# polimi-ispl/deep_prior_interpolation

Hardware: AMD Instinct MI355X
Metric: Adam iters/sec on 3D MultiRes-UNet (whole job over n_gpus; per_gpu beside it); recon SNR(dB) vs ref under config.snr_vs_reference (higher is better)
Workload: dtype f32

## Files before the change

deep_prior_interpolation_amd/_lib.py:

```python
import ctypes as C
import os

_HERE = os.path.dirname(os.path.abspath(__file__))
LIB_PATH = os.path.join(_HERE, "libdpi_hip.so")


class DpiError(RuntimeError):
    pass


ABI_VERSION = 406

IO_X_BF16, IO_Y_BF16, IO_DY_BF16, IO_DX_BF16 = 1, 2, 4, 8
STORE_FWD_BF16, STORE_GRAD_BF16 = 1, 2


class ConvDesc(C.Structure):
    _fields_ = [("size", C.c_int), ("Cin", C.c_int), ("Cout", C.c_int), ("D", C.c_int), ("H", C.c_int), ("W", C.c_int),
                ("k", C.c_int), ("kd", C.c_int), ("stride", C.c_int), ("precision", C.c_int), ("io", C.c_int)]

    def __init__(self, Cin=0, Cout=0, D=1, H=1, W=1, k=1, kd=1, stride=1, precision=0, io=0):
        super().__init__(C.sizeof(ConvDesc), int(Cin), int(Cout), int(D), int(H), int(W), int(k), int(kd), int(stride), int(precision), int(io))


class AdamTensor(C.Structure):
    _fields_ = [("p", C.c_void_p), ("g", C.c_void_p), ("m", C.c_void_p), ("v", C.c_void_p)]


_P = C.c_void_p
_I = C.c_int
_Z = C.c_size_t
_F = C.c_float
_U64 = C.c_uint64
_DESC = C.POINTER(ConvDesc)
_U = C.c_uint

SIGNATURES = {
    "dpi_last_error": (C.c_char_p, []),
    "dpi_version": (_I, []),
    "dpi_conv_desc_size": (_I, []),
    "dpi_device_info": (_I, [_I, C.POINTER(_I), C.POINTER(_I), C.POINTER(_Z), C.c_char_p, _I]),
    "dpi_profile_marker": (_I, [_I, _P]),
    "dpi_conv_fwd_stat_blocks": (_I, [_DESC]),
    "dpi_conv_fwd": (_I, [_DESC, _P, _P, _P, _P, _P, _P, _P]),
    "dpi_conv_bwd_data": (_I, [_DESC, _P, _P, _P, _I, _P]),
    "dpi_conv_fwd_ws_floats": (_Z, [_DESC]),
    "dpi_conv_bwd_data_ws_floats": (_Z, [_DESC]),
    "dpi_conv_fwd_ws": (_I, [_DESC, _P, _P, _P, _P, _P, _P, _P, _Z, _P]),
    "dpi_conv_bwd_data_ws": (_I, [_DESC, _P, _P, _P, _I, _P, _Z, _P]),
    "dpi_conv_bwd_data_dual": (_I, [_DESC, _P, _P, _DESC, _P, _P, _P, _I, _P, _Z, _P]),
    "dpi_conv_bwd_weight_ws_floats": (_Z, [_DESC]),
    "dpi_conv_bwd_weight": (_I, [_DESC, _P, _P, _P, _P, _P, _Z, _P]),
    "dpi_stat_blocks": (_I, [_I, _Z]),
    "dpi_channel_stats": (_I, [_P, _P, _I, _Z, _P, _P]),
    "dpi_bn_finalize": (_I, [_P, _I, _I, _Z, _P, _P, _F, _F, _F, _I, _P, _P, _P, _P, _P, _P, _P]),
    "dpi_chain_apply": (_I, [_P, _P, _I, _Z, _P, _P]),
    "dpi_bn_bwd_reduce": (_I, [_P, _P, _P, _P, _P, _P, _F, _F, _I, _Z, _P, _P]),
    "dpi_bn_bwd_apply": (_I, [_P, _P, _P, _P, _P, _P, _F, _F, _P, _I, _I, _Z, _P, _P, _P, _P]),
    "dpi_bn_bwd_apply_fork": (_I, [_P, _P, _P, _P, _P, _P, _F, _F, _P, _I, _I, _Z, _P, _P, _P,
                                   _P, _P, _P, _P, _P, _F, _P, _P, _P, _P, _P, _P, _F, _P, _P]),
    "dpi_bn_bwd_apply_dual": (_I, [_P, _I, _I, _Z] + [_P, _P, _P, _P, _P, _F, _P, _P, _P, _P] * 2 + [_I, _I, _P, _P, _P, _F, _P, _P]),
    "dpi_chain_add_stats": (_I, [_P, _P, _P, _P, _I, _Z, _F, _P, _P, _P]),
    "dpi_lrelu_bwd": (_I, [_P, _P, _F, _Z, _P, _P]),
    "dpi_act_fwd": (_I, [_P, _Z, _I, _P, _P]),
    "dpi_act_bwd": (_I, [_P, _P, _Z, _I, _P, _P]),
    "dpi_add": (_I, [_P, _P, _Z, _P, _P]),
    "dpi_channel_sum": (_I, [_P, _I, _Z, _P, _P, _P]),
    "dpi_upsample2x_fwd": (_I, [_P, _P, _I, _I, _I, _I, _I, _I, _I, _I, _P, _P]),
    "dpi_upsample2x_bwd_ws_floats": (_Z, [_I, _I, _I, _I, _I, _I, _I, _I]),
    "dpi_upsample2x_bwd": (_I, [_P, _I, _I, _I, _I, _I, _I, _I, _I, _P, _P, _P]),
    "dpi_crop_copy": (_I, [_P, _I, _I, _I, _I, _I, _I, _I, _I, _I, _I, _P, _P]),
    "dpi_crop_copy_bwd": (_I, [_P, _I, _I, _I, _I, _I, _I, _I, _I, _I, _I, _P, _P]),
    "dpi_maxpool2x2_fwd": (_I, [_P, _I, _I, _I, _P, _P]),
    "dpi_maxpool2x2_bwd": (_I, [_P, _P, _I, _I, _I, _P, _P]),
    "dpi_deconv4x4s2_fwd": (_I, [_P, _P, _P, _I, _I, _I, _I, _P, _P]),
    "dpi_deconv4x4s2_bwd_data": (_I, [_P, _P, _I, _I, _I, _I, _P, _P]),
    "dpi_deconv4x4s2_bwd_weight": (_I, [_P, _P, _I, _I, _I, _I, _P, _P]),
    "dpi_loss_ws_doubles": (_Z, [_Z]),
    "dpi_masked_loss": (_I, [_P, _P, _P, _Z, _I, _F, _P, _P, _P, _P]),
    "dpi_adam_multi": (_I, [_P, _P, _I, _P, C.c_double, C.c_double, C.c_double, _P, _P]),
    "dpi_langevin_multi": (_I, [_P, _P, _I, _P, _I, C.c_double, C.c_double, C.c_double, C.c_double, C.c_double, _U64, _P, _P, _P]),
    "dpi_moments_update": (_I, [_P, _P, _P, _Z, _P, _I, _I, _P, _P]),
    "dpi_loop_control": (_I, [_P, _P, _P, _I, _P, _P, _P, _I, C.c_double, C.c_double, _I, C.c_double, C.c_double, _I, C.c_double, _P]),
    "dpi_copy_if": (_I, [_P, _P, _P, _Z, _P]),
    "dpi_masked_loss_holdout": (_I, [_P, _P, _P, _P, _I, _I, _Z, _I, _F, _P, _P, _P, _P]),
    "dpi_loop_control_holdout": (_I, [_P, _P, _P, _I, _P, _P, _P, _I, C.c_double, C.c_double, _I, C.c_double, C.c_double, _I, C.c_double, _P]),
    "dpi_ema_loss": (_I, [_P, _P, _P, _P, _P, _I, _I, _Z, _I, _F, _P, _P, _P, _P, _P]),
    "dpi_loop_control_ema": (_I, [_P, _P, _I, _P, _P, _I, _P, _P, _P, _I, C.c_double, C.c_double, _I, C.c_double, C.c_double, _I, C.c_double, _P]),
    "dpi_noise_add": (_I, [_P, _Z, _F, _U64, _P, _P, _P]),
    "dpi_fill_normal": (_I, [_P, _Z, _F, _F, _U64, _U64, _P]),
    "dpi_fir_axis0": (_I, [_P, _P, _I, _I, _I, _Z, _P, _P]),
    "dpi_axpy": (_I, [_F, _P, _Z, _P, _P]),
    "dpi_diff_axis": (_I, [_P, _Z, _I, _Z, _I, _F, _I, _P, _P]),
    "dpi_hale2d": (_I, [_P, _P, _P, _P, _Z, _I, _I, _I, _P, _P]),
    "dpi_structure_tensor": (_I, [_P, _Z, _I, _I, _F, _F, _P, _P, _P, _P]),
    "dpi_dips": (_I, [_P, _P, _P, _Z, _P, _P, _P]),
    "dpi_hale_sections": (_I, [_P, _P, _I, _I, _I, _I, _I, _P, _P]),
    "dpi_structure_tensor_sections": (_I, [_P, _I, _I, _I, _I, _F, _F, _F, _P, _P, _P, _P, _P, _P]),
    "dpi_max_ws_floats": (_Z, [_Z]),
    "dpi_scaled_max": (_I, [_P, _Z, _F, _P, _P, _P]),
    "dpi_threshold": (_I, [_P, _Z, _P, _P, _P]),
    "dpi_pocs_project": (_I, [_P, _P, _P, _Z, _P, _P]),
    "dpi_overlap_add": (_I, [_P, _I, _I, _I, _I, _I, _I, _P, _I, _I, _I, _P]),
    "dpi_overlap_normalize": (_I, [_P, _I, _I, _I, _I, _I, _I, _I, _I, _I, _F, _P]),
    "dpi_overlap_add_weighted": (_I, [_P, _P, _I, _I, _I, _I, _I, _I, _P, _I, _P, _I, _P, _I, _U, _P, _I, _I, _I, _I, _P]),
    "dpi_overlap_finalize_weighted": (_I, [_P, _I, _I, _I, _I, _F, _P, _P, _P]),
    "dpi_channel_stats_io": (_I, [_P, _P, _I, _Z, _P, _U, _P]),
    "dpi_chain_apply_io": (_I, [_P, _P, _I, _Z, _P, _U, _P]),
    "dpi_chain_add_stats_io": (_I, [_P, _P, _P, _P, _I, _Z, _F, _P, _P, _U, _P]),
    "dpi_bn_bwd_reduce_io": (_I, [_P, _P, _P, _P, _P, _P, _F, _F, _I, _Z, _P, _U, _P]),
    "dpi_bn_bwd_apply_io": (_I, [_P, _P, _P, _P, _P, _P, _F, _F, _P, _I, _I, _Z, _P, _P, _P, _U, _P]),
    "dpi_bn_bwd_apply_fork_io": (_I, [_P, _P, _P, _P, _P, _P, _F, _F, _P, _I, _I, _Z, _P, _P, _P,
                                      _P, _P, _P, _P, _P, _F, _P, _P, _P, _P, _P, _P, _F, _P, _U, _P]),
    "dpi_bn_bwd_apply_dual_io": (_I, [_P, _I, _I, _Z] + [_P, _P, _P, _P, _P, _F, _P, _P, _P, _P] * 2 + [_I, _I, _P, _P, _P, _F, _P, _U, _P]),
    "dpi_upsample2x_fwd_io": (_I, [_P, _P, _I, _I, _I, _I, _I, _I, _I, _I, _P, _U, _P]),
    "dpi_upsample2x_bwd_io": (_I, [_P, _I, _I, _I, _I, _I, _I, _I, _I, _P, _P, _U, _P]),
    "dpi_noise_add_io": (_I, [_P, _Z, _F, _U64, _P, _P, _U, _P]),
    "dpi_noise_add_regen_io": (_I, [_Z, _F, _U64, _U64, _F, _U64, _P, _P, _U, _P]),
    "dpi_set_option": (_I, [C.c_char_p, _I]),
    "dpi_pack_scratch_bytes": (_Z, []),
    "dpi_pack_release": (_I, []),
    "dpi_pack_forget": (_I, [_P]),
    "dpi_pack_slot_count": (_Z, []),
    "dpi_join_bwd_ws_doubles": (_Z, [_I, _Z]),
    "dpi_join_bwd": (_I, [_P, _P, _P, _P, _P, _F, _I, _Z,  _P, _P, _P, _P, _P, _F,  _P, _P, _P, _P, _P, _F,  _P, _P,  _I, _I, _P, _P, _P, _F,
                          _P, _P, _P, _P, _P, _P, _P, _U, _P]),
    "dpi_chain_add_apply": (_I, [_P, _P, _P, _P, _P, _I, _Z, _P, _U, _P]),
}

_lib = None


def load():
    global _lib
    if _lib is not None:
        return _lib
    if not os.path.exists(LIB_PATH):
        raise DpiError("libdpi_hip.so not found at %s — run `python -c 'import __graft_entry__ as g; g.build()'` "
                       "(hipcc --offload-arch=gfx950); there is no CPU fallback" % LIB_PATH)
    import torch
    lib = C.CDLL(LIB_PATH)
    for name, (res, args) in SIGNATURES.items():
        try:
            fn = getattr(lib, name)
        except AttributeError as e:
            raise DpiError("libdpi_hip.so does not export %s (stale build?)" % name) from e
        fn.restype = res
        fn.argtypes = args
    if lib.dpi_version() < ABI_VERSION or lib.dpi_conv_desc_size() != C.sizeof(ConvDesc):
        raise DpiError("libdpi_hip.so is ABI version %d with a %d-byte dpi_conv_desc; this binding needs >= %d and %d bytes (stale build? "
                       "re-run __graft_entry__.build())" % (lib.dpi_version(), lib.dpi_conv_desc_size(), ABI_VERSION, C.sizeof(ConvDesc)))
    lib.set_option = lambda key, value: check(lib.dpi_set_option(key.encode(), int(value)), "dpi_set_option(%s)" % key)
    _lib = lib
    return lib


def check(code, what=""):
    if code != 0:
        msg = load().dpi_last_error()
        raise DpiError("%s failed (%d): %s" % (what, code, msg.decode() if msg else "?"))


def ptr(t):
    return None if t is None else t.data_ptr()


def stream():
    import torch
    return torch.cuda.current_stream().cuda_stream
```

deep_prior_interpolation_amd/csrc/api.cpp:

```cpp
#include <stdarg.h>
#include <string.h>
#include "common.h"

static thread_local char g_err[512] = "";

void dpi_set_error(const char* fmt, ...) {
  va_list ap;
  va_start(ap, fmt);
  vsnprintf(g_err, sizeof(g_err), fmt, ap);
  va_end(ap);
}

int dpi_check_launch(const char* what) {
  const hipError_t e = hipGetLastError();
  if (e != hipSuccess) {
    dpi_set_error("%s: %s", what, hipGetErrorString(e));
    return DPI_E_LAUNCH;
  }
  return DPI_OK;
}

extern "C" const char* dpi_last_error(void) { return g_err; }
extern "C" int dpi_version(void) { return 406; }
extern "C" int dpi_conv_desc_size(void) { return (int)sizeof(dpi_conv_desc); }

extern "C" int dpi_device_info(int device, int* cus, int* lds_bytes, size_t* hbm_bytes, char* name, int name_len) {
  hipDeviceProp_t p;
  const hipError_t e = hipGetDeviceProperties(&p, device);
  if (e != hipSuccess) {
    dpi_set_error("device_info: %s", hipGetErrorString(e));
    return DPI_E_LAUNCH;
  }
  if (cus) *cus = p.multiProcessorCount;
  if (lds_bytes) *lds_bytes = (int)p.sharedMemPerBlock;
  if (hbm_bytes) *hbm_bytes = p.totalGlobalMem;
  if (name && name_len > 0) {
    strncpy(name, p.gcnArchName, name_len - 1);
    name[name_len - 1] = 0;
  }
  return DPI_OK;
}

__global__ void dpi_marker_kernel() {}

extern "C" int dpi_profile_marker(int id, void* stream) {
  DPI_REQUIRE(id >= 1 && id < 65536, "profile_marker: id %d out of range", id);
  dpi_marker_kernel<<<(unsigned)id, 64, 0, (hipStream_t)stream>>>();
  return dpi_check_launch("profile_marker");
}

extern "C" int dpi_set_option(const char* key, int value) {
  DPI_REQUIRE(key != nullptr, "set_option: key is NULL");
  struct Entry { const char* key; int lo, hi; void (*set)(int); };
  static const Entry table[] = {
      {"splitk", 0, 1, dpi_set_splitk},
      {"dual_bwd_data", 0, 1, dpi_set_dual_bwd_data},
      {"bw_pair", 0, 2, dpi_set_bw_pair},
      {"bw_workgroups", 1, 1 << 24, [](int v) { dpi_set_bw_tuning(v, -1); }},
      {"bw_xcd_order", 0, 1, [](int v) { dpi_set_bw_tuning(0, v); }},
      {"mfma_min_cout", 0, 1 << 20, dpi_set_mfma_min_cout},
      {"bwd_weight_mfma_min_cout", 0, 1 << 20, dpi_set_bwd_weight_mfma_min_cout},
      {"fewco_mfma", 0, 1, dpi_set_fewco_mfma},
      {"q4", 0, 2, [](int v) { dpi_set_q4(v, -1); }},
      {"q4_ck", 0, 4, [](int v) { dpi_set_q4(-1, v); }},
      {"q4_debug", 0, 0xFFFF, dpi_set_q4_debug},
      {"bf16_debug", 0, 0x7F, dpi_set_bf16_debug},
  };
  for (const Entry& e : table)
    if (strcmp(key, e.key) == 0) {
      DPI_REQUIRE(value >= e.lo && value <= e.hi && !(strcmp(key, "q4_ck") == 0 && value != 0 && value != 2 && value != 4),
                  "set_option: %s = %d out of range [%d, %d]", key, value, e.lo, e.hi);
      e.set(value);
      return DPI_OK;
    }
  dpi_set_error("set_option: unknown key '%s'", key);
  return DPI_E_ARG;
}
```

deep_prior_interpolation_amd/csrc/dpi_hip_internal.h:

```cpp
#pragma once
#define DPI_INTERNAL __attribute__((visibility("hidden")))
extern "C" {
DPI_INTERNAL void dpi_set_bw_tuning(int want_workgroups, int xcd_order);
DPI_INTERNAL void dpi_set_bf16_debug(int flags);
DPI_INTERNAL void dpi_set_splitk(int on);
DPI_INTERNAL void dpi_set_dual_bwd_data(int on);
DPI_INTERNAL void dpi_set_bw_pair(int mode);
DPI_INTERNAL void dpi_set_mfma_min_cout(int n);
DPI_INTERNAL void dpi_set_bwd_weight_mfma_min_cout(int n);
DPI_INTERNAL void dpi_set_fewco_mfma(int on);
DPI_INTERNAL void dpi_set_q4(int on, int ck);
DPI_INTERNAL void dpi_set_q4_debug(int flags);
}
```

deep_prior_interpolation_amd/csrc/elementwise.hip:

```cpp
#include "common.h"
#include <stdlib.h>

namespace {

constexpr int kStatSpan = 16384;
constexpr int kMaxStatBlocks = 2048;

__host__ __device__ inline size_t stat_span(size_t V, int nblk) {
  size_t s = (V + nblk - 1) / nblk;
  return (s + 3) & ~(size_t)3;
}

typedef float ew_f32x4 __attribute__((ext_vector_type(4)));
constexpr size_t kNtMinFloats = (size_t)32 << 20;
__device__ __forceinline__ float4 ld4(const float* p, bool nt) {
  if (nt) { const ew_f32x4 v = __builtin_nontemporal_load(reinterpret_cast<const ew_f32x4*>(p)); return make_float4(v[0], v[1], v[2], v[3]); }
  return *reinterpret_cast<const float4*>(p);
}
__device__ __forceinline__ void st4(float* p, float4 v, bool nt) {
  if (nt) __builtin_nontemporal_store((ew_f32x4){v.x, v.y, v.z, v.w}, reinterpret_cast<ew_f32x4*>(p));
  else *reinterpret_cast<float4*>(p) = v;
}

template <bool xb = false>
__global__ __launch_bounds__(256) void channel_stats_kernel(const float* __restrict__ x, const float* __restrict__ chain,
                                                            int C, size_t V, int nblk, double* __restrict__ partials) {
  const bool nt = (size_t)gridDim.y * V >= kNtMinFloats;
  const int c = blockIdx.y, b = blockIdx.x;
  const size_t span = stat_span(V, nblk);
  const size_t beg = (size_t)b * span, end = beg + span < V ? beg + span : V;
  const float* __restrict__ xc = dpi_at(x, (size_t)c * V, xb);
  const Chain t = load_chain(chain, c);
  double s = 0.0, q = 0.0;
  const bool vec = (V & 3) == 0;
  for (size_t i = beg + (size_t)threadIdx.x * 4; i < end; i += 1024) {
    float v[4];
    if (vec) {
      const float4 f = dpi_ld4(xc, i, xb, nt);
      v[0] = f.x; v[1] = f.y; v[2] = f.z; v[3] = f.w;
    } else {
#pragma unroll
      for (int k = 0; k < 4; ++k) v[k] = i + k < end ? dpi_ld(xc, i + k, xb) : 0.f;
    }
    float ls = 0.f;
    double lq = 0.0;
#pragma unroll
    for (int k = 0; k < 4; ++k)
      if (i + k < end) {
        const float y = apply_chain(t, v[k]);
        ls += y;
        lq += (double)y * y;
      }
    s += ls; q += lq;
  }
  __shared__ double sh[8];
  const double S = block_sum(s, sh);
  const double Q = block_sum(q, sh + 4);
  if (threadIdx.x == 0) {
    partials[((size_t)b * C + c) * 2 + 0] = S;
    partials[((size_t)b * C + c) * 2 + 1] = Q;
  }
}

__global__ __launch_bounds__(256) void bn_finalize_kernel(const double* __restrict__ partials, int nblk, int C, double count,
                                                         const float* __restrict__ gamma, const float* __restrict__ beta,
                                                         float eps, float momentum, float slope, int act_first,
                                                         const float* __restrict__ in_chain, float* running_mean, float* running_var, int64_t* nbt,
                                                         float* __restrict__ mean_invstd, float* __restrict__ chain_out) {
  const int c = blockIdx.x, lane = threadIdx.x;
  double s = 0.0, q = 0.0;
  {
    double s1 = 0.0, q1 = 0.0;
    int b = lane;
    for (; b + 256 < nblk; b += 512) {
      const double2 u = *reinterpret_cast<const double2*>(partials + ((size_t)b * C + c) * 2);
      const double2 v = *reinterpret_cast<const double2*>(partials + ((size_t)(b + 256) * C + c) * 2);
      s += u.x; q += u.y; s1 += v.x; q1 += v.y;
    }
    if (b < nblk) {
      const double2 u = *reinterpret_cast<const double2*>(partials + ((size_t)b * C + c) * 2);
      s += u.x; q += u.y;
    }
    s += s1; q += q1;
  }
  __shared__ double sh[8];
  s = block_sum(s, sh);
  q = block_sum(q, sh + 4);
  if (lane == 0) {
    const double mean = s / count;
    double var = q / count - mean * mean;
    if (var < 0.0) var = 0.0;
    const float invstd = (float)(1.0 / sqrt(var + (double)eps));
    const float meanf = (float)mean;
    if (mean_invstd) { mean_invstd[c] = meanf; mean_invstd[C + c] = invstd; }
    if (running_mean) running_mean[c] = (1.f - momentum) * running_mean[c] + momentum * meanf;
    if (running_var) {
      const double unb = count > 1.0 ? var * (count / (count - 1.0)) : var;
      running_var[c] = (1.f - momentum) * running_var[c] + momentum * (float)unb;
    }
    if (nbt && c == 0) *nbt += 1;
    if (chain_out) {
      const float g = gamma ? gamma[c] : 1.f, bt = beta ? beta[c] : 0.f;
      const float a = g * invstd;
      float* o = chain_out + (size_t)c * DPI_CHAIN_STRIDE;
      if (in_chain) {
        const float* ic = in_chain + (size_t)c * DPI_CHAIN_STRIDE;
        o[0] = ic[0]; o[1] = ic[1]; o[2] = ic[2]; o[3] = a * ic[3]; o[4] = fmaf(a, ic[4], bt - meanf * a);
      } else if (act_first) { o[0] = 1.f; o[1] = 0.f; o[2] = slope; o[3] = a; o[4] = bt - meanf * a; }
      else { o[0] = a; o[1] = bt - meanf * a; o[2] = slope; o[3] = 1.f; o[4] = 0.f; }
    }
  }
}

template <bool xb = false, bool yb = false>
__global__ __launch_bounds__(256) void chain_apply_kernel(const float* __restrict__ x, const float* __restrict__ chain, size_t V,
                                                          float* __restrict__ y) {
  const bool nt = (size_t)gridDim.y * V >= kNtMinFloats;
  const int c = blockIdx.y;
  const Chain t = load_chain(chain, c);
  const float* __restrict__ xc = dpi_at(x, (size_t)c * V, xb);
  float* __restrict__ yc = dpi_at(y, (size_t)c * V, yb);
  const bool vec = (V & 3) == 0;
  for (size_t i = ((size_t)blockIdx.x * 256 + threadIdx.x) * 4; i < V; i += (size_t)gridDim.x * 1024) {
    if (vec) {
      float4 f = dpi_ld4(xc, i, xb, nt);
      f.x = apply_chain(t, f.x); f.y = apply_chain(t, f.y); f.z = apply_chain(t, f.z); f.w = apply_chain(t, f.w);
      dpi_st4(yc, i, f, yb, nt);
    } else {
      for (int k = 0; k < 4 && i + k < V; ++k) dpi_st(yc, i + k, apply_chain(t, dpi_ld(xc, i + k, xb)), yb);
    }
  }
}

struct BnBwd {
  float mean, invstd, a, pb, pre, post;
  bool chained;
  Chain in;
};
__device__ __forceinline__ BnBwd bn_bwd_consts(const float* __restrict__ mean_invstd, const float* __restrict__ gamma,
                                               const float* __restrict__ beta, const float* __restrict__ in_chain, float pre,
                                               float post, int C, int c) {
  BnBwd k;
  k.chained = in_chain != nullptr;
  k.in = load_chain(in_chain, c);
  k.mean = mean_invstd[c]; k.invstd = mean_invstd[C + c];
  k.a = (gamma ? gamma[c] : 1.f) * k.invstd;
  k.pb = (beta ? beta[c] : 0.f) - k.mean * k.a;
  k.pre = pre; k.post = post;
  return k;
}
__device__ __forceinline__ void bn_bwd_elem(const BnBwd& k, float x, float dy, float& xhat, float& g) {
  if (k.chained) x = apply_chain(k.in, x);
  const float u = x > 0.f ? x : x * k.pre;
  xhat = (u - k.mean) * k.invstd;
  const float yv = fmaf(k.a, u, k.pb);
  g = (k.post == 1.f || yv > 0.f) ? dy : dy * k.post;
}

template <bool fb = false, bool gb = false>
__global__ __launch_bounds__(256) void bn_bwd_reduce_kernel(const float* __restrict__ dy, const float* __restrict__ x,
                                                            const float* __restrict__ mean_invstd, const float* __restrict__ gamma,
                                                            const float* __restrict__ beta, const float* __restrict__ in_chain,
                                                            float pre, float post, int C, size_t V, int nblk,
                                                            double* __restrict__ partials) {
  const bool nt = (size_t)gridDim.y * V >= kNtMinFloats;
  const int c = blockIdx.y, b = blockIdx.x;
  const size_t span = stat_span(V, nblk);
  const size_t beg = (size_t)b * span, end = beg + span < V ? beg + span : V;
  const BnBwd k = bn_bwd_consts(mean_invstd, gamma, beta, in_chain, pre, post, C, c);
  const float* __restrict__ xc = dpi_at(x, (size_t)c * V, fb);
  const float* __restrict__ gc = dpi_at(dy, (size_t)c * V, gb);
  double s = 0.0, q = 0.0;
  const bool vec = (V & 3) == 0;
  for (size_t i = beg + (size_t)threadIdx.x * 4; i < end; i += 1024) {
    float xv[4], gv[4];
    if (vec) {
      const float4 f = dpi_ld4(xc, i, fb, nt);
      const float4 g = dpi_ld4(gc, i, gb, nt);
      xv[0] = f.x; xv[1] = f.y; xv[2] = f.z; xv[3] = f.w;
      gv[0] = g.x; gv[1] = g.y; gv[2] = g.z; gv[3] = g.w;
    } else {
#pragma unroll
      for (int j = 0; j < 4; ++j) { xv[j] = i + j < end ? dpi_ld(xc, i + j, fb) : 0.f; gv[j] = i + j < end ? dpi_ld(gc, i + j, gb) : 0.f; }
    }
    float ls = 0.f, lq = 0.f;
#pragma unroll
    for (int j = 0; j < 4; ++j)
      if (i + j < end) {
        float xh, g;
        bn_bwd_elem(k, xv[j], gv[j], xh, g);
        ls += g; lq = fmaf(g, xh, lq);
      }
    s += ls; q += lq;
  }
  __shared__ double sh[8];
  const double S = block_sum(s, sh);
  const double Q = block_sum(q, sh + 4);
  if (threadIdx.x == 0) {
    partials[((size_t)b * C + c) * 2 + 0] = S;
    partials[((size_t)b * C + c) * 2 + 1] = Q;
  }
}

template <bool fb = false, bool gb = false>
__global__ __launch_bounds__(256) void bn_bwd_apply_kernel(const float* __restrict__ dy, const float* __restrict__ x,
                                                           const float* __restrict__ mean_invstd, const float* __restrict__ gamma,
                                                           const float* __restrict__ beta, const float* __restrict__ in_chain,
                                                           float pre, float post, const double* __restrict__ partials, int nblk, int C, size_t V,
                                                           float* __restrict__ dx, float* __restrict__ dgamma,
                                                           float* __restrict__ dbeta) {
  const bool nt = (size_t)gridDim.y * V >= kNtMinFloats;
  const int c = blockIdx.y;
  __shared__ double tot[2];
  if (threadIdx.x < 64) {
    double s = 0.0, q = 0.0;
    for (int b = threadIdx.x; b < nblk; b += 64) {
      s += partials[((size_t)b * C + c) * 2 + 0];
      q += partials[((size_t)b * C + c) * 2 + 1];
    }
    s = wave_sum(s);
    q = wave_sum(q);
    if (threadIdx.x == 0) { tot[0] = s; tot[1] = q; }
  }
  __syncthreads();
  const BnBwd k = bn_bwd_consts(mean_invstd, gamma, beta, in_chain, pre, post, C, c);
  const float k1 = (float)(tot[0] / (double)V), k2 = (float)(tot[1] / (double)V);
  if (blockIdx.x == 0 && threadIdx.x == 0) {
    if (dgamma) dgamma[c] = (float)tot[1];
    if (dbeta) dbeta[c] = (float)tot[0];
  }
  const float* __restrict__ xc = dpi_at(x, (size_t)c * V, fb);
  const float* __restrict__ gc = dpi_at(dy, (size_t)c * V, gb);
  float* __restrict__ oc = dpi_at(dx, (size_t)c * V, gb);
  const bool vec = (V & 3) == 0;
  auto one = [&](float xv, float gv) {
    float xh, g;
    bn_bwd_elem(k, xv, gv, xh, g);
    const float du = k.a * (g - k1 - xh * k2);
    return (k.pre == 1.f || xv > 0.f) ? du : du * k.pre;
  };
  for (size_t i = ((size_t)blockIdx.x * 256 + threadIdx.x) * 4; i < V; i += (size_t)gridDim.x * 1024) {
    if (vec) {
      const float4 f = dpi_ld4(xc, i, fb, nt);
      const float4 g = dpi_ld4(gc, i, gb, nt);
      dpi_st4(oc, i, make_float4(one(f.x, g.x), one(f.y, g.y), one(f.z, g.z), one(f.w, g.w)), gb, nt);
    } else {
      for (int j = 0; j < 4 && i + j < V; ++j) dpi_st(oc, i + j, one(dpi_ld(xc, i + j, fb), dpi_ld(gc, i + j, gb)), gb);
    }
  }
}

template <bool fb = false>
__global__ __launch_bounds__(256) void chain_add_stats_kernel(const float* __restrict__ a, const float* __restrict__ chain_a,
                                                              const float* __restrict__ b, const float* __restrict__ chain_b, int C,
                                                              size_t V, int nblk, float slope, float* __restrict__ t,
                                                              double* __restrict__ partials) {
  const bool nt = (size_t)gridDim.y * V >= kNtMinFloats;
  const int c = blockIdx.y, blk = blockIdx.x;
  const size_t span = stat_span(V, nblk);
  const size_t beg = (size_t)blk * span, end = beg + span < V ? beg + span : V;
  const Chain ta = load_chain(chain_a, c), tb = load_chain(chain_b, c);
  const float* __restrict__ ac = dpi_at(a, (size_t)c * V, fb);
  const float* __restrict__ bc = dpi_at(b, (size_t)c * V, fb);
  float* __restrict__ tc = dpi_at(t, (size_t)c * V, fb);
  double s = 0.0, q = 0.0;
  const bool vec = (V & 3) == 0;
  for (size_t i = beg + (size_t)threadIdx.x * 4; i < end; i += 1024) {
    float av[4], bv[4], tv[4];
    if (vec) {
      const float4 f = dpi_ld4(ac, i, fb, nt);
      const float4 g = dpi_ld4(bc, i, fb, nt);
      av[0] = f.x; av[1] = f.y; av[2] = f.z; av[3] = f.w;
      bv[0] = g.x; bv[1] = g.y; bv[2] = g.z; bv[3] = g.w;
    } else {
#pragma unroll
      for (int j = 0; j < 4; ++j) { av[j] = i + j < end ? dpi_ld(ac, i + j, fb) : 0.f; bv[j] = i + j < end ? dpi_ld(bc, i + j, fb) : 0.f; }
    }
    float ls = 0.f;
    double lq = 0.0;
#pragma unroll
    for (int j = 0; j < 4; ++j) {
      tv[j] = dpi_stored(apply_chain(ta, av[j]) + apply_chain(tb, bv[j]), fb && t != nullptr);
      if (i + j < end) {
        const float y = tv[j] > 0.f ? tv[j] : tv[j] * slope;
        ls += y;
        lq += (double)y * y;
      }
    }
    if (t != nullptr) {
      if (vec) dpi_st4(tc, i, make_float4(tv[0], tv[1], tv[2], tv[3]), fb, nt);
      else
        for (int j = 0; j < 4 && i + j < end; ++j) dpi_st(tc, i + j, tv[j], fb);
    }
    s += ls; q += lq;
  }
  __shared__ double sh[8];
  const double S = block_sum(s, sh);
  const double Q = block_sum(q, sh + 4);
  if (threadIdx.x == 0) {
    partials[((size_t)blk * C + c) * 2 + 0] = S;
    partials[((size_t)blk * C + c) * 2 + 1] = Q;
  }
}

struct BnFork {
  const float* x;
  const float* mean_invstd;
  const float* gamma;
  const float* beta;
  const float* in_chain;
  float post;
  double* partials;
};
template <bool tb = false, bool gb = false>
__global__ __launch_bounds__(256) void bn_bwd_apply_fork_kernel(const float* __restrict__ dy, const float* __restrict__ x,
                                                                const float* __restrict__ mean_invstd, const float* __restrict__ gamma,
                                                                const float* __restrict__ beta, const float* __restrict__ in_chain,
                                                                float pre, float post, const double* __restrict__ partials, int nblk_in,
                                                                int C, size_t V, int nblk, float* __restrict__ dx,
                                                                float* __restrict__ dgamma, float* __restrict__ dbeta, BnFork fa, BnFork fb) {
  const bool nt = (size_t)gridDim.y * V >= kNtMinFloats;
  const int c = blockIdx.y, b = blockIdx.x;
  __shared__ double tot[2];
  if (threadIdx.x < 64) {
    double s = 0.0, q = 0.0;
    for (int i = threadIdx.x; i < nblk_in; i += 64) {
      s += partials[((size_t)i * C + c) * 2 + 0];
      q += partials[((size_t)i * C + c) * 2 + 1];
    }
    s = wave_sum(s);
    q = wave_sum(q);
    if (threadIdx.x == 0) { tot[0] = s; tot[1] = q; }
  }
  __syncthreads();
  const BnBwd k = bn_bwd_consts(mean_invstd, gamma, beta, in_chain, pre, post, C, c);
  const float k1 = (float)(tot[0] / (double)V), k2 = (float)(tot[1] / (double)V);
  if (b == 0 && threadIdx.x == 0) {
    if (dgamma) dgamma[c] = (float)tot[1];
    if (dbeta) dbeta[c] = (float)tot[0];
  }
  const BnBwd ka = fa.x ? bn_bwd_consts(fa.mean_invstd, fa.gamma, fa.beta, fa.in_chain, 1.f, fa.post, C, c) : k;
  const BnBwd kb = fb.x ? bn_bwd_consts(fb.mean_invstd, fb.gamma, fb.beta, fb.in_chain, 1.f, fb.post, C, c) : k;
  const size_t span = stat_span(V, nblk);
  const size_t beg = (size_t)b * span, end = beg + span < V ? beg + span : V;
  const float* __restrict__ xc = dpi_at(x, (size_t)c * V, tb);
  const float* __restrict__ gc = dpi_at(dy, (size_t)c * V, gb);
  const float* __restrict__ xa = fa.x ? dpi_at(fa.x, (size_t)c * V, tb) : xc;
  const float* __restrict__ xb = fb.x ? dpi_at(fb.x, (size_t)c * V, tb) : xc;
  float* __restrict__ oc = dpi_at(dx, (size_t)c * V, gb);
  double sa = 0.0, qa = 0.0, sb = 0.0, qb = 0.0;
  const bool vec = (V & 3) == 0;
  for (size_t i = beg + (size_t)threadIdx.x * 4; i < end; i += 1024) {
    float xv[4], gv[4], av[4], bv[4], o[4];
    if (vec) {
      const float4 f = dpi_ld4(xc, i, tb, nt);
      const float4 g = dpi_ld4(gc, i, gb, nt);
      xv[0] = f.x; xv[1] = f.y; xv[2] = f.z; xv[3] = f.w;
      gv[0] = g.x; gv[1] = g.y; gv[2] = g.z; gv[3] = g.w;
      if (fa.x) { const float4 t = dpi_ld4(xa, i, tb, nt); av[0] = t.x; av[1] = t.y; av[2] = t.z; av[3] = t.w; }
      if (fb.x) { const float4 t = dpi_ld4(xb, i, tb, nt); bv[0] = t.x; bv[1] = t.y; bv[2] = t.z; bv[3] = t.w; }
    } else {
#pragma unroll
      for (int j = 0; j < 4; ++j) {
        const bool in = i + j < end;
        xv[j] = in ? dpi_ld(xc, i + j, tb) : 0.f; gv[j] = in ? dpi_ld(gc, i + j, gb) : 0.f;
        av[j] = (in && fa.x) ? dpi_ld(xa, i + j, tb) : 0.f; bv[j] = (in && fb.x) ? dpi_ld(xb, i + j, tb) : 0.f;
      }
    }
    float lsa = 0.f, lqa = 0.f, lsb = 0.f, lqb = 0.f;
#pragma unroll
    for (int j = 0; j < 4; ++j) {
      float xh, g;
      bn_bwd_elem(k, xv[j], gv[j], xh, g);
      const float du = k.a * (g - k1 - xh * k2);
      o[j] = dpi_stored((k.pre == 1.f || xv[j] > 0.f) ? du : du * k.pre, gb);
      if (i + j < end) {
        if (fa.x) { float h, ga_; bn_bwd_elem(ka, av[j], o[j], h, ga_); lsa += ga_; lqa = fmaf(ga_, h, lqa); }
        if (fb.x) { float h, gb_; bn_bwd_elem(kb, bv[j], o[j], h, gb_); lsb += gb_; lqb = fmaf(gb_, h, lqb); }
      }
    }
    if (vec) dpi_st4(oc, i, make_float4(o[0], o[1], o[2], o[3]), gb, nt);
    else
      for (int j = 0; j < 4 && i + j < end; ++j) dpi_st(oc, i + j, o[j], gb);
    sa += lsa; qa += lqa; sb += lsb; qb += lqb;
  }
  __shared__ double sh[16];
  const double SA = block_sum(sa, sh), QA = block_sum(qa, sh + 4), SB = block_sum(sb, sh + 8), QB = block_sum(qb, sh + 12);
  if (threadIdx.x == 0) {
    if (fa.x) { fa.partials[((size_t)b * C + c) * 2 + 0] = SA; fa.partials[((size_t)b * C + c) * 2 + 1] = QA; }
    if (fb.x) { fb.partials[((size_t)b * C + c) * 2 + 0] = SB; fb.partials[((size_t)b * C + c) * 2 + 1] = QB; }
  }
}

struct BnSide {
  const float* x;
  const float* mean_invstd;
  const float* gamma;
  const float* beta;
  const float* in_chain;
  float post;
  const double* partials;
  float* dx;
  float* dgamma;
  float* dbeta;
};
template <bool tb = false, bool gb = false>
__global__ __launch_bounds__(256) void bn_bwd_apply_dual_kernel(const float* __restrict__ dy, BnSide A, BnSide B, int nblk_in, int C, size_t V,
                                                                int nblk, int f_lo, int f_hi, const float* __restrict__ f_mi,
                                                                const float* __restrict__ f_gamma, const float* __restrict__ f_beta,
                                                                float f_post, double* __restrict__ f_partials) {
  const bool nt = (size_t)gridDim.y * V >= kNtMinFloats;
  const int c = blockIdx.y, b = blockIdx.x;
  __shared__ double tot[4];
  if (threadIdx.x < 64) {
    double sa = 0.0, qa = 0.0, sb = 0.0, qb = 0.0;
    for (int i = threadIdx.x; i < nblk_in; i += 64) {
      sa += A.partials[((size_t)i * C + c) * 2 + 0]; qa += A.partials[((size_t)i * C + c) * 2 + 1];
      sb += B.partials[((size_t)i * C + c) * 2 + 0]; qb += B.partials[((size_t)i * C + c) * 2 + 1];
    }
    sa = wave_sum(sa); qa = wave_sum(qa); sb = wave_sum(sb); qb = wave_sum(qb);
    if (threadIdx.x == 0) { tot[0] = sa; tot[1] = qa; tot[2] = sb; tot[3] = qb; }
  }
  __syncthreads();
  const BnBwd ka = bn_bwd_consts(A.mean_invstd, A.gamma, A.beta, A.in_chain, 1.f, A.post, C, c);
  const BnBwd kb = bn_bwd_consts(B.mean_invstd, B.gamma, B.beta, B.in_chain, 1.f, B.post, C, c);
  const float a1 = (float)(tot[0] / (double)V), a2 = (float)(tot[1] / (double)V);
  const float b1 = (float)(tot[2] / (double)V), b2 = (float)(tot[3] / (double)V);
  if (b == 0 && threadIdx.x == 0) {
    if (A.dgamma) A.dgamma[c] = (float)tot[1];
    if (A.dbeta) A.dbeta[c] = (float)tot[0];
    if (B.dgamma) B.dgamma[c] = (float)tot[3];
    if (B.dbeta) B.dbeta[c] = (float)tot[2];
  }
  const bool forked = f_partials && c >= f_lo && c < f_hi;
  const int fc = forked ? c - f_lo : 0, fC = f_hi - f_lo;
  const BnBwd kf = forked ? bn_bwd_consts(f_mi, f_gamma, f_beta, nullptr, 1.f, f_post, fC, fc) : ka;
  const size_t span = stat_span(V, nblk);
  const size_t beg = (size_t)b * span, end = beg + span < V ? beg + span : V;
  const float* __restrict__ gc = dpi_at(dy, (size_t)c * V, gb);
  const float* __restrict__ xa = dpi_at(A.x, (size_t)c * V, tb);
  const float* __restrict__ xb = dpi_at(B.x, (size_t)c * V, tb);
  float* __restrict__ oa = dpi_at(A.dx, (size_t)c * V, gb);
  float* __restrict__ ob = dpi_at(B.dx, (size_t)c * V, gb);
  double sf = 0.0, qf = 0.0;
  const bool vec = (V & 3) == 0;
  for (size_t i = beg + (size_t)threadIdx.x * 4; i < end; i += 1024) {
    float gv[4], av[4], bv[4], ra[4], rb[4];
    if (vec) {
      const float4 g = dpi_ld4(gc, i, gb, nt);
      const float4 t = dpi_ld4(xa, i, tb, nt);
      const float4 u = dpi_ld4(xb, i, tb, nt);
      gv[0] = g.x; gv[1] = g.y; gv[2] = g.z; gv[3] = g.w;
      av[0] = t.x; av[1] = t.y; av[2] = t.z; av[3] = t.w;
      bv[0] = u.x; bv[1] = u.y; bv[2] = u.z; bv[3] = u.w;
    } else {
#pragma unroll
      for (int j = 0; j < 4; ++j) {
        const bool in = i + j < end;
        gv[j] = in ? dpi_ld(gc, i + j, gb) : 0.f; av[j] = in ? dpi_ld(xa, i + j, tb) : 0.f; bv[j] = in ? dpi_ld(xb, i + j, tb) : 0.f;
      }
    }
    float lsf = 0.f, lqf = 0.f;
#pragma unroll
    for (int j = 0; j < 4; ++j) {
      float xh, g;
      bn_bwd_elem(ka, av[j], gv[j], xh, g);
      ra[j] = ka.a * (g - a1 - xh * a2);
      bn_bwd_elem(kb, bv[j], gv[j], xh, g);
      rb[j] = dpi_stored(kb.a * (g - b1 - xh * b2), gb);
      if (forked && i + j < end) { float h, gf_; bn_bwd_elem(kf, bv[j], rb[j], h, gf_); lsf += gf_; lqf = fmaf(gf_, h, lqf); }
    }
    if (vec) {
      dpi_st4(oa, i, make_float4(ra[0], ra[1], ra[2], ra[3]), gb, nt);
      dpi_st4(ob, i, make_float4(rb[0], rb[1], rb[2], rb[3]), gb, nt);
    } else {
      for (int j = 0; j < 4 && i + j < end; ++j) { dpi_st(oa, i + j, ra[j], gb); dpi_st(ob, i + j, rb[j], gb); }
    }
    sf += lsf; qf += lqf;
  }
  if (f_partials && f_hi > f_lo) {
    __shared__ double sh[8];
    const double SF = block_sum(sf, sh), QF = block_sum(qf, sh + 4);
    if (threadIdx.x == 0 && forked) {
      f_partials[((size_t)b * fC + fc) * 2 + 0] = SF;
      f_partials[((size_t)b * fC + fc) * 2 + 1] = QF;
    }
  }
}

template <bool fb = false>
__global__ __launch_bounds__(256) void chain_add_apply_kernel(const float* __restrict__ a, const float* __restrict__ chain_a,
                                                              const float* __restrict__ b, const float* __restrict__ chain_b,
                                                              const float* __restrict__ chain_out, size_t V, float* __restrict__ y) {
  const bool nt = (size_t)gridDim.y * V >= kNtMinFloats;
  const int c = blockIdx.y;
  const Chain ta = load_chain(chain_a, c), tb = load_chain(chain_b, c), to = load_chain(chain_out, c);
  const float* __restrict__ ac = dpi_at(a, (size_t)c * V, fb);
  const float* __restrict__ bc = dpi_at(b, (size_t)c * V, fb);
  float* __restrict__ yc = dpi_at(y, (size_t)c * V, fb);
  const bool vec = (V & 3) == 0;
  for (size_t i = ((size_t)blockIdx.x * 256 + threadIdx.x) * 4; i < V; i += (size_t)gridDim.x * 1024) {
    if (vec) {
      const float4 f = dpi_ld4(ac, i, fb, nt), g = dpi_ld4(bc, i, fb, nt);
      float4 o;
      o.x = apply_chain(to, apply_chain(ta, f.x) + apply_chain(tb, g.x)); o.y = apply_chain(to, apply_chain(ta, f.y) + apply_chain(tb, g.y));
      o.z = apply_chain(to, apply_chain(ta, f.z) + apply_chain(tb, g.z)); o.w = apply_chain(to, apply_chain(ta, f.w) + apply_chain(tb, g.w));
      dpi_st4(yc, i, o, fb, nt);
    } else {
      for (int j = 0; j < 4 && i + j < V; ++j)
        dpi_st(yc, i + j, apply_chain(to, apply_chain(ta, dpi_ld(ac, i + j, fb)) + apply_chain(tb, dpi_ld(bc, i + j, fb))), fb);
    }
  }
}

constexpr int kJoinSums = 24;
constexpr int kJoinGroups = 2;
struct JoinSide {
  const float* x;
  const float* mean_invstd;
  const float* gamma;
  const float* beta;
  const float* in_chain;
  float post;
  const float* fwd_chain;
};
struct JoinFork {
  int lo, hi;
  const float* mean_invstd;
  const float* gamma;
  const float* beta;
  float post;
};
template <bool fb = false, bool gb = false>
__global__ __launch_bounds__(256) void join_bwd_sums_kernel(const float* __restrict__ dy, const float* __restrict__ t,
                                                            const float* __restrict__ mean_invstd, const float* __restrict__ gamma,
                                                            const float* __restrict__ beta, float pre, JoinSide A, JoinSide B, JoinFork F,
                                                            int C, size_t V, int nblk, double* __restrict__ partials) {
  const bool nt = (size_t)gridDim.y * V >= kNtMinFloats;
  const int c = blockIdx.y, b = blockIdx.x;
  const BnBwd k = bn_bwd_consts(mean_invstd, gamma, beta, nullptr, pre, 1.f, C, c);
  const BnBwd ka = bn_bwd_consts(A.mean_invstd, A.gamma, A.beta, A.in_chain, 1.f, A.post, C, c);
  const BnBwd kb = bn_bwd_consts(B.mean_invstd, B.gamma, B.beta, B.in_chain, 1.f, B.post, C, c);
  const bool forked = c >= F.lo && c < F.hi;
  const int fC = F.hi - F.lo, fc = forked ? c - F.lo : 0;
  const BnBwd kf = forked ? bn_bwd_consts(F.mean_invstd, F.gamma, F.beta, nullptr, 1.f, F.post, fC, fc) : ka;
  const size_t span = stat_span(V, nblk);
  const size_t beg = (size_t)b * span, end = beg + span < V ? beg + span : V;
  const float* __restrict__ gc = dpi_at(dy, (size_t)c * V, gb);
  const float* __restrict__ tc = t ? dpi_at(t, (size_t)c * V, fb) : nullptr;
  const float* __restrict__ xa = dpi_at(A.x, (size_t)c * V, fb);
  const float* __restrict__ xb = dpi_at(B.x, (size_t)c * V, fb);
  const Chain fwa = load_chain(A.fwd_chain, c), fwb = load_chain(B.fwd_chain, c);
  double s[kJoinSums];
#pragma unroll
  for (int i = 0; i < kJoinSums; ++i) s[i] = 0.0;
  const bool vec = (V & 3) == 0;
  for (size_t i0 = beg + (size_t)threadIdx.x * 4; i0 < end; i0 += 1024 * kJoinGroups) {
   float l[kJoinSums];
#pragma unroll
   for (int q = 0; q < kJoinSums; ++q) l[q] = 0.f;
#pragma unroll
   for (int u = 0; u < kJoinGroups; ++u) {
    const size_t i = i0 + (size_t)u * 1024;
    if (i >= end) break;
    float gv[4], tv[4], av[4], bv[4];
    if (vec) {
      const float4 g = dpi_ld4(gc, i, gb, nt), p = dpi_ld4(xa, i, fb, nt), q = dpi_ld4(xb, i, fb, nt);
      gv[0] = g.x; gv[1] = g.y; gv[2] = g.z; gv[3] = g.w;
      av[0] = p.x; av[1] = p.y; av[2] = p.z; av[3] = p.w;
      bv[0] = q.x; bv[1] = q.y; bv[2] = q.z; bv[3] = q.w;
      if (tc) { const float4 u = dpi_ld4(tc, i, fb, nt); tv[0] = u.x; tv[1] = u.y; tv[2] = u.z; tv[3] = u.w; }
    } else {
#pragma unroll
      for (int j = 0; j < 4; ++j) {
        const bool in = i + j < end;
        gv[j] = in ? dpi_ld(gc, i + j, gb) : 0.f; tv[j] = (in && tc) ? dpi_ld(tc, i + j, fb) : 0.f;
        av[j] = in ? dpi_ld(xa, i + j, fb) : 0.f; bv[j] = in ? dpi_ld(xb, i + j, fb) : 0.f;
      }
    }
    if (!tc) {
#pragma unroll
      for (int j = 0; j < 4; ++j) tv[j] = apply_chain(fwa, av[j]) + apply_chain(fwb, bv[j]);
    }
#pragma unroll
    for (int j = 0; j < 4; ++j)
      if (i + j < end) {
        float X, D, Xa, ma, Xb, mb;
        bn_bwd_elem(k, tv[j], gv[j], X, D);
        bn_bwd_elem(ka, av[j], 1.f, Xa, ma);
        bn_bwd_elem(kb, bv[j], 1.f, Xb, mb);
        const float P = (k.pre == 1.f || tv[j] > 0.f) ? k.a : k.a * k.pre;
        l[0] += D; l[1] = fmaf(D, X, l[1]);
        const float wa = ma * P, wb = mb * P;
        const float waD = wa * D, waX = wa * X, wbD = wb * D, wbX = wb * X;
        l[2] += waD; l[3] += wa; l[4] += waX;
        l[5] = fmaf(waD, Xa, l[5]); l[6] = fmaf(wa, Xa, l[6]); l[7] = fmaf(waX, Xa, l[7]);
        l[8] += wbD; l[9] += wb; l[10] += wbX;
        l[11] = fmaf(wbD, Xb, l[11]); l[12] = fmaf(wb, Xb, l[12]); l[13] = fmaf(wbX, Xb, l[13]);
        if (forked) {
          float Xf, mf;
          bn_bwd_elem(kf, bv[j], 1.f, Xf, mf);
          const float wf = mf * wb, wfD = wf * D, wfX = wf * X, mfXf = mf * Xf;
          l[14] += wfD; l[15] += wf; l[16] += wfX; l[17] += mf; l[18] = fmaf(mf, Xb, l[18]);
          l[19] = fmaf(wfD, Xf, l[19]); l[20] = fmaf(wf, Xf, l[20]); l[21] = fmaf(wfX, Xf, l[21]); l[22] += mfXf; l[23] = fmaf(mfXf, Xb, l[23]);
        }
      }
   }
#pragma unroll
   for (int q = 0; q < kJoinSums; ++q) s[q] += (double)l[q];
  }
  __shared__ double sh[4][kJoinSums];
  const int lane = threadIdx.x & 63, wid = threadIdx.x >> 6;
#pragma unroll
  for (int i = 0; i < kJoinSums; ++i) {
    const double v = wave_sum(s[i]);
    if (lane == 0) sh[wid][i] = v;
  }
  __syncthreads();
  if (threadIdx.x < kJoinSums) {
    const int i = threadIdx.x;
    partials[((size_t)b * C + c) * kJoinSums + i] = (sh[0][i] + sh[1][i]) + (sh[2][i] + sh[3][i]);
  }
}

__global__ __launch_bounds__(64) void join_bwd_coef_kernel(const double* __restrict__ partials, int nblk, int C, double V,
                                                          const float* __restrict__ mi_b, const float* __restrict__ gamma_b, int f_lo, int f_hi,
                                                          float* __restrict__ coef, float* __restrict__ dgb, float* __restrict__ dgb_f) {
  const int c = blockIdx.x, lane = threadIdx.x;
  double s[kJoinSums];
#pragma unroll
  for (int i = 0; i < kJoinSums; ++i) s[i] = 0.0;
  for (int b = lane; b < nblk; b += 64) {
    const double* __restrict__ p = partials + ((size_t)b * C + c) * kJoinSums;
#pragma unroll
    for (int i = 0; i < kJoinSums; ++i) s[i] += p[i];
  }
#pragma unroll
  for (int i = 0; i < kJoinSums; ++i) s[i] = wave_sum(s[i]);
  if (lane != 0) return;
  const double k1 = s[0] / V, k2 = s[1] / V;
  const double Ga = s[2] - k1 * s[3] - k2 * s[4], Ha = s[5] - k1 * s[6] - k2 * s[7];
  const double Gb = s[8] - k1 * s[9] - k2 * s[10], Hb = s[11] - k1 * s[12] - k2 * s[13];
  const float k1f = (float)k1, k2f = (float)k2, a1f = (float)(Ga / V), a2f = (float)(Ha / V), b1f = (float)(Gb / V), b2f = (float)(Hb / V);
  float f1f = 0.f, f2f = 0.f;
  if (c >= f_lo && c < f_hi) {
    const double ab = (double)((gamma_b ? gamma_b[c] : 1.f) * mi_b[C + c]);
    const double T1 = s[14] - k1 * s[15] - k2 * s[16], TX = s[19] - k1 * s[20] - k2 * s[21];
    const double Gf = ab * (T1 - (double)b1f * s[17] - (double)b2f * s[18]);
    const double Hf = ab * (TX - (double)b1f * s[22] - (double)b2f * s[23]);
    f1f = (float)(Gf / V); f2f = (float)(Hf / V);
    dgb_f[c - f_lo] = (float)Hf;
    dgb_f[(f_hi - f_lo) + c - f_lo] = (float)Gf;
  }
  float* o = coef + (size_t)c * 8;
  o[0] = k1f; o[1] = k2f; o[2] = a1f; o[3] = a2f; o[4] = b1f; o[5] = b2f; o[6] = f1f; o[7] = f2f;
  dgb[c] = (float)s[1]; dgb[C + c] = (float)s[0]; dgb[2 * C + c] = (float)Ha; dgb[3 * C + c] = (float)Ga;
  dgb[4 * C + c] = (float)Hb; dgb[5 * C + c] = (float)Gb;
}

template <bool fb = false, bool gb = false>
__global__ __launch_bounds__(256) void join_bwd_apply_kernel(const float* __restrict__ dy, const float* __restrict__ t,
                                                             const float* __restrict__ mean_invstd, const float* __restrict__ gamma,
                                                             const float* __restrict__ beta, float pre, JoinSide A, JoinSide B, JoinFork F,
                                                             const float* __restrict__ coef, int C, size_t V, float* __restrict__ dxa,
                                                             float* __restrict__ dxb, float* __restrict__ dxf) {
  const bool nt = (size_t)gridDim.y * V >= kNtMinFloats;
  const int c = blockIdx.y;
  const BnBwd k = bn_bwd_consts(mean_invstd, gamma, beta, nullptr, pre, 1.f, C, c);
  const BnBwd ka = bn_bwd_consts(A.mean_invstd, A.gamma, A.beta, A.in_chain, 1.f, A.post, C, c);
  const BnBwd kb = bn_bwd_consts(B.mean_invstd, B.gamma, B.beta, B.in_chain, 1.f, B.post, C, c);
  const bool forked = c >= F.lo && c < F.hi;
  const int fC = F.hi - F.lo, fc = forked ? c - F.lo : 0;
  const BnBwd kf = forked ? bn_bwd_consts(F.mean_invstd, F.gamma, F.beta, nullptr, 1.f, F.post, fC, fc) : ka;
  const float* __restrict__ q = coef + (size_t)c * 8;
  const float k1 = q[0], k2 = q[1], a1 = q[2], a2 = q[3], b1 = q[4], b2 = q[5], f1 = q[6], f2 = q[7];
  const float* __restrict__ gc = dpi_at(dy, (size_t)c * V, gb);
  const float* __restrict__ tc = t ? dpi_at(t, (size_t)c * V, fb) : nullptr;
  const float* __restrict__ xa = dpi_at(A.x, (size_t)c * V, fb);
  const float* __restrict__ xb = dpi_at(B.x, (size_t)c * V, fb);
  const Chain fwa = load_chain(A.fwd_chain, c), fwb = load_chain(B.fwd_chain, c);
  float* __restrict__ oa = dpi_at(dxa, (size_t)c * V, gb);
  float* __restrict__ ob = forked ? dpi_at(dxf, (size_t)fc * V, gb) : dpi_at(dxb, (size_t)c * V, gb);
  const bool vec = (V & 3) == 0;
  auto one = [&](float gv, float tv, float av, float bv, float& ra, float& rb) {
    float X, g, xh, gg;
    bn_bwd_elem(k, tv, gv, X, g);
    const float du = k.a * (g - k1 - X * k2);
    const float dt = (k.pre == 1.f || tv > 0.f) ? du : du * k.pre;
    bn_bwd_elem(ka, av, dt, xh, gg);
    ra = ka.a * (gg - a1 - xh * a2);
    bn_bwd_elem(kb, bv, dt, xh, gg);
    rb = kb.a * (gg - b1 - xh * b2);
    if (forked) {
      bn_bwd_elem(kf, bv, rb, xh, gg);
      rb = kf.a * (gg - f1 - xh * f2);
    }
  };
  for (size_t i = ((size_t)blockIdx.x * 256 + threadIdx.x) * 4; i < V; i += (size_t)gridDim.x * 1024) {
    if (vec) {
      const float4 g = dpi_ld4(gc, i, gb, nt), p = dpi_ld4(xa, i, fb, nt), r = dpi_ld4(xb, i, fb, nt);
      float4 u;
      if (tc) u = dpi_ld4(tc, i, fb, nt);
      else u = make_float4(apply_chain(fwa, p.x) + apply_chain(fwb, r.x), apply_chain(fwa, p.y) + apply_chain(fwb, r.y),
                           apply_chain(fwa, p.z) + apply_chain(fwb, r.z), apply_chain(fwa, p.w) + apply_chain(fwb, r.w));
      float4 ya, yb;
      one(g.x, u.x, p.x, r.x, ya.x, yb.x); one(g.y, u.y, p.y, r.y, ya.y, yb.y);
      one(g.z, u.z, p.z, r.z, ya.z, yb.z); one(g.w, u.w, p.w, r.w, ya.w, yb.w);
      dpi_st4(oa, i, ya, gb, nt);
      dpi_st4(ob, i, yb, gb, nt);
    } else {
      for (int j = 0; j < 4 && i + j < V; ++j) {
        float ra, rb;
        const float av = dpi_ld(xa, i + j, fb), bv = dpi_ld(xb, i + j, fb);
        one(dpi_ld(gc, i + j, gb), tc ? dpi_ld(tc, i + j, fb) : apply_chain(fwa, av) + apply_chain(fwb, bv), av, bv, ra, rb);
        dpi_st(oa, i + j, ra, gb); dpi_st(ob, i + j, rb, gb);
      }
    }
  }
}

__global__ __launch_bounds__(256) void lrelu_bwd_kernel(const float* __restrict__ dy, const float* __restrict__ x, float slope,
                                                        size_t n, float* __restrict__ dx) {
  const bool nt = n >= kNtMinFloats;
  const bool vec = (n & 3) == 0;
  for (size_t i = ((size_t)blockIdx.x * 256 + threadIdx.x) * 4; i < n; i += (size_t)gridDim.x * 1024) {
    if (vec) {
      const float4 f = ld4(x + i, nt);
      float4 g = ld4(dy + i, nt);
      g.x = f.x > 0.f ? g.x : g.x * slope; g.y = f.y > 0.f ? g.y : g.y * slope;
      g.z = f.z > 0.f ? g.z : g.z * slope; g.w = f.w > 0.f ? g.w : g.w * slope;
      st4(dx + i, g, nt);
    } else {
      for (int k = 0; k < 4 && i + k < n; ++k) dx[i + k] = x[i + k] > 0.f ? dy[i + k] : dy[i + k] * slope;
    }
  }
}

__device__ __forceinline__ float act_fwd_one(int kind, float x) {
  if (kind == DPI_ACT_ELU) return x > 0.f ? x : expm1f(x);
  if (kind == DPI_ACT_TANH) return tanhf(x);
  return 1.f / (1.f + expf(-x));
}
__device__ __forceinline__ float act_bwd_one(int kind, float y, float dy) {
  if (kind == DPI_ACT_ELU) return y > 0.f ? dy : dy * (y + 1.f);
  if (kind == DPI_ACT_TANH) return dy * (1.f - y * y);
  return dy * (y * (1.f - y));
}
__global__ __launch_bounds__(256) void act_fwd_kernel(const float* __restrict__ x, size_t n, int kind, float* __restrict__ y) {
  const bool vec = (n & 3) == 0;
  for (size_t i = ((size_t)blockIdx.x * 256 + threadIdx.x) * 4; i < n; i += (size_t)gridDim.x * 1024) {
    if (vec) {
      float4 f = *reinterpret_cast<const float4*>(x + i);
      f.x = act_fwd_one(kind, f.x); f.y = act_fwd_one(kind, f.y); f.z = act_fwd_one(kind, f.z); f.w = act_fwd_one(kind, f.w);
      *reinterpret_cast<float4*>(y + i) = f;
    } else {
      for (int k = 0; k < 4 && i + k < n; ++k) y[i + k] = act_fwd_one(kind, x[i + k]);
    }
  }
}
__global__ __launch_bounds__(256) void act_bwd_kernel(const float* __restrict__ dy, const float* __restrict__ y, size_t n, int kind,
                                                      float* __restrict__ dx) {
  const bool vec = (n & 3) == 0;
  for (size_t i = ((size_t)blockIdx.x * 256 + threadIdx.x) * 4; i < n; i += (size_t)gridDim.x * 1024) {
    if (vec) {
      const float4 f = *reinterpret_cast<const float4*>(y + i);
      float4 g = *reinterpret_cast<const float4*>(dy + i);
      g.x = act_bwd_one(kind, f.x, g.x); g.y = act_bwd_one(kind, f.y, g.y); g.z = act_bwd_one(kind, f.z, g.z); g.w = act_bwd_one(kind, f.w, g.w);
      *reinterpret_cast<float4*>(dx + i) = g;
    } else {
      for (int k = 0; k < 4 && i + k < n; ++k) dx[i + k] = act_bwd_one(kind, y[i + k], dy[i + k]);
    }
  }
}

__global__ __launch_bounds__(256) void add_kernel(const float* __restrict__ a, const float* __restrict__ b, size_t n,
                                                  float* __restrict__ y) {
  const bool nt = n >= kNtMinFloats;
  const bool vec = (n & 3) == 0;
  for (size_t i = ((size_t)blockIdx.x * 256 + threadIdx.x) * 4; i < n; i += (size_t)gridDim.x * 1024) {
    if (vec) {
      const float4 f = ld4(a + i, nt);
      const float4 g = ld4(b + i, nt);
      st4(y + i, make_float4(f.x + g.x, f.y + g.y, f.z + g.z, f.w + g.w), nt);
    } else {
      for (int k = 0; k < 4 && i + k < n; ++k) y[i + k] = a[i + k] + b[i + k];
    }
  }
}

__global__ __launch_bounds__(64) void channel_sum_final_kernel(const double* __restrict__ partials, int nblk, int C,
                                                               float* __restrict__ out) {
  const int c = blockIdx.x;
  double s = 0.0;
  for (int b = threadIdx.x; b < nblk; b += 64) s += partials[((size_t)b * C + c) * 2];
  s = wave_sum(s);
  if (threadIdx.x == 0) out[c] = (float)s;
}

__device__ __forceinline__ void lin_src(int o, int n, int& i0, int& i1, float& w0, float& w1) {
  const int h = o >> 1;
  if (o & 1) { i0 = h; i1 = min(h + 1, n - 1); w0 = .75f; w1 = .25f; }
  else { i0 = max(h - 1, 0); i1 = h; w0 = (h == 0) ? 0.f : .25f; w1 = (h == 0) ? 1.f : .75f; }
}

template <bool xb = false, bool yb = false>
__global__ __launch_bounds__(256) void upsample_fwd_kernel(const float* __restrict__ x, const float* __restrict__ chain, int D, int H,
                                                           int W, int Do, int Ho, int Wo, int linear, int scale_d,
                                                           float* __restrict__ y) {
  const int c = blockIdx.y;
  const size_t Vo = (size_t)Do * Ho * Wo, V = (size_t)D * H * W;
  const Chain t = load_chain(chain, c);
  const float* __restrict__ xc = dpi_at(x, (size_t)c * V, xb);
  float* __restrict__ yc = dpi_at(y, (size_t)c * Vo, yb);
  for (size_t i = (size_t)blockIdx.x * 256 + threadIdx.x; i < Vo; i += (size_t)gridDim.x * 256) {
    const int ow = i % Wo, oh = (i / Wo) % Ho, od = i / ((size_t)Wo * Ho);
    float r;
    if (!linear) {
      const int id = scale_d ? od >> 1 : od;
      r = apply_chain(t, dpi_ld(xc, ((size_t)id * H + (oh >> 1)) * W + (ow >> 1), xb));
    } else {
      int d0, d1, h0, h1, w0, w1;
      float a0, a1, b0, b1, c0, c1;
      if (scale_d) lin_src(od, D, d0, d1, a0, a1); else { d0 = d1 = od; a0 = 1.f; a1 = 0.f; }
      lin_src(oh, H, h0, h1, b0, b1);
      lin_src(ow, W, w0, w1, c0, c1);
      auto at = [&](int d, int h, int w) { return apply_chain(t, dpi_ld(xc, ((size_t)d * H + h) * W + w, xb)); };
      const float p0 = b0 * (c0 * at(d0, h0, w0) + c1 * at(d0, h0, w1)) + b1 * (c0 * at(d0, h1, w0) + c1 * at(d0, h1, w1));
      r = a0 * p0;
      if (scale_d)
        r += a1 * (b0 * (c0 * at(d1, h0, w0) + c1 * at(d1, h0, w1)) + b1 * (c0 * at(d1, h1, w0) + c1 * at(d1, h1, w1)));
    }
    dpi_st(yc, i, r, yb);
  }
}

__device__ __forceinline__ float lin_wt(int o, int i, int n) {
  int i0, i1; float w0, w1;
  lin_src(o, n, i0, i1, w0, w1);
  return (i0 == i ? w0 : 0.f) + (i1 == i ? w1 : 0.f);
}

template <bool gb = false>
__global__ __launch_bounds__(256) void upsample_bwd_kernel(const float* __restrict__ dy, int D, int H, int W, int Do, int Ho, int Wo,
                                                           int linear, int scale_d, float* __restrict__ dx) {
  const int c = blockIdx.y;
  const size_t Vo = (size_t)Do * Ho * Wo, V = (size_t)D * H * W;
  const float* __restrict__ gc = dpi_at(dy, (size_t)c * Vo, gb);
  float* __restrict__ oc = dpi_at(dx, (size_t)c * V, gb);
  for (size_t i = (size_t)blockIdx.x * 256 + threadIdx.x; i < V; i += (size_t)gridDim.x * 256) {
    const int iw = i % W, ih = (i / W) % H, id = i / ((size_t)W * H);
    float acc = 0.f;
    if (!linear) {
      const int dlo = scale_d ? 2 * id : id, dhi = scale_d ? 2 * id + 1 : id;
      for (int od = dlo; od <= dhi && od < Do; ++od)
        for (int oh = 2 * ih; oh <= 2 * ih + 1 && oh < Ho; ++oh)
          for (int ow = 2 * iw; ow <= 2 * iw + 1 && ow < Wo; ++ow) acc += dpi_ld(gc, ((size_t)od * Ho + oh) * Wo + ow, gb);
    } else {
      const int dlo = scale_d ? max(2 * id - 1, 0) : id, dhi = scale_d ? min(2 * id + 2, Do - 1) : id;
      for (int od = dlo; od <= dhi; ++od) {
        const float wd = scale_d ? lin_wt(od, id, D) : 1.f;
        if (wd == 0.f) continue;
        for (int oh = max(2 * ih - 1, 0); oh <= min(2 * ih + 2, Ho - 1); ++oh) {
          const float wh = lin_wt(oh, ih, H);
          if (wh == 0.f) continue;
          for (int ow = max(2 * iw - 1, 0); ow <= min(2 * iw + 2, Wo - 1); ++ow) {
            const float ww = lin_wt(ow, iw, W);
            if (ww != 0.f) acc = fmaf(wd * wh * ww, dpi_ld(gc, ((size_t)od * Ho + oh) * Wo + ow, gb), acc);
          }
        }
      }
    }
    dpi_st(oc, i, acc, gb);
  }
}

template <bool SCALE_D, bool xb = false, bool yb = false>
__global__ __launch_bounds__(256) void upsample_lin_fwd_cube_kernel(const float* __restrict__ x, const float* __restrict__ chain, int D, int H,
                                                                    int W, int Do, int Ho, int Wo, float* __restrict__ y) {
  const int c = blockIdx.y;
  const size_t V = (size_t)D * H * W, Vo = (size_t)Do * Ho * Wo;
  const Chain t = load_chain(chain, c);
  const float* __restrict__ xc = dpi_at(x, (size_t)c * V, xb);
  float* __restrict__ yc = dpi_at(y, (size_t)c * Vo, yb);
  for (size_t i = (size_t)blockIdx.x * 256 + threadIdx.x; i < V; i += (size_t)gridDim.x * 256) {
    const int w = i % W, h = (i / W) % H, d = i / ((size_t)W * H);
    const int wm = max(w - 1, 0), wp = min(w + 1, W - 1), hm = max(h - 1, 0), hp = min(h + 1, H - 1);
    const int dm = SCALE_D ? max(d - 1, 0) : d, dp = SCALE_D ? min(d + 1, D - 1) : d;
    const int ds_[3] = {dm, d, dp}, hs_[3] = {hm, h, hp}, ws_[3] = {wm, w, wp};
    float lo[3][3], hi[3][3];
#pragma unroll
    for (int a = 0; a < (SCALE_D ? 3 : 1); ++a)
#pragma unroll
      for (int b = 0; b < 3; ++b) {
        const size_t row = ((size_t)ds_[SCALE_D ? a : 1] * H + hs_[b]) * W;
        const float v0 = apply_chain(t, dpi_ld(xc, row + ws_[0], xb)), v1 = apply_chain(t, dpi_ld(xc, row + ws_[1], xb)),
                    v2 = apply_chain(t, dpi_ld(xc, row + ws_[2], xb));
        lo[a][b] = .25f * v0 + .75f * v1;
        hi[a][b] = .75f * v1 + .25f * v2;
      }
#pragma unroll
    for (int od_ = 0; od_ < (SCALE_D ? 2 : 1); ++od_) {
      const int od = SCALE_D ? 2 * d + od_ : d;
      if (od >= Do) continue;
#pragma unroll
      for (int oh_ = 0; oh_ < 2; ++oh_) {
        const int oh = 2 * h + oh_;
        if (oh >= Ho) continue;
        float r0, r1;
        auto hcomb = [&](int a, float& l, float& u) {
          l = oh_ == 0 ? .25f * lo[a][0] + .75f * lo[a][1] : .75f * lo[a][1] + .25f * lo[a][2];
          u = oh_ == 0 ? .25f * hi[a][0] + .75f * hi[a][1] : .75f * hi[a][1] + .25f * hi[a][2];
        };
        if (SCALE_D) {
          float l0, u0, l1, u1, l2, u2;
          hcomb(0, l0, u0); hcomb(1, l1, u1); hcomb(2, l2, u2);
          r0 = od_ == 0 ? .25f * l0 + .75f * l1 : .75f * l1 + .25f * l2;
          r1 = od_ == 0 ? .25f * u0 + .75f * u1 : .75f * u1 + .25f * u2;
        } else {
          hcomb(0, r0, r1);
        }
        const size_t o = ((size_t)od * Ho + oh) * Wo + 2 * w;
        if (yb && 2 * w + 1 < Wo && !((o + (size_t)c * Vo) & 1)) {
          reinterpret_cast<unsigned*>(reinterpret_cast<unsigned short*>(yc) + o)[0] = dpi_pack_bf16(r0, r1);
        } else {
          if (2 * w < Wo) dpi_st(yc, o, r0, yb);
          if (2 * w + 1 < Wo) dpi_st(yc, o + 1, r1, yb);
        }
      }
    }
  }
}

__device__ __forceinline__ void lin_bwd_taps(int i, int n, int no, int (&o)[4], float (&wt)[4]) {
  o[0] = 2 * i - 1; o[1] = 2 * i; o[2] = 2 * i + 1; o[3] = 2 * i + 2;
  wt[0] = i > 0 ? .25f : 0.f;
  wt[1] = i == 0 ? 1.f : .75f;
  wt[2] = i == n - 1 ? 1.f : .75f;
  wt[3] = i < n - 1 ? .25f : 0.f;
#pragma unroll
  for (int k = 0; k < 4; ++k) {
    if (o[k] < 0 || o[k] >= no) { wt[k] = 0.f; o[k] = 0; }
  }
}

template <bool SCALE_D, bool gb = false>
__global__ __launch_bounds__(256) void upsample_lin_bwd_gather_kernel(const float* __restrict__ dy, int D, int H, int W, int Do, int Ho,
                                                                      int Wo, float* __restrict__ dx) {
  const int c = blockIdx.y;
  const size_t V = (size_t)D * H * W, Vo = (size_t)Do * Ho * Wo;
  const float* __restrict__ gc = dpi_at(dy, (size_t)c * Vo, gb);
  float* __restrict__ oc = dpi_at(dx, (size_t)c * V, gb);
  for (size_t i = (size_t)blockIdx.x * 256 + threadIdx.x; i < V; i += (size_t)gridDim.x * 256) {
    const int w = i % W, h = (i / W) % H, d = i / ((size_t)W * H);
    int ow[4], oh[4], od[4];
    float ww[4], wh[4], wd[4];
    lin_bwd_taps(w, W, Wo, ow, ww);
    lin_bwd_taps(h, H, Ho, oh, wh);
    if (SCALE_D) lin_bwd_taps(d, D, Do, od, wd);
    float acc = 0.f;
#pragma unroll
    for (int a = 0; a < (SCALE_D ? 4 : 1); ++a) {
      const int od_ = SCALE_D ? od[a] : d;
      const float wa = SCALE_D ? wd[a] : 1.f;
      float accd = 0.f;
#pragma unroll
      for (int b = 0; b < 4; ++b) {
        const size_t row = ((size_t)od_ * Ho + oh[b]) * Wo;
        const float rsum = ww[0] * dpi_ld(gc, row + ow[0], gb) + ww[1] * dpi_ld(gc, row + ow[1], gb) + ww[2] * dpi_ld(gc, row + ow[2], gb)
                           + ww[3] * dpi_ld(gc, row + ow[3], gb);
        accd = fmaf(wh[b], rsum, accd);
      }
      acc = fmaf(wa, accd, acc);
    }
    dpi_st(oc, i, acc, gb);
  }
}

template <bool ib = false, bool ob = false>
__global__ __launch_bounds__(256) void upsample_lin_bwd_axis_kernel(const float* __restrict__ in, float* __restrict__ out, unsigned outer,
                                                                    int n, int no, unsigned inner) {
  const unsigned slab = (unsigned)n * inner;
  const unsigned per = slab < 256 ? 256 / slab : 1;
  const unsigned sub = per > 1 ? threadIdx.x / slab : 0;
  const unsigned e = per > 1 ? threadIdx.x - sub * slab : blockIdx.x * 256 + threadIdx.x;
  if (e >= slab || sub >= per) return;
  const unsigned i = e / inner, in_i = e - i * inner;
  int oo[4];
  float wt[4];
  lin_bwd_taps((int)i, n, no, oo, wt);
  const unsigned o0 = oo[0] * inner + in_i, o1 = oo[1] * inner + in_i, o2 = oo[2] * inner + in_i, o3 = oo[3] * inner + in_i;
  for (unsigned o = blockIdx.y * per + sub; o < outer; o += gridDim.y * per) {
    const float* __restrict__ p = dpi_at(in, (size_t)o * no * inner, ib);
    dpi_st(out, (size_t)o * slab + e, (wt[0] * dpi_ld(p, o0, ib) + wt[1] * dpi_ld(p, o1, ib)) + (wt[2] * dpi_ld(p, o2, ib) + wt[3] * dpi_ld(p, o3, ib)), ob);
  }
}

__global__ __launch_bounds__(256) void upsample_lin_bwd_w2_kernel(const float* __restrict__ in, float* __restrict__ out, size_t rows, int n) {
  const int half = n >> 1, no = 2 * n;
  const size_t total = rows * (size_t)half;
  for (size_t p = (size_t)blockIdx.x * 256 + threadIdx.x; p < total; p += (size_t)gridDim.x * 256) {
    const size_t r = p / half;
    const int i = 2 * (int)(p - r * half);
    const float* __restrict__ row = in + r * no;
    const float4 v = *reinterpret_cast<const float4*>(row + 2 * i);
    const float lo = row[i > 0 ? 2 * i - 1 : 0], hi = row[i + 1 < n - 1 ? 2 * i + 4 : 0];
    int o[4];
    float w0[4], w1[4];
    lin_bwd_taps(i, n, no, o, w0);
    lin_bwd_taps(i + 1, n, no, o, w1);
    float2 y;
    y.x = (w0[0] * lo + w0[1] * v.x) + (w0[2] * v.y + w0[3] * v.z);
    y.y = (w1[0] * v.y + w1[1] * v.z) + (w1[2] * v.w + w1[3] * hi);
    *reinterpret_cast<float2*>(out + r * n + i) = y;
  }
}

__global__ __launch_bounds__(256) void crop_copy_kernel(const float* __restrict__ x, int D, int H, int W, int od, int oh, int ow,
                                                        int Do, int Ho, int Wo, float* __restrict__ y, int adjoint) {
  const int c = blockIdx.y;
  const size_t V = (size_t)D * H * W, Vo = (size_t)Do * Ho * Wo;
  if (!adjoint) {
    for (size_t i = (size_t)blockIdx.x * 256 + threadIdx.x; i < Vo; i += (size_t)gridDim.x * 256) {
      const int w = i % Wo, h = (i / Wo) % Ho, d = i / ((size_t)Wo * Ho);
      y[(size_t)c * Vo + i] = x[(size_t)c * V + ((size_t)(d + od) * H + h + oh) * W + w + ow];
    }
  } else {
    for (size_t i = (size_t)blockIdx.x * 256 + threadIdx.x; i < V; i += (size_t)gridDim.x * 256) {
      const int w = i % W, h = (i / W) % H, d = i / ((size_t)W * H);
      const int cd = d - od, ch = h - oh, cw = w - ow;
      const bool in = cd >= 0 && cd < Do && ch >= 0 && ch < Ho && cw >= 0 && cw < Wo;
      y[(size_t)c * V + i] = in ? x[(size_t)c * Vo + ((size_t)cd * Ho + ch) * Wo + cw] : 0.f;
    }
  }
}

__global__ __launch_bounds__(256) void fir_axis0_kernel(const float* __restrict__ x, const float* __restrict__ taps, int K, int T, size_t S,
                                                        float* __restrict__ y) {
  const int c = blockIdx.y, p = K / 2;
  const size_t n = (size_t)T * S;
  for (size_t i = (size_t)blockIdx.x * 256 + threadIdx.x; i < n; i += (size_t)gridDim.x * 256) {
    const int t = (int)(i / S);
    const size_t s_ = i % S;
    float acc = 0.f;
    for (int k = 0; k < K; ++k) {
      const int tt = t + p - k;
      if (tt >= 0 && tt < T) acc = fmaf(taps[k], x[(size_t)c * n + (size_t)tt * S + s_], acc);
    }
    y[(size_t)c * n + i] = acc;
  }
}

__global__ __launch_bounds__(256) void axpy_kernel(float a, const float* __restrict__ x, size_t n, float* __restrict__ y) {
  for (size_t i = (size_t)blockIdx.x * 256 + threadIdx.x; i < n; i += (size_t)gridDim.x * 256) y[i] = fmaf(a, x[i], y[i]);
}

inline unsigned ew_blocks(size_t n_vec4_threads) {
  size_t b = cdivz(n_vec4_threads, 256);
  if (b > 4096) b = 4096;
  if (b < 1) b = 1;
  return (unsigned)b;
}

}

extern "C" int dpi_stat_blocks(int C, size_t V) {
  if (C <= 0 || V == 0) return 0;
  size_t n = cdivz(V, kStatSpan);
  if (n > kMaxStatBlocks) n = kMaxStatBlocks;
  return (int)n;
}

#define DPI_LAUNCH_FG(io, KERNEL, GRID, ST, ...)                                          \
  do {                                                                                    \
    if (DPI_FB(io)) {                                                                     \
      if (DPI_GB(io)) KERNEL<true, true><<<GRID, 256, 0, ST>>>(__VA_ARGS__);              \
      else KERNEL<true, false><<<GRID, 256, 0, ST>>>(__VA_ARGS__);                        \
    } else {                                                                              \
      if (DPI_GB(io)) KERNEL<false, true><<<GRID, 256, 0, ST>>>(__VA_ARGS__);             \
      else KERNEL<false, false><<<GRID, 256, 0, ST>>>(__VA_ARGS__);                       \
    }                                                                                     \
  } while (0)
#define DPI_FB(io) (((io) & DPI_STORE_FWD_BF16) != 0)
#define DPI_GB(io) (((io) & DPI_STORE_GRAD_BF16) != 0)
#define DPI_REQUIRE_IO(io, what) DPI_REQUIRE(((io) & ~3u) == 0, what ": unknown storage-type bits in io = %u", (unsigned)(io))

extern "C" int dpi_channel_stats_io(const float* x, const float* chain, int C, size_t V, double* partials, unsigned io, void* stream) {
  DPI_REQUIRE(x && partials && C > 0 && V > 0, "channel_stats: bad argument");
  DPI_REQUIRE_IO(io, "channel_stats");
  const int nblk = dpi_stat_blocks(C, V);
  if (DPI_FB(io)) channel_stats_kernel<true><<<dim3(nblk, C), 256, 0, (hipStream_t)stream>>>(x, chain, C, V, nblk, partials);
  else channel_stats_kernel<false><<<dim3(nblk, C), 256, 0, (hipStream_t)stream>>>(x, chain, C, V, nblk, partials);
  return dpi_check_launch("channel_stats");
}
extern "C" int dpi_channel_stats(const float* x, const float* chain, int C, size_t V, double* partials, void* stream) {
  return dpi_channel_stats_io(x, chain, C, V, partials, 0, stream);
}

extern "C" int dpi_bn_finalize(const double* partials, int nblk, int C, size_t count, const float* gamma, const float* beta,
                               float eps, float momentum, float slope, int act_first, const float* in_chain, float* running_mean,
                               float* running_var, int64_t* num_batches_tracked, float* mean_invstd, float* chain_out,
                               void* stream) {
  DPI_REQUIRE(partials && nblk > 0 && C > 0 && count > 0, "bn_finalize: bad argument");
  DPI_REQUIRE(!in_chain || (slope == 1.f && !act_first), "bn_finalize: a composed input chain excludes a fused activation");
  bn_finalize_kernel<<<C, 256, 0, (hipStream_t)stream>>>(partials, nblk, C, (double)count, gamma, beta, eps, momentum, slope, act_first,
                                                        in_chain, running_mean, running_var, num_batches_tracked, mean_invstd, chain_out);
  return dpi_check_launch("bn_finalize");
}

extern "C" int dpi_chain_apply_io(const float* x, const float* chain, int C, size_t V, float* y, unsigned io, void* stream) {
  DPI_REQUIRE(x && y && C > 0 && V > 0, "chain_apply: bad argument");
  DPI_REQUIRE_IO(io, "chain_apply");
  if (DPI_FB(io)) chain_apply_kernel<true, true><<<dim3(ew_blocks(cdivz(V, 4)), C), 256, 0, (hipStream_t)stream>>>(x, chain, V, y);
  else chain_apply_kernel<false, false><<<dim3(ew_blocks(cdivz(V, 4)), C), 256, 0, (hipStream_t)stream>>>(x, chain, V, y);
  return dpi_check_launch("chain_apply");
}
extern "C" int dpi_chain_apply(const float* x, const float* chain, int C, size_t V, float* y, void* stream) {
  return dpi_chain_apply_io(x, chain, C, V, y, 0, stream);
}

extern "C" int dpi_bn_bwd_reduce(const float* dy, const float* x, const float* mean_invstd, const float* gamma, const float* beta,
                                 const float* in_chain, float pre_slope, float post_slope, int C, size_t V, double* partials,
                                 void* stream) {
  return dpi_bn_bwd_reduce_io(dy, x, mean_invstd, gamma, beta, in_chain, pre_slope, post_slope, C, V, partials, 0, stream);
}
extern "C" int dpi_bn_bwd_reduce_io(const float* dy, const float* x, const float* mean_invstd, const float* gamma, const float* beta,
                                    const float* in_chain, float pre_slope, float post_slope, int C, size_t V, double* partials,
                                    unsigned io, void* stream) {
  DPI_REQUIRE(dy && x && mean_invstd && partials && C > 0 && V > 0, "bn_bwd_reduce: bad argument");
  DPI_REQUIRE_IO(io, "bn_bwd_reduce");
  DPI_REQUIRE(!in_chain || pre_slope == 1.f, "bn_bwd_reduce: in_chain excludes pre_slope");
  const int nblk = dpi_stat_blocks(C, V);
  DPI_LAUNCH_FG(io, bn_bwd_reduce_kernel, dim3(nblk, C), (hipStream_t)stream, dy, x, mean_invstd, gamma, beta, in_chain, pre_slope, post_slope, C, V,
                nblk, partials);
  return dpi_check_launch("bn_bwd_reduce");
}

extern "C" int dpi_bn_bwd_apply(const float* dy, const float* x, const float* mean_invstd, const float* gamma, const float* beta,
                                const float* in_chain, float pre_slope, float post_slope, const double* partials, int nblk, int C,
                                size_t V, float* dx, float* dgamma, float* dbeta, void* stream) {
  return dpi_bn_bwd_apply_io(dy, x, mean_invstd, gamma, beta, in_chain, pre_slope, post_slope, partials, nblk, C, V, dx, dgamma, dbeta, 0, stream);
}
extern "C" int dpi_bn_bwd_apply_io(const float* dy, const float* x, const float* mean_invstd, const float* gamma, const float* beta,
                                   const float* in_chain, float pre_slope, float post_slope, const double* partials, int nblk, int C,
                                   size_t V, float* dx, float* dgamma, float* dbeta, unsigned io, void* stream) {
  DPI_REQUIRE(dy && x && mean_invstd && partials && dx && C > 0 && V > 0 && nblk > 0, "bn_bwd_apply: bad argument");
  DPI_REQUIRE_IO(io, "bn_bwd_apply");
  DPI_REQUIRE(!in_chain || pre_slope == 1.f, "bn_bwd_apply: in_chain excludes pre_slope");
  unsigned gx = ew_blocks(cdivz(V, 4 * 8));
  DPI_LAUNCH_FG(io, bn_bwd_apply_kernel, dim3(gx, C), (hipStream_t)stream, dy, x, mean_invstd, gamma, beta, in_chain, pre_slope, post_slope, partials, nblk,
                C, V, dx, dgamma, dbeta);
  return dpi_check_launch("bn_bwd_apply");
}

extern "C" int dpi_bn_bwd_apply_fork(const float* dy, const float* x, const float* mean_invstd, const float* gamma, const float* beta,
                                     const float* in_chain, float pre_slope, float post_slope, const double* partials, int nblk, int C,
                                     size_t V, float* dx, float* dgamma, float* dbeta, const float* xa, const float* mi_a,
                                     const float* gamma_a, const float* beta_a, const float* chain_a, float post_a, double* partials_a,
                                     const float* xb, const float* mi_b, const float* gamma_b, const float* beta_b, const float* chain_b,
                                     float post_b, double* partials_b, void* stream) {
  return dpi_bn_bwd_apply_fork_io(dy, x, mean_invstd, gamma, beta, in_chain, pre_slope, post_slope, partials, nblk, C, V, dx, dgamma, dbeta,
                                  xa, mi_a, gamma_a, beta_a, chain_a, post_a, partials_a, xb, mi_b, gamma_b, beta_b, chain_b, post_b, partials_b, 0,
                                  stream);
}
extern "C" int dpi_bn_bwd_apply_fork_io(const float* dy, const float* x, const float* mean_invstd, const float* gamma, const float* beta,
                                        const float* in_chain, float pre_slope, float post_slope, const double* partials, int nblk, int C,
                                        size_t V, float* dx, float* dgamma, float* dbeta, const float* xa, const float* mi_a,
                                        const float* gamma_a, const float* beta_a, const float* chain_a, float post_a, double* partials_a,
                                        const float* xb, const float* mi_b, const float* gamma_b, const float* beta_b, const float* chain_b,
                                        float post_b, double* partials_b, unsigned io, void* stream) {
  DPI_REQUIRE(dy && x && mean_invstd && partials && dx && C > 0 && V > 0 && nblk > 0, "bn_bwd_apply_fork: bad argument");
  DPI_REQUIRE_IO(io, "bn_bwd_apply_fork");
  DPI_REQUIRE(!in_chain || pre_slope == 1.f, "bn_bwd_apply_fork: in_chain excludes pre_slope");
  DPI_REQUIRE((!xa || (mi_a && partials_a)) && (!xb || (mi_b && partials_b)), "bn_bwd_apply_fork: incomplete follow-up BatchNorm");
  const int nb = dpi_stat_blocks(C, V);
  const BnFork fa{xa, mi_a, gamma_a, beta_a, chain_a, post_a, partials_a}, fb{xb, mi_b, gamma_b, beta_b, chain_b, post_b, partials_b};
  DPI_LAUNCH_FG(io, bn_bwd_apply_fork_kernel, dim3(nb, C), (hipStream_t)stream, dy, x, mean_invstd, gamma, beta, in_chain, pre_slope, post_slope,
                partials, nblk, C, V, nb, dx, dgamma, dbeta, fa, fb);
  return dpi_check_launch("bn_bwd_apply_fork");
}

extern "C" int dpi_bn_bwd_apply_dual(const float* dy, int nblk, int C, size_t V, const float* xa, const float* mi_a, const float* gamma_a,
                                     const float* beta_a, const float* chain_a, float post_a, const double* partials_a, float* dxa,
                                     float* dgamma_a, float* dbeta_a, const float* xb, const float* mi_b, const float* gamma_b,
                                     const float* beta_b, const float* chain_b, float post_b, const double* partials_b, float* dxb,
                                     float* dgamma_b, float* dbeta_b, int f_lo, int f_hi, const float* f_mi, const float* f_gamma,
                                     const float* f_beta, float f_post, double* f_partials, void* stream) {
  return dpi_bn_bwd_apply_dual_io(dy, nblk, C, V, xa, mi_a, gamma_a, beta_a, chain_a, post_a, partials_a, dxa, dgamma_a, dbeta_a, xb, mi_b, gamma_b,
                                  beta_b, chain_b, post_b, partials_b, dxb, dgamma_b, dbeta_b, f_lo, f_hi, f_mi, f_gamma, f_beta, f_post, f_partials, 0,
                                  stream);
}
extern "C" int dpi_bn_bwd_apply_dual_io(const float* dy, int nblk, int C, size_t V, const float* xa, const float* mi_a, const float* gamma_a,
                                        const float* beta_a, const float* chain_a, float post_a, const double* partials_a, float* dxa,
                                        float* dgamma_a, float* dbeta_a, const float* xb, const float* mi_b, const float* gamma_b,
                                        const float* beta_b, const float* chain_b, float post_b, const double* partials_b, float* dxb,
                                        float* dgamma_b, float* dbeta_b, int f_lo, int f_hi, const float* f_mi, const float* f_gamma,
                                        const float* f_beta, float f_post, double* f_partials, unsigned io, void* stream) {
  DPI_REQUIRE(dy && xa && xb && mi_a && mi_b && partials_a && partials_b && dxa && dxb && C > 0 && V > 0 && nblk > 0,
              "bn_bwd_apply_dual: bad argument");
  DPI_REQUIRE_IO(io, "bn_bwd_apply_dual");
  DPI_REQUIRE(!f_partials || (f_mi && f_lo >= 0 && f_hi <= C && f_lo < f_hi), "bn_bwd_apply_dual: bad fork range");
  const int nb = dpi_stat_blocks(C, V);
  const BnSide A{xa, mi_a, gamma_a, beta_a, chain_a, post_a, partials_a, dxa, dgamma_a, dbeta_a};
  const BnSide B{xb, mi_b, gamma_b, beta_b, chain_b, post_b, partials_b, dxb, dgamma_b, dbeta_b};
  DPI_LAUNCH_FG(io, bn_bwd_apply_dual_kernel, dim3(nb, C), (hipStream_t)stream, dy, A, B, nblk, C, V, nb, f_lo, f_hi, f_mi, f_gamma, f_beta, f_post,
                f_partials);
  return dpi_check_launch("bn_bwd_apply_dual");
}

static int join_blocks(int C, size_t V) { return dpi_stat_blocks(C, V); }
extern "C" size_t dpi_join_bwd_ws_doubles(int C, size_t V) { return (size_t)join_blocks(C, V) * (size_t)C * kJoinSums; }
extern "C" int dpi_join_bwd(const float* dy, const float* t, const float* mi, const float* gamma, const float* beta, float pre, int C, size_t V,
                            const float* xa, const float* mi_a, const float* gamma_a, const float* beta_a, const float* chain_a, float post_a,
                            const float* xb, const float* mi_b, const float* gamma_b, const float* beta_b, const float* chain_b, float post_b,
                            const float* fwd_chain_a, const float* fwd_chain_b,
                            int f_lo, int f_hi, const float* f_mi, const float* f_gamma, const float* f_beta, float f_post,
                            double* ws, float* coef, float* dxa, float* dxb, float* dxf, float* dgb, float* dgb_f, unsigned io, void* stream) {
  DPI_REQUIRE(dy && mi && xa && xb && mi_a && mi_b && ws && coef && dxa && dxb && dgb && C > 0 && V > 0, "join_bwd: bad argument");
  DPI_REQUIRE_IO(io, "join_bwd");
  DPI_REQUIRE(t || (fwd_chain_a && fwd_chain_b), "join_bwd: without t the two forward chains that form it are needed");
  DPI_REQUIRE(f_lo >= 0 && f_hi <= C && f_lo <= f_hi, "join_bwd: bad fork range");
  DPI_REQUIRE(f_lo == f_hi || (f_mi && dxf && dgb_f), "join_bwd: the fork range needs its BatchNorm's statistics and outputs");
  const int nblk = join_blocks(C, V);
  const JoinSide A{xa, mi_a, gamma_a, beta_a, chain_a, post_a, fwd_chain_a}, B{xb, mi_b, gamma_b, beta_b, chain_b, post_b, fwd_chain_b};
  const JoinFork F{f_lo, f_hi, f_mi, f_gamma, f_beta, f_post};
  hipStream_t st = (hipStream_t)stream;
  DPI_LAUNCH_FG(io, join_bwd_sums_kernel, dim3(nblk, C), st, dy, t, mi, gamma, beta, pre, A, B, F, C, V, nblk, ws);
  join_bwd_coef_kernel<<<C, 64, 0, st>>>(ws, nblk, C, (double)V, mi_b, gamma_b, f_lo, f_hi, coef, dgb, dgb_f);
  DPI_LAUNCH_FG(io, join_bwd_apply_kernel, dim3(ew_blocks(cdivz(V, 4 * 8)), C), st, dy, t, mi, gamma, beta, pre, A, B, F, coef, C, V, dxa, dxb, dxf);
  return dpi_check_launch("join_bwd");
}

extern "C" int dpi_chain_add_stats(const float* a, const float* chain_a, const float* b, const float* chain_b, int C, size_t V,
                                   float slope, float* t, double* partials, void* stream) {
  return dpi_chain_add_stats_io(a, chain_a, b, chain_b, C, V, slope, t, partials, 0, stream);
}
extern "C" int dpi_chain_add_stats_io(const float* a, const float* chain_a, const float* b, const float* chain_b, int C, size_t V,
                                      float slope, float* t, double* partials, unsigned io, void* stream) {
  DPI_REQUIRE(a && b && partials && C > 0 && V > 0, "chain_add_stats: bad argument");
  DPI_REQUIRE_IO(io, "chain_add_stats");
  const int nblk = dpi_stat_blocks(C, V);
  if (DPI_FB(io)) chain_add_stats_kernel<true><<<dim3(nblk, C), 256, 0, (hipStream_t)stream>>>(a, chain_a, b, chain_b, C, V, nblk, slope, t, partials);
  else chain_add_stats_kernel<false><<<dim3(nblk, C), 256, 0, (hipStream_t)stream>>>(a, chain_a, b, chain_b, C, V, nblk, slope, t, partials);
  return dpi_check_launch("chain_add_stats");
}

extern "C" int dpi_chain_add_apply(const float* a, const float* chain_a, const float* b, const float* chain_b, const float* chain_out, int C,
                                   size_t V, float* y, unsigned io, void* stream) {
  DPI_REQUIRE(a && b && y && C > 0 && V > 0, "chain_add_apply: bad argument");
  DPI_REQUIRE_IO(io, "chain_add_apply");
  if (DPI_FB(io)) chain_add_apply_kernel<true><<<dim3(ew_blocks(cdivz(V, 4)), C), 256, 0, (hipStream_t)stream>>>(a, chain_a, b, chain_b, chain_out, V, y);
  else chain_add_apply_kernel<false><<<dim3(ew_blocks(cdivz(V, 4)), C), 256, 0, (hipStream_t)stream>>>(a, chain_a, b, chain_b, chain_out, V, y);
  return dpi_check_launch("chain_add_apply");
}

extern "C" int dpi_lrelu_bwd(const float* dy, const float* x, float slope, size_t n, float* dx, void* stream) {
  DPI_REQUIRE(dy && x && dx && n > 0, "lrelu_bwd: bad argument");
  lrelu_bwd_kernel<<<ew_blocks(cdivz(n, 4)), 256, 0, (hipStream_t)stream>>>(dy, x, slope, n, dx);
  return dpi_check_launch("lrelu_bwd");
}

extern "C" int dpi_act_fwd(const float* x, size_t n, int kind, float* y, void* stream) {
  DPI_REQUIRE(x && y && n > 0 && kind >= DPI_ACT_ELU && kind <= DPI_ACT_SIGMOID, "act_fwd: bad argument");
  act_fwd_kernel<<<ew_blocks(cdivz(n, 4)), 256, 0, (hipStream_t)stream>>>(x, n, kind, y);
  return dpi_check_launch("act_fwd");
}

extern "C" int dpi_act_bwd(const float* dy, const float* y, size_t n, int kind, float* dx, void* stream) {
  DPI_REQUIRE(dy && y && dx && n > 0 && kind >= DPI_ACT_ELU && kind <= DPI_ACT_SIGMOID, "act_bwd: bad argument");
  act_bwd_kernel<<<ew_blocks(cdivz(n, 4)), 256, 0, (hipStream_t)stream>>>(dy, y, n, kind, dx);
  return dpi_check_launch("act_bwd");
}

extern "C" int dpi_add(const float* a, const float* b, size_t n, float* y, void* stream) {
  DPI_REQUIRE(a && b && y && n > 0, "add: bad argument");
  add_kernel<<<ew_blocks(cdivz(n, 4)), 256, 0, (hipStream_t)stream>>>(a, b, n, y);
  return dpi_check_launch("add");
}

extern "C" int dpi_channel_sum(const float* x, int C, size_t V, double* ws, float* out, void* stream) {
  DPI_REQUIRE(x && ws && out && C > 0 && V > 0, "channel_sum: bad argument");
  const int nblk = dpi_stat_blocks(C, V);
  channel_stats_kernel<false><<<dim3(nblk, C), 256, 0, (hipStream_t)stream>>>(x, nullptr, C, V, nblk, ws);
  if (int e = dpi_check_launch("channel_sum.stats")) return e;
  channel_sum_final_kernel<<<C, 64, 0, (hipStream_t)stream>>>(ws, nblk, C, out);
  return dpi_check_launch("channel_sum.final");
}

extern "C" int dpi_upsample2x_fwd(const float* x, const float* chain, int C, int D, int H, int W, int Do, int Ho, int Wo,
                                  int linear, float* y, void* stream) {
  return dpi_upsample2x_fwd_io(x, chain, C, D, H, W, Do, Ho, Wo, linear, y, 0, stream);
}
extern "C" int dpi_upsample2x_fwd_io(const float* x, const float* chain, int C, int D, int H, int W, int Do, int Ho, int Wo,
                                     int linear, float* y, unsigned io, void* stream) {
  DPI_REQUIRE(x && y && C > 0 && D > 0 && H > 0 && W > 0, "upsample_fwd: bad argument");
  DPI_REQUIRE_IO(io, "upsample_fwd");
  const bool fb = DPI_FB(io);
  const int scale_d = !(D == 1 && Do == 1);
  DPI_REQUIRE(Do >= 1 && Ho >= 1 && Wo >= 1 && Do <= (scale_d ? 2 * D : 1) && Ho <= 2 * H && Wo <= 2 * W,
              "upsample_fwd: output (%d,%d,%d) exceeds 2x input (%d,%d,%d)", Do, Ho, Wo, D, H, W);
  const size_t Vo = (size_t)Do * Ho * Wo, V = (size_t)D * H * W;
  if (linear && H > 1 && W > 1 && (!scale_d || D > 1)) {
    if (scale_d) {
      if (fb) upsample_lin_fwd_cube_kernel<true, true, true><<<dim3(ew_blocks(V), C), 256, 0, (hipStream_t)stream>>>(x, chain, D, H, W, Do, Ho, Wo, y);
      else upsample_lin_fwd_cube_kernel<true, false, false><<<dim3(ew_blocks(V), C), 256, 0, (hipStream_t)stream>>>(x, chain, D, H, W, Do, Ho, Wo, y);
    } else {
      if (fb) upsample_lin_fwd_cube_kernel<false, true, true><<<dim3(ew_blocks(V), C), 256, 0, (hipStream_t)stream>>>(x, chain, D, H, W, Do, Ho, Wo, y);
      else upsample_lin_fwd_cube_kernel<false, false, false><<<dim3(ew_blocks(V), C), 256, 0, (hipStream_t)stream>>>(x, chain, D, H, W, Do, Ho, Wo, y);
    }
    return dpi_check_launch("upsample_lin_fwd_cube");
  }
  if (fb) upsample_fwd_kernel<true, true><<<dim3(ew_blocks(Vo), C), 256, 0, (hipStream_t)stream>>>(x, chain, D, H, W, Do, Ho, Wo, linear, scale_d, y);
  else upsample_fwd_kernel<false, false><<<dim3(ew_blocks(Vo), C), 256, 0, (hipStream_t)stream>>>(x, chain, D, H, W, Do, Ho, Wo, linear, scale_d, y);
  return dpi_check_launch("upsample_fwd");
}

extern "C" size_t dpi_upsample2x_bwd_ws_floats(int C, int D, int H, int W, int Do, int Ho, int Wo, int linear) {
  if (!linear || C <= 0) return 0;
  const int scale_d = !(D == 1 && Do == 1);
  return (size_t)C * Do * Ho * W + (scale_d ? (size_t)C * Do * H * W : 0);
}

extern "C" int dpi_upsample2x_bwd(const float* dy, int C, int D, int H, int W, int Do, int Ho, int Wo, int linear, float* dx,
                                  float* ws, void* stream) {
  return dpi_upsample2x_bwd_io(dy, C, D, H, W, Do, Ho, Wo, linear, dx, ws, 0, stream);
}
extern "C" int dpi_upsample2x_bwd_io(const float* dy, int C, int D, int H, int W, int Do, int Ho, int Wo, int linear, float* dx,
                                     float* ws, unsigned io, void* stream) {
  DPI_REQUIRE(dy && dx && C > 0 && D > 0 && H > 0 && W > 0, "upsample_bwd: bad argument");
  DPI_REQUIRE_IO(io, "upsample_bwd");
  const bool gb = DPI_GB(io);
  const int scale_d = !(D == 1 && Do == 1);
  const size_t V = (size_t)D * H * W;
  if (linear && ws) {
    hipStream_t st = (hipStream_t)stream;
    float* t1 = ws;
    float* t2 = ws + (size_t)C * Do * Ho * W;
    DPI_REQUIRE((size_t)C * Do * Ho < (1ull << 32) && (size_t)Do * Ho * Wo < (1ull << 31) && (size_t)Do * H * W < (1ull << 31),
                "upsample_bwd: %d x %d x %d x %d exceeds the 32-bit slab indexing of the separable adjoint", C, Do, Ho, Wo);
    auto launch = [&](const float* src, float* dst, size_t outer, int n, int no, size_t inner, bool ib, bool ob) {
      const unsigned gx = (unsigned)cdivz((size_t)n * inner, 256);
      size_t gy = outer < 65535 ? outer : 65535;
      while (gy > 1 && (size_t)gx * gy > 16384) gy = (gy + 1) / 2;
      const dim3 g(gx, (unsigned)gy);
      if (ib && ob) upsample_lin_bwd_axis_kernel<true, true><<<g, 256, 0, st>>>(src, dst, (unsigned)outer, n, no, (unsigned)inner);
      else if (ib) upsample_lin_bwd_axis_kernel<true, false><<<g, 256, 0, st>>>(src, dst, (unsigned)outer, n, no, (unsigned)inner);
      else if (ob) upsample_lin_bwd_axis_kernel<false, true><<<g, 256, 0, st>>>(src, dst, (unsigned)outer, n, no, (unsigned)inner);
      else upsample_lin_bwd_axis_kernel<false, false><<<g, 256, 0, st>>>(src, dst, (unsigned)outer, n, no, (unsigned)inner);
    };
    static const bool w2 = getenv("DPI_NO_UPW2") == nullptr;
    if (w2 && !gb && Wo == 2 * W && (W & 1) == 0 && (Wo & 3) == 0 && (((uintptr_t)dy | (uintptr_t)t1) & 15) == 0) {
      const size_t rows = (size_t)C * Do * Ho, pairs = rows * (size_t)(W / 2);
      upsample_lin_bwd_w2_kernel<<<ew_blocks(cdivz(pairs, 1)), 256, 0, st>>>(dy, t1, rows, W);
    } else
    launch(dy, t1, (size_t)C * Do * Ho, W, Wo, 1, gb, false);
    launch(t1, scale_d ? t2 : dx, (size_t)C * Do, H, Ho, W, false, scale_d ? false : gb);
    if (scale_d) launch(t2, dx, C, D, Do, (size_t)H * W, false, gb);
    return dpi_check_launch("upsample_lin_bwd_axis");
  }
  if (linear) {
    if (scale_d) {
      if (gb) upsample_lin_bwd_gather_kernel<true, true><<<dim3(ew_blocks(V), C), 256, 0, (hipStream_t)stream>>>(dy, D, H, W, Do, Ho, Wo, dx);
      else upsample_lin_bwd_gather_kernel<true, false><<<dim3(ew_blocks(V), C), 256, 0, (hipStream_t)stream>>>(dy, D, H, W, Do, Ho, Wo, dx);
    } else {
      if (gb) upsample_lin_bwd_gather_kernel<false, true><<<dim3(ew_blocks(V), C), 256, 0, (hipStream_t)stream>>>(dy, D, H, W, Do, Ho, Wo, dx);
      else upsample_lin_bwd_gather_kernel<false, false><<<dim3(ew_blocks(V), C), 256, 0, (hipStream_t)stream>>>(dy, D, H, W, Do, Ho, Wo, dx);
    }
    return dpi_check_launch("upsample_lin_bwd_gather");
  }
  if (gb) upsample_bwd_kernel<true><<<dim3(ew_blocks(V), C), 256, 0, (hipStream_t)stream>>>(dy, D, H, W, Do, Ho, Wo, linear, scale_d, dx);
  else upsample_bwd_kernel<false><<<dim3(ew_blocks(V), C), 256, 0, (hipStream_t)stream>>>(dy, D, H, W, Do, Ho, Wo, linear, scale_d, dx);
  return dpi_check_launch("upsample_bwd");
}

extern "C" int dpi_crop_copy(const float* x, int C, int D, int H, int W, int od, int oh, int ow, int Do, int Ho, int Wo, float* y,
                             void* stream) {
  DPI_REQUIRE(x && y && od >= 0 && oh >= 0 && ow >= 0 && od + Do <= D && oh + Ho <= H && ow + Wo <= W, "crop_copy: bad window");
  crop_copy_kernel<<<dim3(ew_blocks((size_t)Do * Ho * Wo), C), 256, 0, (hipStream_t)stream>>>(x, D, H, W, od, oh, ow, Do, Ho, Wo,
                                                                                            y, 0);
  return dpi_check_launch("crop_copy");
}

extern "C" int dpi_crop_copy_bwd(const float* dy, int C, int D, int H, int W, int od, int oh, int ow, int Do, int Ho, int Wo,
                                 float* dx, void* stream) {
  DPI_REQUIRE(dy && dx && od >= 0 && oh >= 0 && ow >= 0 && od + Do <= D && oh + Ho <= H && ow + Wo <= W, "crop_copy_bwd: bad window");
  crop_copy_kernel<<<dim3(ew_blocks((size_t)D * H * W), C), 256, 0, (hipStream_t)stream>>>(dy, D, H, W, od, oh, ow, Do, Ho, Wo, dx,
                                                                                         1);
  return dpi_check_launch("crop_copy_bwd");
}

extern "C" int dpi_fir_axis0(const float* x, const float* taps, int K, int C, int T, size_t S, float* y, void* stream) {
  DPI_REQUIRE(x && taps && y && K > 0 && (K & 1) && C > 0 && T > 0 && S > 0, "fir_axis0: bad argument (odd tap count required)");
  fir_axis0_kernel<<<dim3(ew_blocks((size_t)T * S), C), 256, 0, (hipStream_t)stream>>>(x, taps, K, T, S, y);
  return dpi_check_launch("fir_axis0");
}

extern "C" int dpi_axpy(float a, const float* x, size_t n, float* y, void* stream) {
  DPI_REQUIRE(x && y && n > 0, "axpy: bad argument");
  axpy_kernel<<<ew_blocks(n), 256, 0, (hipStream_t)stream>>>(a, x, n, y);
  return dpi_check_launch("axpy");
}
```

deep_prior_interpolation_amd/ops.py:

```python
import ctypes as C
import os
import threading

import torch

from . import _lib
from ._lib import ConvDesc, check, ptr, stream

BN_EPS = 1e-5
BN_MOMENTUM = 0.1


def _req(t, name, act=False):
    if not t.is_cuda:
        raise _lib.DpiError("%s must live on the GPU: the HIP path has no CPU fallback" % name)
    if t.dtype != torch.float32 and not (act and t.dtype == torch.bfloat16):
        raise _lib.DpiError("%s must be float32%s (got %s)" % (name, " or bfloat16" if act else "", t.dtype))
    return t.contiguous()


STORAGE_BF16 = os.environ.get("DPI_STORAGE", "fp32") == "bf16"
_tls = threading.local()


# ... 76 lines not shown
    global PRECISION
    if name not in _PRECISIONS:
        raise ValueError("precision must be one of %s" % sorted(_PRECISIONS))
    PRECISION = _PRECISIONS[name]


def make_desc(x, w, stride, ydt=torch.float32):
    Cin, D, H, W = _dims(x)
    k = w.shape[-1]
    kd = w.shape[2] if w.ndim == 5 else 1
    if w.shape[1] != Cin:
        raise _lib.DpiError("conv: weight expects %d input channels, tensor has %d" % (w.shape[1], Cin))
    io = ((_lib.IO_X_BF16 | _lib.IO_DX_BF16) if _bf(x) else 0) | ((_lib.IO_Y_BF16 | _lib.IO_DY_BF16) if ydt == torch.bfloat16 else 0)
    return ConvDesc(Cin, w.shape[0], D, H, W, k, kd, int(stride), precision(), io)


def desc_out_dims(d):
    sd = d.stride if d.kd > 1 else 1
    return conv_out(d.D, d.kd, sd), conv_out(d.H, d.k, d.stride), conv_out(d.W, d.k, d.stride)


class KernelTimer:

    def __init__(self, match):
        self.match = match
        self.events = []

    def durations(self):
        return [a.elapsed_time(b) for _, a, b in self.events]

    def by_key(self):
        out = {}
        for key, a, b in self.events:
            out.setdefault(key, []).append(a.elapsed_time(b))
        return out


_timer = None


def set_timer(t):
    global _timer
    _timer = t


_PROFILE_TAGS = os.environ.get("DPI_PROFILE_TAGS")
_tag_ids = {}


def _tag_id(kind, d):
    key = "%s %d->%d k%d%s s%d @%dx%dx%d" % (kind, d.Cin, d.Cout, d.k, " (2-D)" if d.D == 1 else "", d.stride, d.D, d.H, d.W)
    i = _tag_ids.get(key)
    if i is None:
        i = len(_tag_ids) + 2
        _tag_ids[key] = i
    return i


if _PROFILE_TAGS:
    import atexit
    import json

    def _dump_tags():
        with open(_PROFILE_TAGS, "w") as fp:
            json.dump({str(i): k for k, i in _tag_ids.items()}, fp, indent=0)
    atexit.register(_dump_tags)


def _timed(kind, d, launch):
    if _PROFILE_TAGS:
        L = _lib.load()
        L.dpi_profile_marker(_tag_id(kind, d), stream())
        launch()
        L.dpi_profile_marker(1, stream())
        return
    key = _timer.match(kind, d) if _timer is not None else None
    if key:
        e0, e1 = torch.cuda.Event(enable_timing=True), torch.cuda.Event(enable_timing=True)
        e0.record()
        launch()
        e1.record()
        _timer.events.append((key, e0, e1))
    else:
        launch()


_ws_cache = {}


def _ws_floats(kind, d):
    key = (kind, d.Cin, d.Cout, d.D, d.H, d.W, d.k, d.kd, d.stride, d.precision, d.io)
    n = _ws_cache.get(key)
    if n is None:
        L = _lib.load()
        n = {"fwd": L.dpi_conv_fwd_ws_floats, "bwd_data": L.dpi_conv_bwd_data_ws_floats}[kind](C.byref(d))
        _ws_cache[key] = n
    return n


def reset_ws_cache():
    _ws_cache.clear()


def _conv_ws(n, like):
    return torch.empty(n, dtype=torch.float32, device=like.device) if n else None


def raw_conv_fwd(d, x, chain, w, bias, y, partials=None):
    L = _lib.load()
    n = _ws_floats("fwd", d)
    ws = _conv_ws(n, x)
    _timed("conv_fwd", d, lambda: check(L.dpi_conv_fwd_ws(C.byref(d), ptr(x), ptr(chain), ptr(w), ptr(bias), ptr(y),
                                                          ptr(partials), ptr(ws), n, stream()), "dpi_conv_fwd"))


def raw_conv_bwd_data(d, dy, w, dx, accumulate=False):
    L = _lib.load()
    n = _ws_floats("bwd_data", d)
    ws = _conv_ws(n, dy)
    _timed("conv_bwd_data", d, lambda: check(L.dpi_conv_bwd_data_ws(C.byref(d), ptr(dy), ptr(w), ptr(dx), int(accumulate),
                                                                    ptr(ws), n, stream()), "dpi_conv_bwd_data"))


def raw_conv_bwd_data_dual(d3, dy3, w3, d1, dy1, w1, dx, accumulate=False):
    L = _lib.load()
    n = _ws_floats("bwd_data", d3)
    ws = _conv_ws(n, dy3)

    def launch():
        check(L.dpi_conv_bwd_data_dual(C.byref(d3), ptr(dy3), ptr(w3), C.byref(d1), ptr(dy1), ptr(w1), ptr(dx), int(accumulate),
                                       ptr(ws), n, stream()), "dpi_conv_bwd_data_dual")
    _timed("conv_bwd_data", d3, launch)


OVERLAP_WEIGHT_GRADS = os.environ.get("DPI_OVERLAP_WGRAD", "0") == "1"
OVERLAP_IN_GRAPH = os.environ.get("DPI_OVERLAP_IN_GRAPH", "0") == "1"
OVERLAP_MAX_VOXELS = int(os.environ.get("DPI_OVERLAP_MAX_VOXELS", str(1 << 40)))


def set_weight_grad_overlap(on, in_graph=None):
    global OVERLAP_WEIGHT_GRADS, OVERLAP_IN_GRAPH
    if "DPI_OVERLAP_WGRAD" not in os.environ:
        OVERLAP_WEIGHT_GRADS = bool(on)
    if in_graph is not None and "DPI_OVERLAP_IN_GRAPH" not in os.environ:
        OVERLAP_IN_GRAPH = bool(in_graph)
_side_streams = {}
N_SIDE_STREAMS = int(os.environ.get("DPI_SIDE_STREAMS", "2"))
_side_rr = [0]
_side_used = set()
JOIN_AT = os.environ.get("DPI_JOIN_AT", "step")
_side_keep = []
_in_iteration = [False]
_deferred = []


def begin_iteration():
    _side_rr[0] = 0
    _in_iteration[0] = True
    del _deferred[:]


def abort_iteration():
    try:
        if torch.cuda.is_available():
            join_weight_grads(final=True)
            join_branch()
    finally:
        _in_iteration[0] = False
        _side_used.clear()
        del _side_keep[:]
        del _deferred[:]
        _branch_open[0] = False


def _defer(*tensors):
    if JOIN_AT == "step" and _in_iteration[0]:
        _deferred.extend(t.data_ptr() for t in tensors if t is not None)


def _side_stream():
    dev = torch.cuda.current_device()
    sts = _side_streams.get(dev)
    if sts is None:
        sts = [torch.cuda.Stream(device=dev) for _ in range(max(N_SIDE_STREAMS, 1))]
        _side_streams[dev] = sts
    i = _side_rr[0] % len(sts)
    _side_rr[0] += 1
    _side_used.add(i)
    return sts[i]


def conv_bwd_weight_async(d, x, chain, dy, dw):
    if not OVERLAP_WEIGHT_GRADS or d.D * d.H * d.W >= OVERLAP_MAX_VOXELS or (torch.cuda.is_current_stream_capturing() and not OVERLAP_IN_GRAPH):
        return raw_conv_bwd_weight(d, x, chain, dy, dw)
    side = _side_stream()
    side.wait_stream(torch.cuda.current_stream())
    with torch.cuda.stream(side):
        raw_conv_bwd_weight(d, x, chain, dy, dw)
    if JOIN_AT == "step" and _in_iteration[0]:
        _side_keep.append((x, chain, dy))
        _deferred.append(dw.data_ptr())


def join_weight_grads(final=False):
    if JOIN_AT == "step" and _in_iteration[0] and not final:
        return
    if _side_used:
        sts = _side_streams.get(torch.cuda.current_device()) or []
        for i in sorted(_side_used):
            torch.cuda.current_stream().wait_stream(sts[i])
        _side_used.clear()
    _side_keep.clear()


def finish_backward(params=None):
    join_weight_grads(final=True)
    join_branch()
    _in_iteration[0] = False
    if _deferred and params is not None:
        have = {p.grad.data_ptr() for p in params if p.grad is not None}
        lost = [q for q in _deferred if q not in have]
        if lost:
            n = len(_deferred)
            del _deferred[:]
            raise _lib.DpiError("%d of %d gradients written on a side / branch stream were copied or accumulated by autograd before that stream ran "
                                "(zero_grad(set_to_none=False), a gradient hook, retain_grad or a shared parameter?): with the once-per-step join "
                                "(DPI_JOIN_AT=step) .grad must be None when backward starts; use DPI_JOIN_AT=node otherwise" % (len(lost), n))
    del _deferred[:]


BRANCH_STREAMS = os.environ.get("DPI_BRANCH", "1") == "1"
BRANCH_SHORTCUT = int(os.environ.get("DPI_BRANCH_SHORT", "0"))
BRANCH_SKIP = os.environ.get("DPI_BRANCH_SKIP", "1") == "1"
BRANCH_SKIP_BWD = os.environ.get("DPI_BRANCH_SKIP_BWD", "1") == "1"
_branch_streams = {}
_branch_open = [False]


def branch_on():
    return (BRANCH_STREAMS and OVERLAP_WEIGHT_GRADS and _in_iteration[0] and JOIN_AT == "step"
            and not torch.cuda.is_current_stream_capturing())


def _branch_stream(kind="skip"):
    key = (torch.cuda.current_device(), kind)
    st = _branch_streams.get(key)
    if st is None:
        st = torch.cuda.Stream(device=key[0])
        _branch_streams[key] = st
    return st


class _Branch:

    def __init__(self, kind, *tensors):
        self.st = _branch_stream(kind)
        self.tensors = tensors

    def __enter__(self):
        self.st.wait_stream(torch.cuda.current_stream())
        for t in self.tensors:
            if t is not None:
                t.record_stream(self.st)
        self.ctx = torch.cuda.stream(self.st)
        self.ctx.__enter__()
        _branch_open[0] = True
        return self

    def __exit__(self, *exc):
        return self.ctx.__exit__(*exc)


def join_branch(kind=None):
    if not _branch_open[0]:
        return
    dev = torch.cuda.current_device()
    for (d, k), st in _branch_streams.items():
        if d == dev and (kind is None or k == kind):
            torch.cuda.current_stream().wait_stream(st)
    if kind is None:
        _branch_open[0] = False


def raw_conv_bwd_weight(d, x, chain, dy, dw):
    L = _lib.load()
    n = L.dpi_conv_bwd_weight_ws_floats(C.byref(d))
    ws = torch.empty(n, dtype=torch.float32, device=x.device)
    _timed("conv_bwd_weight", d, lambda: check(L.dpi_conv_bwd_weight(C.byref(d), ptr(x), ptr(chain), ptr(dy), ptr(dw),
                                                                     ptr(ws), n, stream()), "dpi_conv_bwd_weight"))


def raw_channel_sum(x, C_, V, out):
    L = _lib.load()
    nblk = L.dpi_stat_blocks(C_, V)
    ws = torch.empty(nblk * C_ * 2, dtype=torch.float64, device=x.device)
    check(L.dpi_channel_sum(ptr(x), C_, V, ptr(ws), ptr(out), stream()), "dpi_channel_sum")


def raw_bn_stats_finalize(x, chain_in, C_, V, gamma, beta, slope, running_mean, running_var, nbt, mean_invstd, chain_out,
                          eps=BN_EPS, momentum=BN_MOMENTUM, act_first=0, compose=False):
    L = _lib.load()
    nblk = L.dpi_stat_blocks(C_, V)
    part = torch.empty(nblk * C_ * 2, dtype=torch.float64, device=x.device)
    check(L.dpi_channel_stats_io(ptr(x), ptr(chain_in), C_, V, ptr(part), _io(x), stream()), "dpi_channel_stats")
    check(L.dpi_bn_finalize(ptr(part), nblk, C_, V, ptr(gamma), ptr(beta), eps, momentum, slope, act_first,
                            ptr(chain_in) if compose else None, ptr(running_mean), ptr(running_var), ptr(nbt), ptr(mean_invstd),
                            ptr(chain_out), stream()), "dpi_bn_finalize")


def raw_bn_finalize(part, nblk, C_, count, gamma, beta, slope, running_mean, running_var, nbt, mean_invstd, chain_out,
                    eps=BN_EPS, momentum=BN_MOMENTUM, act_first=0):
    L = _lib.load()
    check(L.dpi_bn_finalize(ptr(part), nblk, C_, count, ptr(gamma), ptr(beta), eps, momentum, slope, act_first, None,
                            ptr(running_mean), ptr(running_var), ptr(nbt), ptr(mean_invstd), ptr(chain_out), stream()),
          "dpi_bn_finalize")


def raw_upsample2x_bwd(dy, C_, D, H, W, Do, Ho, Wo, linear, dx):
    L = _lib.load()
    n = L.dpi_upsample2x_bwd_ws_floats(C_, D, H, W, Do, Ho, Wo, linear)
    ws = torch.empty(n, dtype=torch.float32, device=dy.device) if n else None
    _same_type(dy, dx, "upsample2x_bwd")
    check(L.dpi_upsample2x_bwd_io(ptr(dy), C_, D, H, W, Do, Ho, Wo, linear, ptr(dx), ptr(ws), _io(None, dy), stream()), "dpi_upsample2x_bwd")


def raw_chain_apply(x, chain, C_, V, y):
    L = _lib.load()
    _same_type(x, y, "chain_apply")
    check(L.dpi_chain_apply_io(ptr(x), ptr(chain), C_, V, ptr(y), _io(x), stream()), "dpi_chain_apply")


_slope_chains = {}


def slope_chain(C_, slope, device):
    key = (C_, float(slope), str(device))
    t = _slope_chains.get(key)
    if t is None:
        t = torch.tensor([1.0, 0.0, slope, 1.0, 0.0], dtype=torch.float32).repeat(C_, 1).to(device).contiguous()
        _slope_chains[key] = t
    return t


class ConvFn(torch.autograd.Function):

    @staticmethod
    def forward(ctx, x, w, b, stride):
        x, w = _req(x, "conv input", act=True), _req(w, "conv weight")
        b = _req(b, "conv bias") if b is not None else None
        d = make_desc(x, w, stride)
        Do, Ho, Wo = desc_out_dims(d)
        y = torch.empty(_like_spatial(x, d.Cout, Do, Ho, Wo), dtype=torch.float32, device=x.device)
        raw_conv_fwd(d, x, None, w, b, y)
        ctx.save_for_backward(x, w)
        ctx.d = d
        ctx.has_bias = b is not None
        return y

    @staticmethod
    def backward(ctx, dy):
        x, w = ctx.saved_tensors
        d = ctx.d
        dy = _req(dy, "conv grad")
        dx = dw = db = None
        if ctx.needs_input_grad[1]:
            dw = torch.empty_like(w)
            conv_bwd_weight_async(d, x, None, dy, dw)
        if ctx.needs_input_grad[0]:
            dx = torch.empty_like(x)
            raw_conv_bwd_data(d, dy, w, dx)
        if ctx.has_bias and ctx.needs_input_grad[2]:
            db = torch.empty(d.Cout, dtype=torch.float32, device=x.device)
            raw_channel_sum(dy, d.Cout, dy.numel() // d.Cout, db)
        join_weight_grads()
        return dx, dw, db, None


def _bn_backward(dy, x, mi, gamma, beta, pre_slope, post_slope, in_chain=None, dx=None):
    L = _lib.load()
    C_ = x.shape[1]
    V = x.numel() // C_
    nblk = L.dpi_stat_blocks(C_, V)
    part = torch.empty(nblk * C_ * 2, dtype=torch.float64, device=x.device)
    io = _io(x, dy)
    check(L.dpi_bn_bwd_reduce_io(ptr(dy), ptr(x), ptr(mi), ptr(gamma), ptr(beta), ptr(in_chain), pre_slope, post_slope, C_, V,
                                 ptr(part), io, stream()), "dpi_bn_bwd_reduce")
    if dx is None:
        dx = torch.empty_like(dy)
    _same_type(dy, dx, "bn_backward")
    dgamma = torch.empty_like(gamma)
    dbeta = torch.empty_like(gamma)
    check(L.dpi_bn_bwd_apply_io(ptr(dy), ptr(x), ptr(mi), ptr(gamma), ptr(beta), ptr(in_chain), pre_slope, post_slope, ptr(part), nblk,
                                C_, V, ptr(dx), ptr(dgamma), ptr(dbeta), io, stream()), "dpi_bn_bwd_apply")
    return dx, dgamma, dbeta


def _bn_backward_fork(dy, x, mi, gamma, beta, pre_slope, post_slope, forks):
    L = _lib.load()
    C_ = x.shape[1]
    V = x.numel() // C_
    nblk = L.dpi_stat_blocks(C_, V)
    part = torch.empty(nblk * C_ * 2, dtype=torch.float64, device=x.device)
    io = _io(x, dy)
    check(L.dpi_bn_bwd_reduce_io(ptr(dy), ptr(x), ptr(mi), ptr(gamma), ptr(beta), None, pre_slope, post_slope, C_, V, ptr(part),
                                 io, stream()), "dpi_bn_bwd_reduce")
    dx = torch.empty_like(dy)
    dgamma, dbeta = torch.empty_like(gamma), torch.empty_like(gamma)
    fparts = [torch.empty(nblk * C_ * 2, dtype=torch.float64, device=x.device) for _ in forks]
    fa = []
    for k in range(2):
        if k < len(forks):
            xk, mik, gk, ek, chk, postk = forks[k]
            _same_type(x, xk, "bn_backward_fork")
            fa += [ptr(xk), ptr(mik), ptr(gk), ptr(ek), ptr(chk), postk, ptr(fparts[k])]
        else:
            fa += [None, None, None, None, None, 1.0, None]
    check(L.dpi_bn_bwd_apply_fork_io(ptr(dy), ptr(x), ptr(mi), ptr(gamma), ptr(beta), None, pre_slope, post_slope, ptr(part), nblk, C_, V,
                                     ptr(dx), ptr(dgamma), ptr(dbeta), *fa, io, stream()), "dpi_bn_bwd_apply_fork")
    return dx, dgamma, dbeta, [(nblk, fp) for fp in fparts]


def _bn_backward_apply(dy, x, mi, gamma, beta, pre_slope, post_slope, red, in_chain=None, dx=None):
    L = _lib.load()
    C_ = x.shape[1]
    V = x.numel() // C_
    nblk, part = red
    if dx is None:
        dx = torch.empty_like(dy)
    _same_type(dy, dx, "bn_backward_apply")
    dgamma, dbeta = torch.empty_like(gamma), torch.empty_like(gamma)
    check(L.dpi_bn_bwd_apply_io(ptr(dy), ptr(x), ptr(mi), ptr(gamma), ptr(beta), ptr(in_chain), pre_slope, post_slope, ptr(part), nblk,
                                C_, V, ptr(dx), ptr(dgamma), ptr(dbeta), _io(x, dy), stream()), "dpi_bn_bwd_apply")
    return dx, dgamma, dbeta


def _bn_backward_apply_dual(dy, side_a, side_b, fork=None):
    L = _lib.load()
    xa, mia, ga, ea, cha, posta, (nblk, parta) = side_a
    xb, mib, gb, eb, chb, postb, (nblk_b, partb) = side_b
    assert nblk == nblk_b
    C_ = xa.shape[1]
    V = xa.numel() // C_
    _same_type(xa, xb, "bn_backward_apply_dual")
    dxa, dxb = torch.empty_like(dy), torch.empty_like(dy)
    dga, dea, dgb, deb = (torch.empty_like(g) for g in (ga, ga, gb, gb))
    red_f = None
    fargs = [0, 0, None, None, None, 1.0, None]
    if fork is not None:
        lo, hi, mif, gf, ef, postf = fork
        nb = L.dpi_stat_blocks(C_, V)
        pf = torch.empty(nb * (hi - lo) * 2, dtype=torch.float64, device=xa.device)
        fargs = [lo, hi, ptr(mif), ptr(gf), ptr(ef), postf, ptr(pf)]
        red_f = (nb, pf)
    check(L.dpi_bn_bwd_apply_dual_io(ptr(dy), nblk, C_, V,
                                     ptr(xa), ptr(mia), ptr(ga), ptr(ea), ptr(cha), posta, ptr(parta), ptr(dxa), ptr(dga), ptr(dea),
                                     ptr(xb), ptr(mib), ptr(gb), ptr(eb), ptr(chb), postb, ptr(partb), ptr(dxb), ptr(dgb), ptr(deb),
                                     *fargs, _io(xa, dy), stream()), "dpi_bn_bwd_apply_dual")
    return (dxa, dga, dea), (dxb, dgb, deb), red_f


JOIN_BWD_FUSED = os.environ.get("DPI_JOIN_BWD", "1") == "1"
EARLY_SHORTCUT_WGRAD = os.environ.get("DPI_EARLY_SHORTCUT_WGRAD", "0") == "1"


def _join_backward(dy, t, mi, gamma, beta, pre_slope, side_a, side_b, fork=None, fwd_chains=None):
    L = _lib.load()
    xa, mia, ga, ea, cha, posta = side_a
    xb, mib, gb, eb, chb, postb = side_b
    C_ = dy.shape[1]
    V = dy.numel() // C_
    dev = dy.device
    fwa, fwb = fwd_chains if fwd_chains is not None else (None, None)
    ws = torch.empty(L.dpi_join_bwd_ws_doubles(C_, V), dtype=torch.float64, device=dev)
    coef = torch.empty(C_ * 8, dtype=torch.float32, device=dev)
    dgb = torch.empty((6, C_), dtype=torch.float32, device=dev)
    dxa, dxb = torch.empty_like(dy), torch.empty_like(dy)
    if fork is not None:
        lo, hi, mif, gf, ef, postf, dxf = fork
        dgbf = torch.empty((2, hi - lo), dtype=torch.float32, device=dev)
        fa = [lo, hi, ptr(mif), ptr(gf), ptr(ef), postf]
    else:
        dxf = dgbf = None
        fa = [0, 0, None, None, None, 1.0]
    check(L.dpi_join_bwd(ptr(dy), ptr(t), ptr(mi), ptr(gamma), ptr(beta), pre_slope, C_, V,
                         ptr(xa), ptr(mia), ptr(ga), ptr(ea), ptr(cha), posta, ptr(xb), ptr(mib), ptr(gb), ptr(eb), ptr(chb), postb,
                         ptr(fwa), ptr(fwb), *fa, ptr(ws), ptr(coef), ptr(dxa), ptr(dxb), ptr(dxf), ptr(dgb), ptr(dgbf), _io(xa, dy), stream()),
          "dpi_join_bwd")
    f = None if dgbf is None else (dgbf[0], dgbf[1])
    return (dxa, dgb[2], dgb[3]), (dxb, dgb[4], dgb[5]), (dgb[0], dgb[1]), f


def _join_fused_ok(*tensors):
    return JOIN_BWD_FUSED and (all(x.dtype == torch.float32 for x in tensors) or all(x.dtype == torch.bfloat16 for x in tensors))


def _join_forward(a, ch_a, b, ch_b, C_, V, slope, bn, gamma, beta, mi_out, y, keep_t):
    L = _lib.load()
    dev = a.device
    t = torch.empty_like(a) if keep_t else None
    nblk = L.dpi_stat_blocks(C_, V)
    part = torch.empty(nblk * C_ * 2, dtype=torch.float64, device=dev)
    check(L.dpi_chain_add_stats_io(ptr(a), ptr(ch_a), ptr(b), ptr(ch_b), C_, V, slope, ptr(t), ptr(part), _io(a), stream()),
          "dpi_chain_add_stats")
    ch_out = torch.empty(C_ * 5, dtype=torch.float32, device=dev)
    raw_bn_finalize(part, nblk, C_, V, gamma, beta, slope, bn.running_mean, bn.running_var, bn.num_batches_tracked, mi_out, ch_out,
                    act_first=1)
    if keep_t:
        raw_chain_apply(t, ch_out, C_, V, y)
    else:
        check(L.dpi_chain_add_apply(ptr(a), ptr(ch_a), ptr(b), ptr(ch_b), ptr(ch_out), C_, V, ptr(y), _io(a), stream()), "dpi_chain_add_apply")
    return t


def _pre_chain(C_, pre_slope, device):
    return None if pre_slope == 1.0 else slope_chain(C_, pre_slope, device)


class BatchNormFn(torch.autograd.Function):

    @staticmethod
    def forward(ctx, x, gamma, beta, running_mean, running_var, nbt, post_slope, pre_slope=1.0):
        x = _req(x, "batchnorm input")
        C_ = x.shape[1]
        V = x.numel() // C_
        mi = torch.empty(2 * C_, dtype=torch.float32, device=x.device)
        chain = torch.empty(C_ * 5, dtype=torch.float32, device=x.device)
        if pre_slope != 1.0 and post_slope != 1.0:
            raise _lib.DpiError("batch_norm: pre and post activation cannot both be fused")
        raw_bn_stats_finalize(x, _pre_chain(C_, pre_slope, x.device), C_, V, gamma, beta,
                              pre_slope if pre_slope != 1.0 else post_slope, running_mean, running_var, nbt, mi, chain,
                              act_first=int(pre_slope != 1.0))
        y = torch.empty_like(x)
        raw_chain_apply(x, chain, C_, V, y)
        ctx.save_for_backward(x, gamma, beta, mi)
        ctx.slopes = (float(pre_slope), float(post_slope))
        return y

    @staticmethod
    def backward(ctx, dy):
        x, gamma, beta, mi = ctx.saved_tensors
        dx, dgamma, dbeta = _bn_backward(_req(dy, "batchnorm grad"), x, mi, gamma, beta, *ctx.slopes)
        return dx, dgamma, dbeta, None, None, None, None, None


FAN_IN = os.environ.get("DPI_FAN_IN", "1") == "1"


class FanIn:
    __slots__ = ("dx", "branched")

    def __init__(self):
        self.dx = None
        self.branched = False


class ConvBnActFn(torch.autograd.Function):

    @staticmethod
    def forward(ctx, x, w, b, gamma, beta, running_mean, running_var, nbt, stride, slope, fan=None):
        x, w = _req(x, "conv input", act=True), _req(w, "conv weight")
        ctx.fan = fan
        adt = act_dtype() if x.ndim == 5 else torch.float32
        if x.ndim != 5 and _bf(x):
            raise _lib.DpiError("conv_bn_act: bf16 storage is built for the 3-D nets only")
        d = make_desc(x, w, stride, adt)
        Do, Ho, Wo = desc_out_dims(d)
        L = _lib.load()
        r = torch.empty(_like_spatial(x, d.Cout, Do, Ho, Wo), dtype=adt, device=x.device)
        nblk = L.dpi_conv_fwd_stat_blocks(C.byref(d))
        part = torch.empty(nblk * d.Cout * 2, dtype=torch.float64, device=x.device)
        raw_conv_fwd(d, x, None, w, b, r, part)
        V = Do * Ho * Wo
        mi = torch.empty(2 * d.Cout, dtype=torch.float32, device=x.device)
        chain = torch.empty(d.Cout * 5, dtype=torch.float32, device=x.device)
        raw_bn_finalize(part, nblk, d.Cout, V, gamma, beta, slope, running_mean, running_var, nbt, mi, chain)
        y = torch.empty_like(r)
        raw_chain_apply(r, chain, d.Cout, V, y)
        ctx.save_for_backward(x, w, r, gamma, beta, mi)
        ctx.d, ctx.slope, ctx.has_bias, ctx.bias_ref = d, float(slope), b is not None, b
        return y

    @staticmethod
    def backward(ctx, dy):
        x, w, r, gamma, beta, mi = ctx.saved_tensors
        d = ctx.d
        dr, dgamma, dbeta = _bn_backward(_req(dy, "conv-bn-act grad", act=True), r, mi, gamma, beta, 1.0, ctx.slope)
        dx = dw = db = None
        if ctx.needs_input_grad[1]:
            dw = torch.empty_like(w)
            conv_bwd_weight_async(d, x, None, dr, dw)
        if ctx.needs_input_grad[0]:
            fan = ctx.fan
            if fan is not None and fan.dx is not None and fan.dx.shape == x.shape and fan.dx.dtype == x.dtype:
                if fan.branched:
                    join_branch("skip")
                raw_conv_bwd_data(d, dr, w, fan.dx, accumulate=True)
                fan.dx = None
            else:
                dx = torch.empty_like(x)
                raw_conv_bwd_data(d, dr, w, dx)
        if ctx.has_bias and ctx.needs_input_grad[2]:
            db = _zeros_like_or_none(ctx.bias_ref, dr)
        join_weight_grads()
        return dx, dw, db, dgamma, dbeta, None, None, None, None, None, None


def _cba_raw(d, x, in_chain, w, b, bn, slope, r_out, mi_out, chain_out):
    L = _lib.load()
    nblk = L.dpi_conv_fwd_stat_blocks(C.byref(d))
    part = torch.empty(nblk * d.Cout * 2, dtype=torch.float64, device=x.device)
    raw_conv_fwd(d, x, in_chain, w, b, r_out, part)
    Do, Ho, Wo = desc_out_dims(d)
    raw_bn_finalize(part, nblk, d.Cout, Do * Ho * Wo, bn.weight, bn.bias, slope, bn.running_mean, bn.running_var,
                    bn.num_batches_tracked, mi_out, chain_out)


DEAD_BIAS = "off"


def _zeros_like_or_none(b, dr=None):
    if b is None or DEAD_BIAS == "off":
        return None
    if DEAD_BIAS == "noise":
        return torch.randn_like(b) * 1e-6
    return dr.sum(dim=[0] + list(range(2, dr.ndim)), dtype=torch.float32)


class Block3dFn(torch.autograd.Function):

    @staticmethod
    def forward(ctx, x, blk, slope, *p):
        x = _req(x, "block input", act=True)
        (w1, b1, g1, e1, w2, b2, g2, e2, w3, b3, g3, e3, ws, bs, gs, es, gA, eA, gB, eB) = p
        L = _lib.load()
        dev = x.device
        f32 = dict(dtype=torch.float32, device=dev)
        adt = act_dtype()
        c1, c2, c3 = w1.shape[0], w2.shape[0], w3.shape[0]
        Ct = c1 + c2 + c3
        bn1_, bn2_, bn3_, bns_ = (m._parts()[1] for m in (blk.conv3x3, blk.conv5x5, blk.conv7x7, blk.shortcut))
        d1 = make_desc(x, w1, 1, adt)
        Do, Ho, Wo = desc_out_dims(d1)
        V = Do * Ho * Wo
        R = torch.empty(_like_spatial(x, Ct, Do, Ho, Wo), dtype=adt, device=dev)
        CH = torch.empty(Ct * 5, **f32)
        r1, r2, r3 = R[:, :c1], R[:, c1:c1 + c2], R[:, c1 + c2:]
        ch1, ch2, ch3 = CH[:c1 * 5], CH[c1 * 5:(c1 + c2) * 5], CH[(c1 + c2) * 5:]
        mi1, mi2, mi3 = (torch.empty(2 * c, **f32) for c in (c1, c2, c3))
        miA, miS, miB = (torch.empty(2 * Ct, **f32) for _ in range(3))
        dsc = make_desc(x, ws, 1, adt)
        S = torch.empty_like(R)
        chSA = torch.empty((2, Ct * 5), **f32)
        chS, chA = chSA[0], chSA[1]
        side_shortcut = BRANCH_SHORTCUT if branch_on() else 0

        def shortcut_on_branch():
            with _Branch("short", x, S, miS, chS):
                _cba_raw(dsc, x, None, ws, bs, bns_, slope, S, miS, chS)
        if side_shortcut == 1:
            shortcut_on_branch()
        _cba_raw(d1, x, None, w1, b1, bn1_, slope, r1, mi1, ch1)
        if side_shortcut == 2:
            shortcut_on_branch()
        d2 = make_desc(r1, w2, 1, adt)
        _cba_raw(d2, r1, ch1, w2, b2, bn2_, slope, r2, mi2, ch2)
        d3 = make_desc(r2, w3, 1, adt)
        _cba_raw(d3, r2, ch2, w3, b3, bn3_, slope, r3, mi3, ch3)
        A = blk.bn1
        raw_bn_stats_finalize(R, CH, Ct, V, gA, eA, 1.0, A.running_mean, A.running_var, A.num_batches_tracked, miA, chA,
                              compose=True)
        if side_shortcut:
            join_branch("short")
        else:
            _cba_raw(dsc, x, None, ws, bs, bns_, slope, S, miS, chS)
        y = torch.empty_like(R)
        tless = _join_fused_ok(R, S)
        t = _join_forward(S, chS, R, chA, Ct, V, slope, blk.bn2, gB, eB, miB, y, keep_t=not tless)
        if tless:
            t = chSA
        ctx.tless = tless
        ctx.save_for_backward(x, R, S, t, CH, mi1, mi2, mi3, miA, miS, miB, *[q for q in p if q is not None])
        ctx.none_mask = [q is None for q in p]
        ctx.descs = (d1, d2, d3, dsc)
        ctx.slope = float(slope)
        ctx.split = (c1, c2, c3)
        return y

    @staticmethod
    def backward(ctx, dy):
        dy = _req(dy, "block grad", act=True)
        x, R, S, t, CH, mi1, mi2, mi3, miA, miS, miB = ctx.saved_tensors[:11]
        it = iter(ctx.saved_tensors[11:])
        p = [None if isnone else next(it) for isnone in ctx.none_mask]
        (w1, b1, g1, e1, w2, b2, g2, e2, w3, b3, g3, e3, ws, bs, gs, es, gA, eA, gB, eB) = p
        d1, d2, d3, dsc = ctx.descs
        slope = ctx.slope
        c1, c2, c3 = ctx.split
        s1, s2, s3 = slice(0, c1), slice(c1, c1 + c2), slice(c1 + c2, c1 + c2 + c3)
        ch1, ch2 = CH[:c1 * 5], CH[c1 * 5:(c1 + c2) * 5]
        dR = torch.empty_like(R)
        if ctx.tless or _join_fused_ok(dy, t, S, R):
            (dS, dgs, des), (dcat, dgA, deA), (dgB, deB), (dg3, de3) = _join_backward(
                dy, None if ctx.tless else t, miB, gB, eB, slope, (S, miS, gs, es, None, slope), (R, miA, gA, eA, CH, 1.0),
                fork=(c1 + c2, c1 + c2 + c3, mi3, g3, e3, slope, dR[:, s3]), fwd_chains=(t[0], t[1]) if ctx.tless else None)
        else:
            dt, dgB, deB, (redS, redA) = _bn_backward_fork(dy, t, miB, gB, eB, slope, 1.0,
                                                           [(S, miS, gs, es, None, slope), (R, miA, gA, eA, CH, 1.0)])
            (dS, dgs, des), (dcat, dgA, deA), red3 = _bn_backward_apply_dual(
                dt, (S, miS, gs, es, None, slope, redS), (R, miA, gA, eA, CH, 1.0, redA), fork=(c1 + c2, c1 + c2 + c3, mi3, g3, e3, slope))
            del dt
            _, dg3, de3 = _bn_backward_apply(dcat[:, s3], R[:, s3], mi3, g3, e3, 1.0, slope, red3, dx=dR[:, s3])
        dws = torch.empty_like(ws)
        if EARLY_SHORTCUT_WGRAD:
            conv_bwd_weight_async(dsc, x, None, dS, dws)
        dw3 = torch.empty_like(w3)
        conv_bwd_weight_async(d3, R[:, s2], ch2, dR[:, s3], dw3)
        raw_conv_bwd_data(d3, dR[:, s3], w3, dcat[:, s2], accumulate=True)
        _, dg2, de2 = _bn_backward(dcat[:, s2], R[:, s2], mi2, g2, e2, 1.0, slope, dx=dR[:, s2])
        dw2 = torch.empty_like(w2)
        conv_bwd_weight_async(d2, R[:, s1], ch1, dR[:, s2], dw2)
        raw_conv_bwd_data(d2, dR[:, s2], w2, dcat[:, s1], accumulate=True)
        _, dg1, de1 = _bn_backward(dcat[:, s1], R[:, s1], mi1, g1, e1, 1.0, slope, dx=dR[:, s1])
        dw1 = torch.empty_like(w1)
        conv_bwd_weight_async(d1, x, None, dR[:, s1], dw1)
        if not EARLY_SHORTCUT_WGRAD:
            conv_bwd_weight_async(dsc, x, None, dS, dws)
        dx = None
        if ctx.needs_input_grad[0]:
            dx = torch.empty_like(x)
            raw_conv_bwd_data_dual(d1, dR[:, s1], w1, dsc, dS, ws, dx)
        join_weight_grads()
        z = _zeros_like_or_none
        return (dx, None, None, dw1, z(b1, dR[:, s1]), dg1, de1, dw2, z(b2, dR[:, s2]), dg2, de2, dw3, z(b3, dR[:, s3]), dg3, de3,
                dws, z(bs, dS), dgs, des, dgA, deA, dgB, deB)


def _respath_bn_backward(dy, t, miB, gB, eB, slope, r3, mi3, g3, e3, r1, mi1, g1, e1, tless=False):
    if tless or _join_fused_ok(dy, t, r3, r1):
        a, b, top, _ = _join_backward(dy, None if tless else t, miB, gB, eB, slope, (r3, mi3, g3, e3, None, slope), (r1, mi1, g1, e1, None, slope),
                                      fwd_chains=(t[1], t[0]) if tless else None)
        return a, b, top
    dt, dgB, deB, (red3, red1) = _bn_backward_fork(dy, t, miB, gB, eB, slope, 1.0,
                                                   [(r3, mi3, g3, e3, None, slope), (r1, mi1, g1, e1, None, slope)])
    a, b, _ = _bn_backward_apply_dual(dt, (r3, mi3, g3, e3, None, slope, red3), (r1, mi1, g1, e1, None, slope, red1))
    return a, b, (dgB, deB)


class ResPath3dFn(torch.autograd.Function):

    @staticmethod
    def forward(ctx, x, rp, slope, *p):
        x = _req(x, "respath input", act=True)
        (w3, b3, g3, e3, w1, b1, g1, e1, gB, eB) = p
        L = _lib.load()
        f32 = dict(dtype=torch.float32, device=x.device)
        adt = act_dtype()
        Ct = w3.shape[0]
        bn3_, bn1_ = rp.conv3x3._parts()[1], rp.conv1x1._parts()[1]
        d3, d1 = make_desc(x, w3, 1, adt), make_desc(x, w1, 1, adt)
        Do, Ho, Wo = desc_out_dims(d3)
        V = Do * Ho * Wo
        r3 = torch.empty(_like_spatial(x, Ct, Do, Ho, Wo), dtype=adt, device=x.device)
        r1 = torch.empty_like(r3)
        mi3, mi1, miB = (torch.empty(2 * Ct, **f32) for _ in range(3))
        ch13 = torch.empty((2, 5 * Ct), **f32)
        ch1, ch3 = ch13[0], ch13[1]
        _cba_raw(d3, x, None, w3, b3, bn3_, slope, r3, mi3, ch3)
        _cba_raw(d1, x, None, w1, b1, bn1_, slope, r1, mi1, ch1)
        y = torch.empty_like(r3)
        tless = _join_fused_ok(r3, r1)
        t = _join_forward(r1, ch1, r3, ch3, Ct, V, slope, rp.bn, gB, eB, miB, y, keep_t=not tless)
        if tless:
            t = ch13
        ctx.tless = tless
        ctx.save_for_backward(x, r3, r1, t, mi3, mi1, miB, *[q for q in p if q is not None])
        ctx.none_mask = [q is None for q in p]
        ctx.descs = (d3, d1)
        ctx.slope = float(slope)
        return y

    @staticmethod
    def backward(ctx, dy):
        dy = _req(dy, "respath grad", act=True)
        x, r3, r1, t, mi3, mi1, miB = ctx.saved_tensors[:7]
        it = iter(ctx.saved_tensors[7:])
        (w3, b3, g3, e3, w1, b1, g1, e1, gB, eB) = [None if isnone else next(it) for isnone in ctx.none_mask]
        d3, d1 = ctx.descs
        slope = ctx.slope
        (dr3, dg3, de3), (dr1, dg1, de1), (dgB, deB) = _respath_bn_backward(dy, t, miB, gB, eB, slope, r3, mi3, g3, e3, r1, mi1, g1, e1, ctx.tless)
        dw3, dw1 = torch.empty_like(w3), torch.empty_like(w1)
        conv_bwd_weight_async(d3, x, None, dr3, dw3)
        conv_bwd_weight_async(d1, x, None, dr1, dw1)
        dx = None
        if ctx.needs_input_grad[0]:
            dx = torch.empty_like(x)
            raw_conv_bwd_data_dual(d3, dr3, w3, d1, dr1, w1, dx)
        join_weight_grads()
        z = _zeros_like_or_none
        return dx, None, None, dw3, z(b3, dr3), dg3, de3, dw1, z(b1, dr1), dg1, de1, dgB, deB


def _skip_alloc(x, p, Cd):
    (w3, b3, g3, e3, w1, b1, g1, e1, gB, eB) = p
    f32 = dict(dtype=torch.float32, device=x.device)
    adt = act_dtype()
    Cs = w3.shape[0]
    d3, d1 = make_desc(x, w3, 1, adt), make_desc(x, w1, 1, adt)
    Do, Ho, Wo = desc_out_dims(d3)
    T = dict(adt=adt, Cs=Cs, Cd=Cd, d3=d3, d1=d1, dims=(Do, Ho, Wo))
    T["r3"] = torch.empty(_like_spatial(x, Cs, Do, Ho, Wo), dtype=adt, device=x.device)
    T["r1"] = torch.empty_like(T["r3"])
    T["tless"] = _join_fused_ok(T["r3"])
    T["mi3"], T["mi1"], T["miB"] = (torch.empty(2 * Cs, **f32) for _ in range(3))
# ... 493 lines not shown
```

include/dpi_hip.h:

```cpp
#ifndef DPI_HIP_H
#define DPI_HIP_H

#include <stddef.h>
#include <stdint.h>

#ifdef __cplusplus
extern "C" {
#endif

#define DPI_OK 0
#define DPI_E_ARG (-1)
#define DPI_E_LAUNCH (-2)
#define DPI_E_WORKSPACE (-3)

#define DPI_CHAIN_STRIDE 5

const char* dpi_last_error(void);
int dpi_version(void);
int dpi_device_info(int device, int* cus, int* lds_bytes, size_t* hbm_bytes, char* name, int name_len);
int dpi_profile_marker(int id, void* stream);
int dpi_set_option(const char* key, int value);

typedef struct {
  int size;
  int Cin, Cout;
  int D, H, W;
  int k, kd;
  int stride;
  int precision;
  int io;
} dpi_conv_desc;
#define DPI_IO_X_BF16 1
#define DPI_IO_Y_BF16 2
#define DPI_IO_DY_BF16 4
#define DPI_IO_DX_BF16 8
int dpi_conv_desc_size(void);

int dpi_conv_fwd_stat_blocks(const dpi_conv_desc* d);
int dpi_conv_fwd(const dpi_conv_desc* d, const float* x, const float* x_chain, const float* w,
                 const float* bias, float* y, double* stat_partials, void* stream);
int dpi_conv_bwd_data(const dpi_conv_desc* d, const float* dy, const float* w, float* dx,
                      int accumulate, void* stream);
size_t dpi_conv_fwd_ws_floats(const dpi_conv_desc* d);
size_t dpi_conv_bwd_data_ws_floats(const dpi_conv_desc* d);
int dpi_conv_fwd_ws(const dpi_conv_desc* d, const float* x, const float* x_chain, const float* w,
                    const float* bias, float* y, double* stat_partials, float* ws, size_t ws_floats, void* stream);
int dpi_conv_bwd_data_ws(const dpi_conv_desc* d, const float* dy, const float* w, float* dx,
                         int accumulate, float* ws, size_t ws_floats, void* stream);
int dpi_conv_bwd_data_dual(const dpi_conv_desc* d3, const float* dy3, const float* w3,
                           const dpi_conv_desc* d1, const float* dy1, const float* w1,
                           float* dx, int accumulate, float* ws, size_t ws_floats, void* stream);
size_t dpi_conv_bwd_weight_ws_floats(const dpi_conv_desc* d);
int dpi_conv_bwd_weight(const dpi_conv_desc* d, const float* x, const float* x_chain, const float* dy,
                        float* dw, float* ws, size_t ws_floats, void* stream);


int dpi_stat_blocks(int C, size_t V);
int dpi_channel_stats(const float* x, const float* chain, int C, size_t V, double* partials, void* stream);
int dpi_bn_finalize(const double* partials, int nblk, int C, size_t count, const float* gamma,
                    const float* beta, float eps, float momentum, float slope, int act_first,
                    const float* in_chain, float* running_mean, float* running_var, int64_t* num_batches_tracked,
                    float* mean_invstd, float* chain_out, void* stream);
int dpi_chain_apply(const float* x, const float* chain, int C, size_t V, float* y, void* stream);
int dpi_bn_bwd_reduce(const float* dy, const float* x, const float* mean_invstd, const float* gamma,
                      const float* beta, const float* in_chain, float pre_slope, float post_slope, int C,
                      size_t V, double* partials, void* stream);
int dpi_bn_bwd_apply(const float* dy, const float* x, const float* mean_invstd, const float* gamma,
                     const float* beta, const float* in_chain, float pre_slope, float post_slope,
                     const double* partials, int nblk, int C, size_t V, float* dx, float* dgamma,
                     float* dbeta, void* stream);
int dpi_bn_bwd_apply_fork(const float* dy, const float* x, const float* mean_invstd, const float* gamma,
                          const float* beta, const float* in_chain, float pre_slope, float post_slope,
                          const double* partials, int nblk, int C, size_t V, float* dx, float* dgamma,
                          float* dbeta, const float* xa, const float* mi_a, const float* gamma_a,
                          const float* beta_a, const float* chain_a, float post_a, double* partials_a,
                          const float* xb, const float* mi_b, const float* gamma_b, const float* beta_b,
                          const float* chain_b, float post_b, double* partials_b, void* stream);
int dpi_bn_bwd_apply_dual(const float* dy, int nblk, int C, size_t V, const float* xa, const float* mi_a,
                          const float* gamma_a, const float* beta_a, const float* chain_a, float post_a,
                          const double* partials_a, float* dxa, float* dgamma_a, float* dbeta_a, const float* xb,
                          const float* mi_b, const float* gamma_b, const float* beta_b, const float* chain_b,
                          float post_b, const double* partials_b, float* dxb, float* dgamma_b, float* dbeta_b,
                          int f_lo, int f_hi, const float* f_mi, const float* f_gamma, const float* f_beta,
                          float f_post, double* f_partials, void* stream);
int dpi_chain_add_stats(const float* a, const float* chain_a, const float* b, const float* chain_b, int C,
                        size_t V, float slope, float* t, double* partials, void* stream);
int dpi_lrelu_bwd(const float* dy, const float* x, float slope, size_t n, float* dx, void* stream);
#define DPI_ACT_ELU 1
#define DPI_ACT_TANH 2
#define DPI_ACT_SIGMOID 3
int dpi_act_fwd(const float* x, size_t n, int kind, float* y, void* stream);
int dpi_act_bwd(const float* dy, const float* y, size_t n, int kind, float* dx, void* stream);
int dpi_add(const float* a, const float* b, size_t n, float* y, void* stream);
int dpi_channel_sum(const float* x, int C, size_t V, double* ws, float* out, void* stream);

#define DPI_STORE_FWD_BF16 1u
#define DPI_STORE_GRAD_BF16 2u
int dpi_channel_stats_io(const float* x , const float* chain, int C, size_t V, double* partials, unsigned io, void* stream);
int dpi_chain_apply_io(const float* x , const float* chain, int C, size_t V, float* y , unsigned io, void* stream);
int dpi_chain_add_stats_io(const float* a , const float* chain_a, const float* b , const float* chain_b, int C, size_t V,
                           float slope, float* t , double* partials, unsigned io, void* stream);
int dpi_bn_bwd_reduce_io(const float* dy , const float* x , const float* mean_invstd, const float* gamma, const float* beta,
                         const float* in_chain, float pre_slope, float post_slope, int C, size_t V, double* partials, unsigned io,
                         void* stream);
int dpi_bn_bwd_apply_io(const float* dy , const float* x , const float* mean_invstd, const float* gamma, const float* beta,
                        const float* in_chain, float pre_slope, float post_slope, const double* partials, int nblk, int C, size_t V,
                        float* dx , float* dgamma, float* dbeta, unsigned io, void* stream);
int dpi_bn_bwd_apply_fork_io(const float* dy , const float* x , const float* mean_invstd, const float* gamma, const float* beta,
                             const float* in_chain, float pre_slope, float post_slope, const double* partials, int nblk, int C,
                             size_t V, float* dx , float* dgamma, float* dbeta, const float* xa , const float* mi_a,
                             const float* gamma_a, const float* beta_a, const float* chain_a, float post_a, double* partials_a,
                             const float* xb , const float* mi_b, const float* gamma_b, const float* beta_b, const float* chain_b,
                             float post_b, double* partials_b, unsigned io, void* stream);
int dpi_bn_bwd_apply_dual_io(const float* dy , int nblk, int C, size_t V, const float* xa , const float* mi_a,
                             const float* gamma_a, const float* beta_a, const float* chain_a, float post_a,
                             const double* partials_a, float* dxa , float* dgamma_a, float* dbeta_a, const float* xb ,
                             const float* mi_b, const float* gamma_b, const float* beta_b, const float* chain_b,
                             float post_b, const double* partials_b, float* dxb , float* dgamma_b, float* dbeta_b,
                             int f_lo, int f_hi, const float* f_mi, const float* f_gamma, const float* f_beta,
                             float f_post, double* f_partials, unsigned io, void* stream);
int dpi_upsample2x_fwd_io(const float* x , const float* chain, int C, int D, int H, int W, int Do, int Ho, int Wo, int linear,
                          float* y , unsigned io, void* stream);
int dpi_upsample2x_bwd_io(const float* dy , int C, int D, int H, int W, int Do, int Ho, int Wo, int linear, float* dx ,
                          float* ws, unsigned io, void* stream);
int dpi_noise_add_io(const float* z, size_t n, float std, uint64_t seed, const uint64_t* step_ptr, float* out , unsigned io,
                     void* stream);

int dpi_upsample2x_fwd(const float* x, const float* chain, int C, int D, int H, int W, int Do, int Ho,
                       int Wo, int linear, float* y, void* stream);
size_t dpi_upsample2x_bwd_ws_floats(int C, int D, int H, int W, int Do, int Ho, int Wo, int linear);
int dpi_upsample2x_bwd(const float* dy, int C, int D, int H, int W, int Do, int Ho, int Wo, int linear,
                       float* dx, float* ws, void* stream);
int dpi_crop_copy(const float* x, int C, int D, int H, int W, int od, int oh, int ow, int Do, int Ho,
                  int Wo, float* y, void* stream);
int dpi_crop_copy_bwd(const float* dy, int C, int D, int H, int W, int od, int oh, int ow, int Do,
                      int Ho, int Wo, float* dx, void* stream);

int dpi_maxpool2x2_fwd(const float* x, int C, int H, int W, float* y, void* stream);
int dpi_maxpool2x2_bwd(const float* dy, const float* x, int C, int H, int W, float* dx, void* stream);
int dpi_deconv4x4s2_fwd(const float* x, const float* w, const float* bias, int Cin, int Cout, int H, int W,
                        float* y, void* stream);
int dpi_deconv4x4s2_bwd_data(const float* dy, const float* w, int Cin, int Cout, int H, int W, float* dx,
                             void* stream);
int dpi_deconv4x4s2_bwd_weight(const float* x, const float* dy, int Cin, int Cout, int H, int W, float* dw,
                               void* stream);

size_t dpi_loss_ws_doubles(size_t n);
int dpi_masked_loss(const float* out, const float* img, const float* mask, size_t n, int kind,
                    float grad_scale, float* dout, double* ws, double* result, void* stream);
int dpi_masked_loss_holdout(const float* out, const float* img, const float* mask, const float* sel, int C, int T, size_t S,
                            int kind, float grad_scale, float* dout, double* ws, double* result, void* stream);

int dpi_ema_loss(const float* out, float* avg, const float* img, const float* mask, const float* sel, int C, int T, size_t S,
                 int kind, float beta, const float* step_lr, const int* active, double* ws, double* result, void* stream);

typedef struct { float* p; const float* g; float* m; float* v; } dpi_adam_tensor;
int dpi_adam_multi(const dpi_adam_tensor* tensors, const int64_t* sizes, int ntensors,
                   const float* step_lr, double beta1, double beta2, double eps, const int* active,
                   void* stream);
int dpi_langevin_multi(const dpi_adam_tensor* tensors, const int64_t* sizes, int ntensors, const float* step_lr, int kind,
                       double weight_decay, double beta, double lambda, double noise_scale, double temperature, uint64_t seed,
                       const float* const* xi, const int* active, void* stream);
int dpi_moments_update(const float* out, float* mean, float* m2, size_t n, const float* step_lr, int burn_in, int thin,
                       const int* active, void* stream);

int dpi_loop_control(const double* metrics, double* state, double* hist, int max_iters, float* step_lr,
                     int* active, int* improved, int use_plateau, double factor, double threshold,
                     int patience, double min_lr, double lr_eps, int es_patience, double es_min_delta,
                     void* stream);
int dpi_loop_control_holdout(const double* metrics, double* state, double* hist, int max_iters, float* step_lr,
                             int* active, int* improved, int use_plateau, double factor, double threshold,
                             int patience, double min_lr, double lr_eps, int es_patience, double es_min_delta,
                             void* stream);
int dpi_loop_control_ema(const double* metrics, const double* ema_metrics, int has_holdout, double* state, double* hist,
                         int max_iters, float* step_lr, int* active, int* improved, int use_plateau, double factor,
                         double threshold, int patience, double min_lr, double lr_eps, int es_patience, double es_min_delta,
                         void* stream);
int dpi_copy_if(const int* flag, const float* src, float* dst, size_t n, void* stream);

int dpi_noise_add(const float* z, size_t n, float std, uint64_t seed, const uint64_t* step_ptr,
                  float* out, void* stream);
int dpi_fill_normal(float* out, size_t n, float mean, float std, uint64_t seed, uint64_t stream_id,
                    void* stream);
int dpi_noise_add_regen_io(size_t n, float z_std, uint64_t z_seed, uint64_t z_stream_id, float std, uint64_t seed,
                           const uint64_t* step_ptr, float* out , unsigned io, void* stream);
int dpi_fir_axis0(const float* x, const float* taps, int K, int C, int T, size_t S, float* y, void* stream);
int dpi_axpy(float a, const float* x, size_t n, float* y, void* stream);

int dpi_overlap_add(const float* patch, int pd, int ph, int pw, int od, int oh, int ow, float* acc,
                    int D, int H, int W, void* stream);
int dpi_overlap_normalize(float* acc, int D, int H, int W, int pd, int ph, int pw, int sd, int sh,
                          int sw, float gain, void* stream);
int dpi_overlap_add_weighted(const float* mean, const float* std , int pd, int ph, int pw, int od, int oh, int ow,
                             const float* ramp_d, int ld, const float* ramp_h, int lh, const float* ramp_w, int lw, unsigned sides,
                             float* acc, int K, int D, int H, int W, void* stream);
int dpi_overlap_finalize_weighted(const float* acc, int K, int D, int H, int W, float gain, float* out_mean, float* out_std ,
                                  void* stream);

int dpi_diff_axis(const float* x, size_t outer, int n, size_t inner, int stencil, float spacing, int adjoint, float* y,
                  void* stream);
int dpi_hale2d(const float* x, const float* a, const float* b, const float* c, size_t N, int H, int W, int adjoint, float* y,
               void* stream);
int dpi_structure_tensor(const float* x, size_t N, int H, int W, float dv, float dh, float* gvv, float* gvh, float* ghh,
                         void* stream);
int dpi_dips(const float* gvv, const float* gvh, const float* ghh, size_t n, float* phi, float* anisotropy, void* stream);
int dpi_hale_sections(const float* x, const float* coef, int C, int T, int X, int Y, int adjoint, float* y, void* stream);
int dpi_structure_tensor_sections(const float* x, int C, int T, int X, int Y, float dt, float dx, float dy, float* gtt, float* gtx,
                                  float* gxx, float* gty, float* gyy, void* stream);

size_t dpi_max_ws_floats(size_t n);
int dpi_scaled_max(const float* x, size_t n, float scale, float* ws, float* out, void* stream);
int dpi_threshold(const float* x, size_t n, const float* thresh, float* y, void* stream);
int dpi_pocs_project(const float* x, const float* wdata, const float* wmask, size_t n, float* y, void* stream);

size_t dpi_join_bwd_ws_doubles(int C, size_t V);
int dpi_join_bwd(const float* dy, const float* t, const float* mi, const float* gamma, const float* beta, float pre, int C, size_t V,
                 const float* xa, const float* mi_a, const float* gamma_a, const float* beta_a, const float* chain_a, float post_a,
                 const float* xb, const float* mi_b, const float* gamma_b, const float* beta_b, const float* chain_b, float post_b,
                 const float* fwd_chain_a, const float* fwd_chain_b,
                 int f_lo, int f_hi, const float* f_mi, const float* f_gamma, const float* f_beta, float f_post,
                 double* ws, float* coef, float* dxa, float* dxb, float* dxf, float* dgb, float* dgb_f, unsigned io, void* stream);
int dpi_chain_add_apply(const float* a, const float* chain_a, const float* b, const float* chain_b, const float* chain_out, int C, size_t V,
                        float* y, unsigned io, void* stream);

size_t dpi_pack_scratch_bytes(void);
size_t dpi_pack_slot_count(void);
int dpi_pack_forget(const void* w);
int dpi_pack_release(void);

#ifdef __cplusplus
}
#endif
#endif
```

Baseline: 33.94.

## Fuse BN stats/finalize/apply chains into single per-channel kernels

Refactors the BatchNorm statistics, finalize and apply kernels into device-inlined bodies and adds fused single-launch kernels (one block per channel) for join forward, stats plus finalize, join backward and BN backward. A per-chain size threshold decides whether the fused path or the old multi-kernel path runs, and a tunable stat span option is added. The goal is to cut kernel launch count and the round trips of partial sums through global memory for small volumes. The risk is lower parallelism, since one block per channel may underuse the GPU for large V.

```diff
diff --git a/deep_prior_interpolation_amd/_lib.py b/deep_prior_interpolation_amd/_lib.py
--- a/deep_prior_interpolation_amd/_lib.py
+++ b/deep_prior_interpolation_amd/_lib.py
@@ -126,7 +126,12 @@
     "dpi_join_bwd": (_I, [_P, _P, _P, _P, _P, _F, _I, _Z,  _P, _P, _P, _P, _P, _F,  _P, _P, _P, _P, _P, _F,  _P, _P,  _I, _I, _P, _P, _P, _F,
                           _P, _P, _P, _P, _P, _P, _P, _U, _P]),
     "dpi_chain_add_apply": (_I, [_P, _P, _P, _P, _P, _I, _Z, _P, _U, _P]),
+    "dpi_chain_fused": (_I, [_I, _I, _Z, _U]),
+    "dpi_bn_stats_finalize": (_I, [_P, _P, _I, _Z, _P, _P, _P, _F, _F, _F, _I, _P, _P, _P, _P, _P, _P, _U, _P]),
+    "dpi_bn_bwd": (_I, [_P, _P, _P, _P, _P, _P, _F, _F, _I, _Z, _P, _P, _P, _P, _U, _P]),
+    "dpi_join_fwd": (_I, [_P, _P, _P, _P, _I, _Z, _F, _P, _P, _P, _P, _F, _F, _P, _P, _P, _P, _P, _P, _U, _P]),
 }
+CHAIN_JOIN_FWD, CHAIN_STATS, CHAIN_JOIN_BWD, CHAIN_BN_BWD = 0, 1, 2, 3
 
 _lib = None
 
diff --git a/deep_prior_interpolation_amd/csrc/api.cpp b/deep_prior_interpolation_amd/csrc/api.cpp
--- a/deep_prior_interpolation_amd/csrc/api.cpp
+++ b/deep_prior_interpolation_amd/csrc/api.cpp
@@ -65,6 +65,12 @@
       {"q4_ck", 0, 4, [](int v) { dpi_set_q4(-1, v); }},
       {"q4_debug", 0, 0xFFFF, dpi_set_q4_debug},
       {"bf16_debug", 0, 0x7F, dpi_set_bf16_debug},
+      {"stat_span", 4, 1 << 24, dpi_set_stat_span},
+      {"chain_fuse", 0, 1, [](int v) { dpi_set_chain_fuse(-1, v); }},
+      {"chain_fuse_v_join_fwd", 0, 1 << 24, [](int v) { dpi_set_chain_fuse(DPI_CHAIN_JOIN_FWD, v); }},
+      {"chain_fuse_v_stats", 0, 1 << 24, [](int v) { dpi_set_chain_fuse(DPI_CHAIN_STATS, v); }},
+      {"chain_fuse_v_join_bwd", 0, 1 << 24, [](int v) { dpi_set_chain_fuse(DPI_CHAIN_JOIN_BWD, v); }},
+      {"chain_fuse_v_bn_bwd", 0, 1 << 24, [](int v) { dpi_set_chain_fuse(DPI_CHAIN_BN_BWD, v); }},
   };
   for (const Entry& e : table)
     if (strcmp(key, e.key) == 0) {
diff --git a/deep_prior_interpolation_amd/csrc/dpi_hip_internal.h b/deep_prior_interpolation_amd/csrc/dpi_hip_internal.h
--- a/deep_prior_interpolation_amd/csrc/dpi_hip_internal.h
+++ b/deep_prior_interpolation_amd/csrc/dpi_hip_internal.h
@@ -11,4 +11,6 @@
 DPI_INTERNAL void dpi_set_fewco_mfma(int on);
 DPI_INTERNAL void dpi_set_q4(int on, int ck);
 DPI_INTERNAL void dpi_set_q4_debug(int flags);
+DPI_INTERNAL void dpi_set_stat_span(int voxels);
+DPI_INTERNAL void dpi_set_chain_fuse(int chain, int value);
 }
diff --git a/deep_prior_interpolation_amd/csrc/elementwise.hip b/deep_prior_interpolation_amd/csrc/elementwise.hip
--- a/deep_prior_interpolation_amd/csrc/elementwise.hip
+++ b/deep_prior_interpolation_amd/csrc/elementwise.hip
@@ -22,11 +22,9 @@
   else *reinterpret_cast<float4*>(p) = v;
 }
 
-template <bool xb = false>
-__global__ __launch_bounds__(256) void channel_stats_kernel(const float* __restrict__ x, const float* __restrict__ chain,
-                                                            int C, size_t V, int nblk, double* __restrict__ partials) {
-  const bool nt = (size_t)gridDim.y * V >= kNtMinFloats;
-  const int c = blockIdx.y, b = blockIdx.x;
+template <bool xb>
+__device__ __forceinline__ void channel_stats_body(const float* __restrict__ x, const float* __restrict__ chain, int C, size_t V, int nblk,
+                                                   double* __restrict__ partials, int c, int b, bool nt, double& S, double& Q) {
   const size_t span = stat_span(V, nblk);
   const size_t beg = (size_t)b * span, end = beg + span < V ? beg + span : V;
   const float* __restrict__ xc = dpi_at(x, (size_t)c * V, xb);
@@ -54,31 +52,49 @@
     s += ls; q += lq;
   }
   __shared__ double sh[8];
-  const double S = block_sum(s, sh);
-  const double Q = block_sum(q, sh + 4);
+  S = block_sum(s, sh);
+  Q = block_sum(q, sh + 4);
   if (threadIdx.x == 0) {
     partials[((size_t)b * C + c) * 2 + 0] = S;
     partials[((size_t)b * C + c) * 2 + 1] = Q;
   }
 }
-
-__global__ __launch_bounds__(256) void bn_finalize_kernel(const double* __restrict__ partials, int nblk, int C, double count,
-                                                         const float* __restrict__ gamma, const float* __restrict__ beta,
-                                                         float eps, float momentum, float slope, int act_first,
-                                                         const float* __restrict__ in_chain, float* running_mean, float* running_var, int64_t* nbt,
-                                                         float* __restrict__ mean_invstd, float* __restrict__ chain_out) {
-  const int c = blockIdx.x, lane = threadIdx.x;
+template <bool xb = false>
+__global__ __launch_bounds__(256) void channel_stats_kernel(const float* __restrict__ x, const float* __restrict__ chain,
+                                                            int C, size_t V, int nblk, double* __restrict__ partials) {
+  double S, Q;
+  channel_stats_body<xb>(x, chain, C, V, nblk, partials, blockIdx.y, blockIdx.x, (size_t)gridDim.y * V >= kNtMinFloats, S, Q);
+}
+
+struct BnFinalizeArgs {
+  int nblk, C;
+  double count;
+  const float* gamma;
+  const float* beta;
+  float eps, momentum, slope;
+  int act_first;
+  const float* in_chain;
+  float* running_mean;
+  float* running_var;
+  int64_t* nbt;
+  float* mean_invstd;
+  float* chain_out;
+};
+template <class Part>
+__device__ __forceinline__ void bn_finalize_body(const BnFinalizeArgs& f, int c, Part part, float* lds_chain) {
+  const int lane = threadIdx.x, nblk = f.nblk, C = f.C;
+  const double count = f.count;
   double s = 0.0, q = 0.0;
   {
     double s1 = 0.0, q1 = 0.0;
     int b = lane;
     for (; b + 256 < nblk; b += 512) {
-      const double2 u = *reinterpret_cast<const double2*>(partials + ((size_t)b * C + c) * 2);
-      const double2 v = *reinterpret_cast<const double2*>(partials + ((size_t)(b + 256) * C + c) * 2);
+      const double2 u = part(b);
+      const double2 v = part(b + 256);
       s += u.x; q += u.y; s1 += v.x; q1 += v.y;
     }
     if (b < nblk) {
-      const double2 u = *reinterpret_cast<const double2*>(partials + ((size_t)b * C + c) * 2);
+      const double2 u = part(b);
       s += u.x; q += u.y;
     }
     s += s1; q += q1;
@@ -87,29 +103,39 @@
   s = block_sum(s, sh);
   q = block_sum(q, sh + 4);
   if (lane == 0) {
+    const float momentum = f.momentum, slope = f.slope;
     const double mean = s / count;
     double var = q / count - mean * mean;
     if (var < 0.0) var = 0.0;
-    const float invstd = (float)(1.0 / sqrt(var + (double)eps));
+    const float invstd = (float)(1.0 / sqrt(var + (double)f.eps));
     const float meanf = (float)mean;
-    if (mean_invstd) { mean_invstd[c] = meanf; mean_invstd[C + c] = invstd; }
-    if (running_mean) running_mean[c] = (1.f - momentum) * running_mean[c] + momentum * meanf;
-    if (running_var) {
+    if (f.mean_invstd) { f.mean_invstd[c] = meanf; f.mean_invstd[C + c] = invstd; }
+    if (f.running_mean) f.running_mean[c] = (1.f - momentum) * f.running_mean[c] + momentum * meanf;
+    if (f.running_var) {
       const double unb = count > 1.0 ? var * (count / (count - 1.0)) : var;
-      running_var[c] = (1.f - momentum) * running_var[c] + momentum * (float)unb;
-    }
-    if (nbt && c == 0) *nbt += 1;
-    if (chain_out) {
-      const float g = gamma ? gamma[c] : 1.f, bt = beta ? beta[c] : 0.f;
+      f.running_var[c] = (1.f - momentum) * f.running_var[c] + momentum * (float)unb;
+    }
+    if (f.nbt && c == 0) *f.nbt += 1;
+    if (f.chain_out || lds_chain) {
+      const float g = f.gamma ? f.gamma[c] : 1.f, bt = f.beta ? f.beta[c] : 0.f;
       const float a = g * invstd;
-      float* o = chain_out + (size_t)c * DPI_CHAIN_STRIDE;
-      if (in_chain) {
-        const float* ic = in_chain + (size_t)c * DPI_CHAIN_STRIDE;
+      float o[DPI_CHAIN_STRIDE];
+      if (f.in_chain) {
+        const float* ic = f.in_chain + (size_t)c * DPI_CHAIN_STRIDE;
         o[0] = ic[0]; o[1] = ic[1]; o[2] = ic[2]; o[3] = a * ic[3]; o[4] = fmaf(a, ic[4], bt - meanf * a);
-      } else if (act_first) { o[0] = 1.f; o[1] = 0.f; o[2] = slope; o[3] = a; o[4] = bt - meanf * a; }
+      } else if (f.act_first) { o[0] = 1.f; o[1] = 0.f; o[2] = slope; o[3] = a; o[4] = bt - meanf * a; }
       else { o[0] = a; o[1] = bt - meanf * a; o[2] = slope; o[3] = 1.f; o[4] = 0.f; }
-    }
-  }
+#pragma unroll
+      for (int i = 0; i < 5; ++i) {
+        if (f.chain_out) f.chain_out[(size_t)c * DPI_CHAIN_STRIDE + i] = o[i];
+        if (lds_chain) lds_chain[i] = o[i];
+      }
+    }
+  }
+}
+__global__ __launch_bounds__(256) void bn_finalize_kernel(const double* __restrict__ partials, BnFinalizeArgs f) {
+  const int c = blockIdx.x, C = f.C;
+  bn_finalize_body(f, c, [&](int b) { return *reinterpret_cast<const double2*>(partials + ((size_t)b * C + c) * 2); }, nullptr);
 }
 
 template <bool xb = false, bool yb = false>
@@ -157,14 +183,12 @@
   g = (k.post == 1.f || yv > 0.f) ? dy : dy * k.post;
 }
 
-template <bool fb = false, bool gb = false>
-__global__ __launch_bounds__(256) void bn_bwd_reduce_kernel(const float* __restrict__ dy, const float* __restrict__ x,
-                                                            const float* __restrict__ mean_invstd, const float* __restrict__ gamma,
-                                                            const float* __restrict__ beta, const float* __restrict__ in_chain,
-                                                            float pre, float post, int C, size_t V, int nblk,
-                                                            double* __restrict__ partials) {
-  const bool nt = (size_t)gridDim.y * V >= kNtMinFloats;
-  const int c = blockIdx.y, b = blockIdx.x;
+template <bool fb, bool gb>
+__device__ __forceinline__ void bn_bwd_reduce_body(const float* __restrict__ dy, const float* __restrict__ x,
+                                                   const float* __restrict__ mean_invstd, const float* __restrict__ gamma,
+                                                   const float* __restrict__ beta, const float* __restrict__ in_chain,
+                                                   float pre, float post, int C, size_t V, int nblk,
+                                                   double* __restrict__ partials, int c, int b, bool nt, double& S, double& Q) {
   const size_t span = stat_span(V, nblk);
   const size_t beg = (size_t)b * span, end = beg + span < V ? beg + span : V;
   const BnBwd k = bn_bwd_consts(mean_invstd, gamma, beta, in_chain, pre, post, C, c);
@@ -194,29 +218,38 @@
     s += ls; q += lq;
   }
   __shared__ double sh[8];
-  const double S = block_sum(s, sh);
-  const double Q = block_sum(q, sh + 4);
+  S = block_sum(s, sh);
+  Q = block_sum(q, sh + 4);
   if (threadIdx.x == 0) {
     partials[((size_t)b * C + c) * 2 + 0] = S;
     partials[((size_t)b * C + c) * 2 + 1] = Q;
   }
 }
-
 template <bool fb = false, bool gb = false>
-__global__ __launch_bounds__(256) void bn_bwd_apply_kernel(const float* __restrict__ dy, const float* __restrict__ x,
-                                                           const float* __restrict__ mean_invstd, const float* __restrict__ gamma,
-                                                           const float* __restrict__ beta, const float* __restrict__ in_chain,
-                                                           float pre, float post, const double* __restrict__ partials, int nblk, int C, size_t V,
-                                                           float* __restrict__ dx, float* __restrict__ dgamma,
-                                                           float* __restrict__ dbeta) {
-  const bool nt = (size_t)gridDim.y * V >= kNtMinFloats;
-  const int c = blockIdx.y;
+__global__ __launch_bounds__(256) void bn_bwd_reduce_kernel(const float* __restrict__ dy, const float* __restrict__ x,
+                                                            const float* __restrict__ mean_invstd, const float* __restrict__ gamma,
+                                                            const float* __restrict__ beta, const float* __restrict__ in_chain,
+                                                            float pre, float post, int C, size_t V, int nblk,
+                                                            double* __restrict__ partials) {
+  double S, Q;
+  bn_bwd_reduce_body<fb, gb>(dy, x, mean_invstd, gamma, beta, in_chain, pre, post, C, V, nblk, partials, blockIdx.y, blockIdx.x,
+                             (size_t)gridDim.y * V >= kNtMinFloats, S, Q);
+}
+
+template <bool fb, bool gb, class Part>
+__device__ __forceinline__ void bn_bwd_apply_body(const float* __restrict__ dy, const float* __restrict__ x,
+                                                  const float* __restrict__ mean_invstd, const float* __restrict__ gamma,
+                                                  const float* __restrict__ beta, const float* __restrict__ in_chain,
+                                                  float pre, float post, Part part, int nblk, int C, size_t V,
+                                                  float* __restrict__ dx, float* __restrict__ dgamma,
+                                                  float* __restrict__ dbeta, int c, unsigned bx, unsigned gx, bool nt) {
   __shared__ double tot[2];
   if (threadIdx.x < 64) {
     double s = 0.0, q = 0.0;
     for (int b = threadIdx.x; b < nblk; b += 64) {
-      s += partials[((size_t)b * C + c) * 2 + 0];
-      q += partials[((size_t)b * C + c) * 2 + 1];
+      const double2 u = part(b);
+      s += u.x;
+      q += u.y;
     }
     s = wave_sum(s);
     q = wave_sum(q);
@@ -225,7 +258,7 @@
   __syncthreads();
   const BnBwd k = bn_bwd_consts(mean_invstd, gamma, beta, in_chain, pre, post, C, c);
   const float k1 = (float)(tot[0] / (double)V), k2 = (float)(tot[1] / (double)V);
-  if (blockIdx.x == 0 && threadIdx.x == 0) {
+  if (bx == 0 && threadIdx.x == 0) {
     if (dgamma) dgamma[c] = (float)tot[1];
     if (dbeta) dbeta[c] = (float)tot[0];
   }
@@ -239,7 +272,7 @@
     const float du = k.a * (g - k1 - xh * k2);
     return (k.pre == 1.f || xv > 0.f) ? du : du * k.pre;
   };
-  for (size_t i = ((size_t)blockIdx.x * 256 + threadIdx.x) * 4; i < V; i += (size_t)gridDim.x * 1024) {
+  for (size_t i = ((size_t)bx * 256 + threadIdx.x) * 4; i < V; i += (size_t)gx * 1024) {
     if (vec) {
       const float4 f = dpi_ld4(xc, i, fb, nt);
       const float4 g = dpi_ld4(gc, i, gb, nt);
@@ -249,14 +282,24 @@
     }
   }
 }
-
-template <bool fb = false>
-__global__ __launch_bounds__(256) void chain_add_stats_kernel(const float* __restrict__ a, const float* __restrict__ chain_a,
-                                                              const float* __restrict__ b, const float* __restrict__ chain_b, int C,
-                                                              size_t V, int nblk, float slope, float* __restrict__ t,
-                                                              double* __restrict__ partials) {
-  const bool nt = (size_t)gridDim.y * V >= kNtMinFloats;
-  const int c = blockIdx.y, blk = blockIdx.x;
+template <bool fb = false, bool gb = false>
+__global__ __launch_bounds__(256) void bn_bwd_apply_kernel(const float* __restrict__ dy, const float* __restrict__ x,
+                                                           const float* __restrict__ mean_invstd, const float* __restrict__ gamma,
+                                                           const float* __restrict__ beta, const float* __restrict__ in_chain,
+                                                           float pre, float post, const double* __restrict__ partials, int nblk, int C, size_t V,
+                                                           float* __restrict__ dx, float* __restrict__ dgamma,
+                                                           float* __restrict__ dbeta) {
+  const int c = blockIdx.y;
+  bn_bwd_apply_body<fb, gb>(dy, x, mean_invstd, gamma, beta, in_chain, pre, post,
+                            [&](int b) { return make_double2(partials[((size_t)b * C + c) * 2 + 0], partials[((size_t)b * C + c) * 2 + 1]); },
+                            nblk, C, V, dx, dgamma, dbeta, c, blockIdx.x, gridDim.x, (size_t)gridDim.y * V >= kNtMinFloats);
+}
+
+template <bool fb>
+__device__ __forceinline__ void chain_add_stats_body(const float* __restrict__ a, const float* __restrict__ chain_a,
+                                                     const float* __restrict__ b, const float* __restrict__ chain_b, int C,
+                                                     size_t V, int nblk, float slope, float* __restrict__ t,
+                                                     double* __restrict__ partials, int c, int blk, bool nt, double& S, double& Q) {
   const size_t span = stat_span(V, nblk);
   const size_t beg = (size_t)blk * span, end = beg + span < V ? beg + span : V;
   const Chain ta = load_chain(chain_a, c), tb = load_chain(chain_b, c);
@@ -295,12 +338,21 @@
     s += ls; q += lq;
   }
   __shared__ double sh[8];
-  const double S = block_sum(s, sh);
-  const double Q = block_sum(q, sh + 4);
+  S = block_sum(s, sh);
+  Q = block_sum(q, sh + 4);
   if (threadIdx.x == 0) {
     partials[((size_t)blk * C + c) * 2 + 0] = S;
     partials[((size_t)blk * C + c) * 2 + 1] = Q;
   }
+}
+template <bool fb = false>
+__global__ __launch_bounds__(256) void chain_add_stats_kernel(const float* __restrict__ a, const float* __restrict__ chain_a,
+                                                              const float* __restrict__ b, const float* __restrict__ chain_b, int C,
+                                                              size_t V, int nblk, float slope, float* __restrict__ t,
+                                                              double* __restrict__ partials) {
+  double S, Q;
+  chain_add_stats_body<fb>(a, chain_a, b, chain_b, C, V, nblk, slope, t, partials, blockIdx.y, blockIdx.x,
+                           (size_t)gridDim.y * V >= kNtMinFloats, S, Q);
 }
 
 struct BnFork {
@@ -489,17 +541,15 @@
 }
 
 template <bool fb = false>
-__global__ __launch_bounds__(256) void chain_add_apply_kernel(const float* __restrict__ a, const float* __restrict__ chain_a,
-                                                              const float* __restrict__ b, const float* __restrict__ chain_b,
-                                                              const float* __restrict__ chain_out, size_t V, float* __restrict__ y) {
-  const bool nt = (size_t)gridDim.y * V >= kNtMinFloats;
-  const int c = blockIdx.y;
-  const Chain ta = load_chain(chain_a, c), tb = load_chain(chain_b, c), to = load_chain(chain_out, c);
+__device__ __forceinline__ void chain_add_apply_body(const float* __restrict__ a, const float* __restrict__ chain_a,
+                                                     const float* __restrict__ b, const float* __restrict__ chain_b,
+                                                     const Chain to, size_t V, float* __restrict__ y, int c, unsigned bx, unsigned gx, bool nt) {
+  const Chain ta = load_chain(chain_a, c), tb = load_chain(chain_b, c);
   const float* __restrict__ ac = dpi_at(a, (size_t)c * V, fb);
   const float* __restrict__ bc = dpi_at(b, (size_t)c * V, fb);
   float* __restrict__ yc = dpi_at(y, (size_t)c * V, fb);
   const bool vec = (V & 3) == 0;
-  for (size_t i = ((size_t)blockIdx.x * 256 + threadIdx.x) * 4; i < V; i += (size_t)gridDim.x * 1024) {
+  for (size_t i = ((size_t)bx * 256 + threadIdx.x) * 4; i < V; i += (size_t)gx * 1024) {
     if (vec) {
       const float4 f = dpi_ld4(ac, i, fb, nt), g = dpi_ld4(bc, i, fb, nt);
       float4 o;
@@ -511,6 +561,13 @@
         dpi_st(yc, i + j, apply_chain(to, apply_chain(ta, dpi_ld(ac, i + j, fb)) + apply_chain(tb, dpi_ld(bc, i + j, fb))), fb);
     }
   }
+}
+template <bool fb = false>
+__global__ __launch_bounds__(256) void chain_add_apply_kernel(const float* __restrict__ a, const float* __restrict__ chain_a,
+                                                              const float* __restrict__ b, const float* __restrict__ chain_b,
+                                                              const float* __restrict__ chain_out, size_t V, float* __restrict__ y) {
+  const int c = blockIdx.y;
+  chain_add_apply_body<fb>(a, chain_a, b, chain_b, load_chain(chain_out, c), V, y, c, blockIdx.x, gridDim.x, (size_t)gridDim.y * V >= kNtMinFloats);
 }
 
 constexpr int kJoinSums = 24;
@@ -532,12 +589,11 @@
   float post;
 };
 template <bool fb = false, bool gb = false>
-__global__ __launch_bounds__(256) void join_bwd_sums_kernel(const float* __restrict__ dy, const float* __restrict__ t,
-                                                            const float* __restrict__ mean_invstd, const float* __restrict__ gamma,
-                                                            const float* __restrict__ beta, float pre, JoinSide A, JoinSide B, JoinFork F,
-                                                            int C, size_t V, int nblk, double* __restrict__ partials) {
-  const bool nt = (size_t)gridDim.y * V >= kNtMinFloats;
-  const int c = blockIdx.y, b = blockIdx.x;
+__device__ __forceinline__ void join_bwd_sums_body(const float* __restrict__ dy, const float* __restrict__ t,
+                                                   const float* __restrict__ mean_invstd, const float* __restrict__ gamma,
+                                                   const float* __restrict__ beta, float pre, const JoinSide& A, const JoinSide& B, const JoinFork& F,
+                                                   int C, size_t V, int nblk, double* __restrict__ partials, int c, int b, bool nt,
+                                                   double* lds_part) {
   const BnBwd k = bn_bwd_consts(mean_invstd, gamma, beta, nullptr, pre, 1.f, C, c);
   const BnBwd ka = bn_bwd_consts(A.mean_invstd, A.gamma, A.beta, A.in_chain, 1.f, A.post, C, c);
   const BnBwd kb = bn_bwd_consts(B.mean_invstd, B.gamma, B.beta, B.in_chain, 1.f, B.post, C, c);
@@ -619,19 +675,29 @@
   __syncthreads();
   if (threadIdx.x < kJoinSums) {
     const int i = threadIdx.x;
-    partials[((size_t)b * C + c) * kJoinSums + i] = (sh[0][i] + sh[1][i]) + (sh[2][i] + sh[3][i]);
-  }
-}
-
-__global__ __launch_bounds__(64) void join_bwd_coef_kernel(const double* __restrict__ partials, int nblk, int C, double V,
-                                                          const float* __restrict__ mi_b, const float* __restrict__ gamma_b, int f_lo, int f_hi,
-                                                          float* __restrict__ coef, float* __restrict__ dgb, float* __restrict__ dgb_f) {
-  const int c = blockIdx.x, lane = threadIdx.x;
+    const double v = (sh[0][i] + sh[1][i]) + (sh[2][i] + sh[3][i]);
+    partials[((size_t)b * C + c) * kJoinSums + i] = v;
+    if (lds_part) lds_part[i] = v;
+  }
+}
+template <bool fb = false, bool gb = false>
+__global__ __launch_bounds__(256) void join_bwd_sums_kernel(const float* __restrict__ dy, const float* __restrict__ t,
+                                                            const float* __restrict__ mean_invstd, const float* __restrict__ gamma,
+                                                            const float* __restrict__ beta, float pre, JoinSide A, JoinSide B, JoinFork F,
+                                                            int C, size_t V, int nblk, double* __restrict__ partials) {
+  join_bwd_sums_body<fb, gb>(dy, t, mean_invstd, gamma, beta, pre, A, B, F, C, V, nblk, partials, blockIdx.y, blockIdx.x,
+                             (size_t)gridDim.y * V >= kNtMinFloats, nullptr);
+}
+
+template <class Part>
+__device__ __forceinline__ void join_bwd_coef_body(Part part, int nblk, int C, double V, const float* __restrict__ mi_b,
+                                                   const float* __restrict__ gamma_b, int f_lo, int f_hi, float* __restrict__ coef,
+                                                   float* __restrict__ dgb, float* __restrict__ dgb_f, int c, int lane, float* lds_coef) {
   double s[kJoinSums];
 #pragma unroll
   for (int i = 0; i < kJoinSums; ++i) s[i] = 0.0;
   for (int b = lane; b < nblk; b += 64) {
-    const double* __restrict__ p = partials + ((size_t)b * C + c) * kJoinSums;
+    const double* p = part(b);
 #pragma unroll
     for (int i = 0; i < kJoinSums; ++i) s[i] += p[i];
   }
@@ -654,25 +720,30 @@
   }
   float* o = coef + (size_t)c * 8;
   o[0] = k1f; o[1] = k2f; o[2] = a1f; o[3] = a2f; o[4] = b1f; o[5] = b2f; o[6] = f1f; o[7] = f2f;
+  if (lds_coef) { lds_coef[0] = k1f; lds_coef[1] = k2f; lds_coef[2] = a1f; lds_coef[3] = a2f; lds_coef[4] = b1f; lds_coef[5] = b2f; lds_coef[6] = f1f; lds_coef[7] = f2f; }
   dgb[c] = (float)s[1]; dgb[C + c] = (float)s[0]; dgb[2 * C + c] = (float)Ha; dgb[3 * C + c] = (float)Ga;
   dgb[4 * C + c] = (float)Hb; dgb[5 * C + c] = (float)Gb;
 }
-
-template <bool fb = false, bool gb = false>
-__global__ __launch_bounds__(256) void join_bwd_apply_kernel(const float* __restrict__ dy, const float* __restrict__ t,
-                                                             const float* __restrict__ mean_invstd, const float* __restrict__ gamma,
-                                                             const float* __restrict__ beta, float pre, JoinSide A, JoinSide B, JoinFork F,
-                                                             const float* __restrict__ coef, int C, size_t V, float* __restrict__ dxa,
-                                                             float* __restrict__ dxb, float* __restrict__ dxf) {
-  const bool nt = (size_t)gridDim.y * V >= kNtMinFloats;
-  const int c = blockIdx.y;
+__global__ __launch_bounds__(64) void join_bwd_coef_kernel(const double* __restrict__ partials, int nblk, int C, double V,
+                                                          const float* __restrict__ mi_b, const float* __restrict__ gamma_b, int f_lo, int f_hi,
+                                                          float* __restrict__ coef, float* __restrict__ dgb, float* __restrict__ dgb_f) {
+  const int c = blockIdx.x;
+  join_bwd_coef_body([&](int b) { return partials + ((size_t)b * C + c) * kJoinSums; }, nblk, C, V, mi_b, gamma_b, f_lo, f_hi, coef, dgb, dgb_f, c,
+                     threadIdx.x, nullptr);
+}
+
+template <bool fb, bool gb>
+__device__ __forceinline__ void join_bwd_apply_body(const float* __restrict__ dy, const float* __restrict__ t,
+                                                    const float* __restrict__ mean_invstd, const float* __restrict__ gamma,
+                                                    const float* __restrict__ beta, float pre, const JoinSide& A, const JoinSide& B, const JoinFork& F,
+                                                    const float* q, int C, size_t V, float* __restrict__ dxa,
+                                                    float* __restrict__ dxb, float* __restrict__ dxf, int c, unsigned bx, unsigned gx, bool nt) {
   const BnBwd k = bn_bwd_consts(mean_invstd, gamma, beta, nullptr, pre, 1.f, C, c);
   const BnBwd ka = bn_bwd_consts(A.mean_invstd, A.gamma, A.beta, A.in_chain, 1.f, A.post, C, c);
   const BnBwd kb = bn_bwd_consts(B.mean_invstd, B.gamma, B.beta, B.in_chain, 1.f, B.post, C, c);
   const bool forked = c >= F.lo && c < F.hi;
   const int fC = F.hi - F.lo, fc = forked ? c - F.lo : 0;
   const BnBwd kf = forked ? bn_bwd_consts(F.mean_invstd, F.gamma, F.beta, nullptr, 1.f, F.post, fC, fc) : ka;
-  const float* __restrict__ q = coef + (size_t)c * 8;
   const float k1 = q[0], k2 = q[1], a1 = q[2], a2 = q[3], b1 = q[4], b2 = q[5], f1 = q[6], f2 = q[7];
   const float* __restrict__ gc = dpi_at(dy, (size_t)c * V, gb);
   const float* __restrict__ tc = t ? dpi_at(t, (size_t)c * V, fb) : nullptr;
@@ -696,7 +767,7 @@
       rb = kf.a * (gg - f1 - xh * f2);
     }
   };
-  for (size_t i = ((size_t)blockIdx.x * 256 + threadIdx.x) * 4; i < V; i += (size_t)gridDim.x * 1024) {
+  for (size_t i = ((size_t)bx * 256 + threadIdx.x) * 4; i < V; i += (size_t)gx * 1024) {
     if (vec) {
       const float4 g = dpi_ld4(gc, i, gb, nt), p = dpi_ld4(xa, i, fb, nt), r = dpi_ld4(xb, i, fb, nt);
       float4 u;
@@ -717,6 +788,93 @@
       }
     }
   }
+}
+
+template <bool fb = false, bool gb = false>
+__global__ __launch_bounds__(256) void join_bwd_apply_kernel(const float* __restrict__ dy, const float* __restrict__ t,
+                                                             const float* __restrict__ mean_invstd, const float* __restrict__ gamma,
+                                                             const float* __restrict__ beta, float pre, JoinSide A, JoinSide B, JoinFork F,
+                                                             const float* __restrict__ coef, int C, size_t V, float* __restrict__ dxa,
+                                                             float* __restrict__ dxb, float* __restrict__ dxf) {
+  const int c = blockIdx.y;
+  join_bwd_apply_body<fb, gb>(dy, t, mean_invstd, gamma, beta, pre, A, B, F, coef + (size_t)c * 8, C, V, dxa, dxb, dxf, c, blockIdx.x, gridDim.x,
+                              (size_t)gridDim.y * V >= kNtMinFloats);
+}
+
+constexpr int kFuseMaxBlk = 16;
+
+__global__ __launch_bounds__(256) void stats_finalize_fused_kernel(const float* __restrict__ x, const float* __restrict__ chain, size_t V,
+                                                                   double* __restrict__ partials, BnFinalizeArgs f) {
+  const int c = blockIdx.x;
+  const bool nt = (size_t)gridDim.x * V >= kNtMinFloats;
+  __shared__ double part[kFuseMaxBlk][2];
+  for (int b = 0; b < f.nblk; ++b) {
+    double S, Q;
+    channel_stats_body<false>(x, chain, f.C, V, f.nblk, partials, c, b, nt, S, Q);
+    if (threadIdx.x == 0) { part[b][0] = S; part[b][1] = Q; }
+  }
+  __syncthreads();
+  bn_finalize_body(f, c, [&](int b) { return make_double2(part[b][0], part[b][1]); }, nullptr);
+}
+
+__global__ __launch_bounds__(256) void join_fwd_fused_kernel(const float* __restrict__ a, const float* __restrict__ chain_a,
+                                                             const float* __restrict__ b, const float* __restrict__ chain_b, size_t V,
+                                                             float* __restrict__ t, double* __restrict__ partials, BnFinalizeArgs f,
+                                                             float* __restrict__ y) {
+  const int c = blockIdx.x;
+  const bool nt = (size_t)gridDim.x * V >= kNtMinFloats;
+  __shared__ double part[kFuseMaxBlk][2];
+  __shared__ float ch[DPI_CHAIN_STRIDE];
+  for (int blk = 0; blk < f.nblk; ++blk) {
+    double S, Q;
+    chain_add_stats_body<false>(a, chain_a, b, chain_b, f.C, V, f.nblk, f.slope, t, partials, c, blk, nt, S, Q);
+    if (threadIdx.x == 0) { part[blk][0] = S; part[blk][1] = Q; }
+  }
+  __syncthreads();
+  bn_finalize_body(f, c, [&](int blk) { return make_double2(part[blk][0], part[blk][1]); }, ch);
+  __syncthreads();
+  Chain to;
+  to.ps = ch[0]; to.pb = ch[1]; to.slope = ch[2]; to.qs = ch[3]; to.qb = ch[4];
+  chain_add_apply_body<false>(a, chain_a, b, chain_b, to, V, y, c, 0, 1, nt);
+}
+
+__global__ __launch_bounds__(256) void bn_bwd_fused_kernel(const float* __restrict__ dy, const float* __restrict__ x,
+                                                           const float* __restrict__ mean_invstd, const float* __restrict__ gamma,
+                                                           const float* __restrict__ beta, const float* __restrict__ in_chain,
+                                                           float pre, float post, int C, size_t V, int nblk, double* __restrict__ partials,
+                                                           float* __restrict__ dx, float* __restrict__ dgamma, float* __restrict__ dbeta) {
+  const int c = blockIdx.x;
+  const bool nt = (size_t)gridDim.x * V >= kNtMinFloats;
+  __shared__ double part[kFuseMaxBlk][2];
+  for (int b = 0; b < nblk; ++b) {
+    double S, Q;
+    bn_bwd_reduce_body<false, false>(dy, x, mean_invstd, gamma, beta, in_chain, pre, post, C, V, nblk, partials, c, b, nt, S, Q);
+    if (threadIdx.x == 0) { part[b][0] = S; part[b][1] = Q; }
+  }
+  __syncthreads();
+  bn_bwd_apply_body<false, false>(dy, x, mean_invstd, gamma, beta, in_chain, pre, post,
+                                  [&](int b) { return make_double2(part[b][0], part[b][1]); }, nblk, C, V, dx, dgamma, dbeta, c, 0, 1, nt);
+}
+
+__global__ __launch_bounds__(256) void join_bwd_fused_kernel(const float* __restrict__ dy, const float* __restrict__ t,
+                                                             const float* __restrict__ mean_invstd, const float* __restrict__ gamma,
+                                                             const float* __restrict__ beta, float pre, JoinSide A, JoinSide B, JoinFork F,
+                                                             int C, size_t V, int nblk, double* __restrict__ partials, float* __restrict__ coef,
+                                                             float* __restrict__ dgb, float* __restrict__ dgb_f, float* __restrict__ dxa,
+                                                             float* __restrict__ dxb, float* __restrict__ dxf) {
+  const int c = blockIdx.x;
+  const bool nt = (size_t)gridDim.x * V >= kNtMinFloats;
+  __shared__ double part[kFuseMaxBlk][kJoinSums];
+  __shared__ float q[8];
+  for (int b = 0; b < nblk; ++b) {
+    join_bwd_sums_body<false, false>(dy, t, mean_invstd, gamma, beta, pre, A, B, F, C, V, nblk, partials, c, b, nt, part[b]);
+    __syncthreads();
+  }
+  if (threadIdx.x < 64)
+    join_bwd_coef_body([&](int b) { return (const double*)part[b]; }, nblk, C, (double)V, B.mean_invstd, B.gamma, F.lo, F.hi, coef, dgb, dgb_f, c,
+                       threadIdx.x, q);
+  __syncthreads();
+  join_bwd_apply_body<false, false>(dy, t, mean_invstd, gamma, beta, pre, A, B, F, q, C, V, dxa, dxb, dxf, c, 0, 1, nt);
 }
 
 __global__ __launch_bounds__(256) void lrelu_bwd_kernel(const float* __restrict__ dy, const float* __restrict__ x, float slope,
@@ -1061,11 +1219,26 @@
   return (unsigned)b;
 }
 
+int g_stat_span = kStatSpan;
+int g_chain_fuse = 1;
+size_t g_chain_fuse_max_v[DPI_CHAIN_COUNT] = {8192, 8192, 8192, 8192};
+
+}
+
+extern "C" void dpi_set_stat_span(int voxels) { g_stat_span = voxels; }
+extern "C" void dpi_set_chain_fuse(int chain, int value) {
+  if (chain < 0) g_chain_fuse = value;
+  else if (chain < DPI_CHAIN_COUNT) g_chain_fuse_max_v[chain] = (size_t)value;
+}
+
+extern "C" int dpi_chain_fused(int chain, int C, size_t V, unsigned io) {
+  if (chain < 0 || chain >= DPI_CHAIN_COUNT || C <= 0 || V == 0 || io != 0 || !g_chain_fuse) return 0;
+  return V <= g_chain_fuse_max_v[chain] && dpi_stat_blocks(C, V) <= kFuseMaxBlk;
 }
 
 extern "C" int dpi_stat_blocks(int C, size_t V) {
   if (C <= 0 || V == 0) return 0;
-  size_t n = cdivz(V, kStatSpan);
+  size_t n = cdivz(V, (size_t)g_stat_span);
   if (n > kMaxStatBlocks) n = kMaxStatBlocks;
   return (int)n;
 }
@@ -1102,9 +1275,27 @@
                                void* stream) {
   DPI_REQUIRE(partials && nblk > 0 && C > 0 && count > 0, "bn_finalize: bad argument");
   DPI_REQUIRE(!in_chain || (slope == 1.f && !act_first), "bn_finalize: a composed input chain excludes a fused activation");
-  bn_finalize_kernel<<<C, 256, 0, (hipStream_t)stream>>>(partials, nblk, C, (double)count, gamma, beta, eps, momentum, slope, act_first,
-                                                        in_chain, running_mean, running_var, num_batches_tracked, mean_invstd, chain_out);
+  const BnFinalizeArgs f{nblk, C, (double)count, gamma, beta, eps, momentum, slope, act_first, in_chain, running_mean, running_var,
+                         num_batches_tracked, mean_invstd, chain_out};
+  bn_finalize_kernel<<<C, 256, 0, (hipStream_t)stream>>>(partials, f);
   return dpi_check_launch("bn_finalize");
+}
+
+extern "C" int dpi_bn_stats_finalize(const float* x, const float* chain, int C, size_t V, double* partials, const float* gamma,
+                                     const float* beta, float eps, float momentum, float slope, int act_first, const float* in_chain,
+                                     float* running_mean, float* running_var, int64_t* num_batches_tracked, float* mean_invstd,
+                                     float* chain_out, unsigned io, void* stream) {
+  if (!dpi_chain_fused(DPI_CHAIN_STATS, C, V, io)) {
+    if (int e = dpi_channel_stats_io(x, chain, C, V, partials, io, stream)) return e;
+    return dpi_bn_finalize(partials, dpi_stat_blocks(C, V), C, V, gamma, beta, eps, momentum, slope, act_first, in_chain, running_mean,
+                           running_var, num_batches_tracked, mean_invstd, chain_out, stream);
+  }
+  DPI_REQUIRE(x && partials, "bn_stats_finalize: bad argument");
+  DPI_REQUIRE(!in_chain || (slope == 1.f && !act_first), "bn_stats_finalize: a composed input chain excludes a fused activation");
+  const BnFinalizeArgs f{dpi_stat_blocks(C, V), C, (double)V, gamma, beta, eps, momentum, slope, act_first, in_chain, running_mean, running_var,
+                         num_batches_tracked, mean_invstd, chain_out};
+  stats_finalize_fused_kernel<<<C, 256, 0, (hipStream_t)stream>>>(x, chain, V, partials, f);
+  return dpi_check_launch("bn_stats_finalize");
 }
 
 extern "C" int dpi_chain_apply_io(const float* x, const float* chain, int C, size_t V, float* y, unsigned io, void* stream) {
@@ -1150,6 +1341,21 @@
   DPI_LAUNCH_FG(io, bn_bwd_apply_kernel, dim3(gx, C), (hipStream_t)stream, dy, x, mean_invstd, gamma, beta, in_chain, pre_slope, post_slope, partials, nblk,
                 C, V, dx, dgamma, dbeta);
   return dpi_check_launch("bn_bwd_apply");
+}
+
+extern "C" int dpi_bn_bwd(const float* dy, const float* x, const float* mean_invstd, const float* gamma, const float* beta,
+                          const float* in_chain, float pre_slope, float post_slope, int C, size_t V, double* partials, float* dx,
+                          float* dgamma, float* dbeta, unsigned io, void* stream) {
+  if (!dpi_chain_fused(DPI_CHAIN_BN_BWD, C, V, io)) {
+    if (int e = dpi_bn_bwd_reduce_io(dy, x, mean_invstd, gamma, beta, in_chain, pre_slope, post_slope, C, V, partials, io, stream)) return e;
+    return dpi_bn_bwd_apply_io(dy, x, mean_invstd, gamma, beta, in_chain, pre_slope, post_slope, partials, dpi_stat_blocks(C, V), C, V, dx, dgamma,
+                               dbeta, io, stream);
+  }
+  DPI_REQUIRE(dy && x && mean_invstd && partials && dx, "bn_bwd: bad argument");
+  DPI_REQUIRE(!in_chain || pre_slope == 1.f, "bn_bwd: in_chain excludes pre_slope");
+  bn_bwd_fused_kernel<<<C, 256, 0, (hipStream_t)stream>>>(dy, x, mean_invstd, gamma, beta, in_chain, pre_slope, post_slope, C, V,
+                                                          dpi_stat_blocks(C, V), partials, dx, dgamma, dbeta);
+  return dpi_check_launch("bn_bwd");
 }
 
 extern "C" int dpi_bn_bwd_apply_fork(const float* dy, const float* x, const float* mean_invstd, const float* gamma, const float* beta,
@@ -1224,6 +1430,10 @@
   const JoinSide A{xa, mi_a, gamma_a, beta_a, chain_a, post_a, fwd_chain_a}, B{xb, mi_b, gamma_b, beta_b, chain_b, post_b, fwd_chain_b};
   const JoinFork F{f_lo, f_hi, f_mi, f_gamma, f_beta, f_post};
   hipStream_t st = (hipStream_t)stream;
+  if (dpi_chain_fused(DPI_CHAIN_JOIN_BWD, C, V, io)) {
+    join_bwd_fused_kernel<<<C, 256, 0, st>>>(dy, t, mi, gamma, beta, pre, A, B, F, C, V, nblk, ws, coef, dgb, dgb_f, dxa, dxb, dxf);
+    return dpi_check_launch("join_bwd (fused)");
+  }
   DPI_LAUNCH_FG(io, join_bwd_sums_kernel, dim3(nblk, C), st, dy, t, mi, gamma, beta, pre, A, B, F, C, V, nblk, ws);
   join_bwd_coef_kernel<<<C, 64, 0, st>>>(ws, nblk, C, (double)V, mi_b, gamma_b, f_lo, f_hi, coef, dgb, dgb_f);
   DPI_LAUNCH_FG(io, join_bwd_apply_kernel, dim3(ew_blocks(cdivz(V, 4 * 8)), C), st, dy, t, mi, gamma, beta, pre, A, B, F, coef, C, V, dxa, dxb, dxf);
@@ -1251,6 +1461,25 @@
   if (DPI_FB(io)) chain_add_apply_kernel<true><<<dim3(ew_blocks(cdivz(V, 4)), C), 256, 0, (hipStream_t)stream>>>(a, chain_a, b, chain_b, chain_out, V, y);
   else chain_add_apply_kernel<false><<<dim3(ew_blocks(cdivz(V, 4)), C), 256, 0, (hipStream_t)stream>>>(a, chain_a, b, chain_b, chain_out, V, y);
   return dpi_check_launch("chain_add_apply");
+}
+
+extern "C" int dpi_join_fwd(const float* a, const float* chain_a, const float* b, const float* chain_b, int C, size_t V, float slope, float* t,
+                            double* partials, const float* gamma, const float* beta, float eps, float momentum, float* running_mean,
+                            float* running_var, int64_t* num_batches_tracked, float* mean_invstd, float* chain_out, float* y, unsigned io,
+                            void* stream) {
+  DPI_REQUIRE(chain_out && y, "join_fwd: bad argument");
+  if (!dpi_chain_fused(DPI_CHAIN_JOIN_FWD, C, V, io)) {
+    if (int e = dpi_chain_add_stats_io(a, chain_a, b, chain_b, C, V, slope, t, partials, io, stream)) return e;
+    if (int e = dpi_bn_finalize(partials, dpi_stat_blocks(C, V), C, V, gamma, beta, eps, momentum, slope, 1, nullptr, running_mean, running_var,
+                                num_batches_tracked, mean_invstd, chain_out, stream))
+      return e;
+    return dpi_chain_add_apply(a, chain_a, b, chain_b, chain_out, C, V, y, io, stream);
+  }
+  DPI_REQUIRE(a && b && partials, "join_fwd: bad argument");
+  const BnFinalizeArgs f{dpi_stat_blocks(C, V), C, (double)V, gamma, beta, eps, momentum, slope, 1, nullptr, running_mean, running_var,
+                         num_batches_tracked, mean_invstd, chain_out};
+  join_fwd_fused_kernel<<<C, 256, 0, (hipStream_t)stream>>>(a, chain_a, b, chain_b, V, t, partials, f, y);
+  return dpi_check_launch("join_fwd");
 }
 
 extern "C" int dpi_lrelu_bwd(const float* dy, const float* x, float slope, size_t n, float* dx, void* stream) {
diff --git a/deep_prior_interpolation_amd/ops.py b/deep_prior_interpolation_amd/ops.py
--- a/deep_prior_interpolation_amd/ops.py
+++ b/deep_prior_interpolation_amd/ops.py
@@ -402,10 +402,9 @@
     L = _lib.load()
     nblk = L.dpi_stat_blocks(C_, V)
     part = torch.empty(nblk * C_ * 2, dtype=torch.float64, device=x.device)
-    check(L.dpi_channel_stats_io(ptr(x), ptr(chain_in), C_, V, ptr(part), _io(x), stream()), "dpi_channel_stats")
-    check(L.dpi_bn_finalize(ptr(part), nblk, C_, V, ptr(gamma), ptr(beta), eps, momentum, slope, act_first,
-                            ptr(chain_in) if compose else None, ptr(running_mean), ptr(running_var), ptr(nbt), ptr(mean_invstd),
-                            ptr(chain_out), stream()), "dpi_bn_finalize")
+    check(L.dpi_bn_stats_finalize(ptr(x), ptr(chain_in), C_, V, ptr(part), ptr(gamma), ptr(beta), eps, momentum, slope, act_first,
+                                  ptr(chain_in) if compose else None, ptr(running_mean), ptr(running_var), ptr(nbt), ptr(mean_invstd),
+                                  ptr(chain_out), _io(x), stream()), "dpi_bn_stats_finalize")
 
 
 def raw_bn_finalize(part, nblk, C_, count, gamma, beta, slope, running_mean, running_var, nbt, mean_invstd, chain_out,
@@ -483,15 +482,13 @@
     nblk = L.dpi_stat_blocks(C_, V)
     part = torch.empty(nblk * C_ * 2, dtype=torch.float64, device=x.device)
     io = _io(x, dy)
-    check(L.dpi_bn_bwd_reduce_io(ptr(dy), ptr(x), ptr(mi), ptr(gamma), ptr(beta), ptr(in_chain), pre_slope, post_slope, C_, V,
-                                 ptr(part), io, stream()), "dpi_bn_bwd_reduce")
     if dx is None:
         dx = torch.empty_like(dy)
     _same_type(dy, dx, "bn_backward")
     dgamma = torch.empty_like(gamma)
     dbeta = torch.empty_like(gamma)
-    check(L.dpi_bn_bwd_apply_io(ptr(dy), ptr(x), ptr(mi), ptr(gamma), ptr(beta), ptr(in_chain), pre_slope, post_slope, ptr(part), nblk,
-                                C_, V, ptr(dx), ptr(dgamma), ptr(dbeta), io, stream()), "dpi_bn_bwd_apply")
+    check(L.dpi_bn_bwd(ptr(dy), ptr(x), ptr(mi), ptr(gamma), ptr(beta), ptr(in_chain), pre_slope, post_slope, C_, V, ptr(part),
+                       ptr(dx), ptr(dgamma), ptr(dbeta), io, stream()), "dpi_bn_bwd")
     return dx, dgamma, dbeta
 
 
@@ -600,15 +597,17 @@
     t = torch.empty_like(a) if keep_t else None
     nblk = L.dpi_stat_blocks(C_, V)
     part = torch.empty(nblk * C_ * 2, dtype=torch.float64, device=dev)
+    ch_out = torch.empty(C_ * 5, dtype=torch.float32, device=dev)
+    if not keep_t:
+        check(L.dpi_join_fwd(ptr(a), ptr(ch_a), ptr(b), ptr(ch_b), C_, V, slope, None, ptr(part), ptr(gamma), ptr(beta), BN_EPS, BN_MOMENTUM,
+                             ptr(bn.running_mean), ptr(bn.running_var), ptr(bn.num_batches_tracked), ptr(mi_out), ptr(ch_out), ptr(y),
+                             _io(a), stream()), "dpi_join_fwd")
+        return None
     check(L.dpi_chain_add_stats_io(ptr(a), ptr(ch_a), ptr(b), ptr(ch_b), C_, V, slope, ptr(t), ptr(part), _io(a), stream()),
           "dpi_chain_add_stats")
-    ch_out = torch.empty(C_ * 5, dtype=torch.float32, device=dev)
     raw_bn_finalize(part, nblk, C_, V, gamma, beta, slope, bn.running_mean, bn.running_var, bn.num_batches_tracked, mi_out, ch_out,
                     act_first=1)
-    if keep_t:
-        raw_chain_apply(t, ch_out, C_, V, y)
-    else:
-        check(L.dpi_chain_add_apply(ptr(a), ptr(ch_a), ptr(b), ptr(ch_b), ptr(ch_out), C_, V, ptr(y), _io(a), stream()), "dpi_chain_add_apply")
+    raw_chain_apply(t, ch_out, C_, V, y)
     return t
 
 
diff --git a/include/dpi_hip.h b/include/dpi_hip.h
--- a/include/dpi_hip.h
+++ b/include/dpi_hip.h
@@ -223,6 +223,23 @@
 int dpi_chain_add_apply(const float* a, const float* chain_a, const float* b, const float* chain_b, const float* chain_out, int C, size_t V,
                         float* y, unsigned io, void* stream);
 
+#define DPI_CHAIN_JOIN_FWD 0
+#define DPI_CHAIN_STATS 1
+#define DPI_CHAIN_JOIN_BWD 2
+#define DPI_CHAIN_BN_BWD 3
+#define DPI_CHAIN_COUNT 4
+int dpi_chain_fused(int chain, int C, size_t V, unsigned io);
+int dpi_bn_stats_finalize(const float* x , const float* chain, int C, size_t V, double* partials, const float* gamma, const float* beta,
+                          float eps, float momentum, float slope, int act_first, const float* in_chain, float* running_mean,
+                          float* running_var, int64_t* num_batches_tracked, float* mean_invstd, float* chain_out, unsigned io, void* stream);
+int dpi_bn_bwd(const float* dy , const float* x , const float* mean_invstd, const float* gamma, const float* beta,
+               const float* in_chain, float pre_slope, float post_slope, int C, size_t V, double* partials, float* dx , float* dgamma,
+               float* dbeta, unsigned io, void* stream);
+int dpi_join_fwd(const float* a , const float* chain_a, const float* b , const float* chain_b, int C, size_t V, float slope,
+                 float* t , double* partials, const float* gamma, const float* beta, float eps, float momentum, float* running_mean,
+                 float* running_var, int64_t* num_batches_tracked, float* mean_invstd, float* chain_out, float* y , unsigned io,
+                 void* stream);
+
 size_t dpi_pack_scratch_bytes(void);
 size_t dpi_pack_slot_count(void);
 int dpi_pack_forget(const void* w);
```

Result: no change. 33.67, median of 2 (-0.8%).
